# Healthcare-Robotics/mr-gan

Measured on NVIDIA B200. Metric: gan_train_step_pairs_per_sec, higher is better.
Workload: dtype f16

## Files before the change

mr_gan_b200/csrc/kernels_tc.cuh:

```cuda
#pragma once
#include <cuda.h>
#include "common.cuh"

enum { HEAD_NONE = 0, HEAD_DISC = 1, HEAD_FM = 2, HEAD_BN = 3 };

struct alignas(64) TcOp {
  CUtensorMap mapA, mapB;
  GemmDesc g;
  int ME, NE, KE;
  int bn;
  int net;
  int ws_stride;
  float* ws;
  int esz;
  int head;
  int stats_stride;
  const void* hd;
  float* stats;
};

#define TC_KBLK 32
#define TC_SPIN_LIMIT (1ll << 31)

#ifdef MRGAN_PHASE_TIMING
__device__ __forceinline__ unsigned long long gtimer() { unsigned long long t; asm volatile("mov.u64 %0, %globaltimer;" : "=l"(t)); return t; }
#define PT_MARK(i) do { pt[i] = gtimer(); } while (0)
#else
#define PT_MARK(i) do { } while (0)
#endif

namespace tc {

__device__ __forceinline__ uint32_t smem_u32(const void* p) { return (uint32_t)__cvta_generic_to_shared(p); }

__device__ __forceinline__ void mbar_init(uint64_t* bar, uint32_t count) {
  asm volatile("mbarrier.init.shared::cta.b64 [%1], %0;" ::"r"(count), "r"(smem_u32(bar)) : "memory");
}
__device__ __forceinline__ void mbar_expect_tx(uint64_t* bar, uint32_t bytes) {
  asm volatile("mbarrier.arrive.expect_tx.shared::cta.b64 _, [%1], %0;" ::"r"(bytes), "r"(smem_u32(bar)) : "memory");
}
__device__ __forceinline__ bool mbar_try_wait(uint64_t* bar, uint32_t parity) {
  uint32_t ok;
  asm volatile(
      "{\n\t.reg .pred P1;\n\t"
      "mbarrier.try_wait.parity.shared::cta.b64 P1, [%1], %2;\n\t"
      "selp.b32 %0, 1, 0, P1;\n\t}"
      : "=r"(ok) : "r"(smem_u32(bar)), "r"(parity) : "memory");
  return ok != 0;
}
__device__ __forceinline__ void mbar_wait(uint64_t* bar, uint32_t parity) {
  if (mbar_try_wait(bar, parity)) return;
  const long long t0 = clock64();
  while (!mbar_try_wait(bar, parity)) {
    if (clock64() - t0 > TC_SPIN_LIMIT) __trap();
  }
}
__device__ __forceinline__ void tma_load_2d(const CUtensorMap* map, uint64_t* bar, void* dst, int c0, int c1) {
  asm volatile(
      "cp.async.bulk.tensor.2d.shared::cluster.global.mbarrier::complete_tx::bytes [%0], [%1, {%3, %4}], [%2];"
      ::"r"(smem_u32(dst)), "l"((uint64_t)map), "r"(smem_u32(bar)), "r"(c0), "r"(c1) : "memory");
}
__device__ __forceinline__ void prefetch_map(const CUtensorMap* map) {
  asm volatile("prefetch.tensormap [%0];" ::"l"((uint64_t)map) : "memory");
}
__device__ __forceinline__ void fence_before() { asm volatile("tcgen05.fence::before_thread_sync;" ::: "memory"); }
__device__ __forceinline__ void fence_after() { asm volatile("tcgen05.fence::after_thread_sync;" ::: "memory"); }

__device__ __forceinline__ uint64_t smem_desc(uint32_t saddr, uint32_t lbo, uint32_t sbo, uint32_t layout) {
  return (uint64_t)((saddr >> 4) & 0x3FFF) | ((uint64_t)((lbo >> 4) & 0x3FFF) << 16) |
         ((uint64_t)((sbo >> 4) & 0x3FFF) << 32) | (1ull << 46) | ((uint64_t)layout << 61);
}
__device__ __forceinline__ void mma_tf32(uint32_t tmem_d, uint64_t da, uint64_t db, uint32_t idesc, uint32_t accum) {
  asm volatile(
      "{\n\t.reg .pred p;\n\t"
      "setp.ne.b32 p, %4, 0;\n\t"
      "tcgen05.mma.cta_group::1.kind::tf32 [%0], %1, %2, %3, p;\n\t}"
      ::"r"(tmem_d), "l"(da), "l"(db), "r"(idesc), "r"(accum) : "memory");
}
__device__ __forceinline__ void mma_f16(uint32_t tmem_d, uint64_t da, uint64_t db, uint32_t idesc, uint32_t accum) {
  asm volatile(
      "{\n\t.reg .pred p;\n\t"
      "setp.ne.b32 p, %4, 0;\n\t"
      "tcgen05.mma.cta_group::1.kind::f16 [%0], %1, %2, %3, p;\n\t}"
      ::"r"(tmem_d), "l"(da), "l"(db), "r"(idesc), "r"(accum) : "memory");
}
__device__ __forceinline__ void mma_commit(uint64_t* bar) {
  asm volatile("tcgen05.commit.cta_group::1.mbarrier::arrive::one.shared::cluster.b64 [%0];" ::"r"(smem_u32(bar)) : "memory");
}
__device__ __forceinline__ void tmem_ld16(uint32_t taddr, float v[16]) {
  uint32_t r[16];
  asm volatile(
      "tcgen05.ld.sync.aligned.32x32b.x16.b32 {%0, %1, %2, %3, %4, %5, %6, %7, %8, %9, %10, %11, %12, %13, %14, %15}, [%16];"
      : "=r"(r[0]), "=r"(r[1]), "=r"(r[2]), "=r"(r[3]), "=r"(r[4]), "=r"(r[5]), "=r"(r[6]), "=r"(r[7]), "=r"(r[8]),
        "=r"(r[9]), "=r"(r[10]), "=r"(r[11]), "=r"(r[12]), "=r"(r[13]), "=r"(r[14]), "=r"(r[15])
      : "r"(taddr) : "memory");
  asm volatile("tcgen05.wait::ld.sync.aligned;" ::: "memory");
#pragma unroll
  for (int i = 0; i < 16; ++i) v[i] = __uint_as_float(r[i]);
}

__device__ __forceinline__ void tmem_ld16_issue(uint32_t taddr, uint32_t (&r)[16]) {
  asm volatile(
      "tcgen05.ld.sync.aligned.32x32b.x16.b32 {%0, %1, %2, %3, %4, %5, %6, %7, %8, %9, %10, %11, %12, %13, %14, %15}, [%16];"
      : "=r"(r[0]), "=r"(r[1]), "=r"(r[2]), "=r"(r[3]), "=r"(r[4]), "=r"(r[5]), "=r"(r[6]), "=r"(r[7]), "=r"(r[8]),
        "=r"(r[9]), "=r"(r[10]), "=r"(r[11]), "=r"(r[12]), "=r"(r[13]), "=r"(r[14]), "=r"(r[15])
      : "r"(taddr) : "memory");
}
__device__ __forceinline__ void tmem_wait_ld() { asm volatile("tcgen05.wait::ld.sync.aligned;" ::: "memory"); }
__device__ __forceinline__ void tmem_fence16(uint32_t (&r)[16]) {
  asm volatile("" : "+r"(r[0]), "+r"(r[1]), "+r"(r[2]), "+r"(r[3]), "+r"(r[4]), "+r"(r[5]), "+r"(r[6]), "+r"(r[7]), "+r"(r[8]),
                    "+r"(r[9]), "+r"(r[10]), "+r"(r[11]), "+r"(r[12]), "+r"(r[13]), "+r"(r[14]), "+r"(r[15]) :: "memory");
}

__device__ __forceinline__ void tmem_ld8(uint32_t taddr, float v[8]) {
  uint32_t r[8];
  asm volatile(
      "tcgen05.ld.sync.aligned.32x32b.x8.b32 {%0, %1, %2, %3, %4, %5, %6, %7}, [%8];"
      : "=r"(r[0]), "=r"(r[1]), "=r"(r[2]), "=r"(r[3]), "=r"(r[4]), "=r"(r[5]), "=r"(r[6]), "=r"(r[7])
      : "r"(taddr) : "memory");
  asm volatile("tcgen05.wait::ld.sync.aligned;" ::: "memory");
#pragma unroll
  for (int i = 0; i < 8; ++i) v[i] = __uint_as_float(r[i]);
}

__device__ __forceinline__ void tmem_ld4(uint32_t taddr, float v[4]) {
  uint32_t r[4];
  asm volatile("tcgen05.ld.sync.aligned.32x32b.x4.b32 {%0, %1, %2, %3}, [%4];"
               : "=r"(r[0]), "=r"(r[1]), "=r"(r[2]), "=r"(r[3]) : "r"(taddr) : "memory");
  asm volatile("tcgen05.wait::ld.sync.aligned;" ::: "memory");
#pragma unroll
  for (int i = 0; i < 4; ++i) v[i] = __uint_as_float(r[i]);
}

__device__ __forceinline__ void tmem_st4(uint32_t taddr, const float v[4]) {
  asm volatile("tcgen05.st.sync.aligned.32x32b.x4.b32 [%0], {%1, %2, %3, %4};"
               ::"r"(taddr), "r"(__float_as_uint(v[0])), "r"(__float_as_uint(v[1])), "r"(__float_as_uint(v[2])), "r"(__float_as_uint(v[3]))
               : "memory");
}
__device__ __forceinline__ void tmem_st16(uint32_t taddr, const float v[16]) {
  asm volatile(
      "tcgen05.st.sync.aligned.32x32b.x16.b32 [%0], {%1, %2, %3, %4, %5, %6, %7, %8, %9, %10, %11, %12, %13, %14, %15, %16};"
      ::"r"(taddr), "r"(__float_as_uint(v[0])), "r"(__float_as_uint(v[1])), "r"(__float_as_uint(v[2])), "r"(__float_as_uint(v[3])),
        "r"(__float_as_uint(v[4])), "r"(__float_as_uint(v[5])), "r"(__float_as_uint(v[6])), "r"(__float_as_uint(v[7])),
        "r"(__float_as_uint(v[8])), "r"(__float_as_uint(v[9])), "r"(__float_as_uint(v[10])), "r"(__float_as_uint(v[11])),
        "r"(__float_as_uint(v[12])), "r"(__float_as_uint(v[13])), "r"(__float_as_uint(v[14])), "r"(__float_as_uint(v[15]))
      : "memory");
}
__device__ __forceinline__ void tmem_wait_st() { asm volatile("tcgen05.wait::st.sync.aligned;" ::: "memory"); }

}


__device__ __forceinline__ void stg_f32(float* p, float v) { asm volatile("st.global.f32 [%0], %1;" ::"l"(p), "f"(v) : "memory"); }
__device__ __forceinline__ void stg_h16(__half* p, __half v) { asm volatile("st.global.b16 [%0], %1;" ::"l"(p), "h"(__half_as_ushort(v)) : "memory"); }

template <bool F16, int ACT, bool HAS_C, bool HAS_C2, bool FULL>
__device__ __forceinline__ void fwd_rows(const uint32_t (&va)[16], const float (&nz)[16], int nrows, float* pC, __half* hC, int ldc,
                                         bool c_op, float* pC2, __half* hC2, int ldc2, bool c2_op, float sigma, float alpha, bool mul) {
  float x[16];
#pragma unroll
  for (int j = 0; j < 16; ++j) {
    float v = __uint_as_float(va[j]);
    if (!F16) v *= TF32_TRUNC_DEBIAS;
    if (ACT == ACT_RELU) v = fmaxf(v, 0.f);
    else if (ACT == ACT_SOFTPLUS) v = softplus_fast(v);
    else if (ACT == ACT_LEAKY) v = v > 0.f ? v : alpha * v;
    x[j] = v;
  }
  if (HAS_C) {
    if (!F16 && c_op) {
#pragma unroll
      for (int j = 0; j < 16; ++j) if (FULL || j < nrows) stg_f32(pC + (uint32_t)(j * ldc), rna_tf32(x[j]));
    } else {
#pragma unroll
      for (int j = 0; j < 16; ++j) if (FULL || j < nrows) stg_f32(pC + (uint32_t)(j * ldc), x[j]);
    }
    if (F16 && c_op) {
#pragma unroll
      for (int j = 0; j < 16; ++j) if (FULL || j < nrows) stg_h16(hC + (uint32_t)(j * ldc), __float2half_rn(x[j]));
    }
  }
  if (HAS_C2) {
    float y[16];
#pragma unroll
    for (int j = 0; j < 16; ++j) y[j] = mul ? x[j] * nz[j] : fmaf(sigma, nz[j], x[j]);
    if (F16 && c2_op) {
#pragma unroll
      for (int j = 0; j < 16; ++j) if (FULL || j < nrows) stg_h16(hC2 + (uint32_t)(j * ldc2), __float2half_rn(y[j]));
    } else if (!F16 && c2_op) {
#pragma unroll
      for (int j = 0; j < 16; ++j) if (FULL || j < nrows) stg_f32(pC2 + (uint32_t)(j * ldc2), rna_tf32(y[j]));
    } else {
#pragma unroll
      for (int j = 0; j < 16; ++j) if (FULL || j < nrows) stg_f32(pC2 + (uint32_t)(j * ldc2), y[j]);
    }
  }
}

template <bool F16, int ACT, bool FULL>
__device__ __forceinline__ void dx_rows(const uint32_t (&va)[16], const float (&av)[16], int nrows, float* pC, __half* hC, int ldc, bool op_only,
                                        float alpha, float dinv, bool drop) {
  float x[16];
#pragma unroll
  for (int j = 0; j < 16; ++j) {
    float v = __uint_as_float(va[j]);
    if (!F16) v *= TF32_TRUNC_DEBIAS;
    if (ACT == ACT_RELU || ACT == ACT_LEAKY) {
      float m = (av[j] > 0.f ? 1.0f : (ACT == ACT_LEAKY ? alpha : 0.f)) * dinv;
      if (drop && av[j] == 0.f) m = 0.f;
      v *= m;
    } else if (ACT == ACT_SOFTPLUS) v *= 1.0f - __expf(-av[j]);
    x[j] = v;
  }
  if (F16 && op_only) {
#pragma unroll
    for (int j = 0; j < 16; ++j) if (FULL || j < nrows) stg_h16(hC + (uint32_t)(j * ldc), grad_to_half(x[j]));
  } else if (!F16 && op_only) {
#pragma unroll
    for (int j = 0; j < 16; ++j) if (FULL || j < nrows) stg_f32(pC + (uint32_t)(j * ldc), rna_tf32(x[j]));
  } else {
#pragma unroll
    for (int j = 0; j < 16; ++j) if (FULL || j < nrows) stg_f32(pC + (uint32_t)(j * ldc), x[j]);
  }
}


template <bool F16, int ACT>
__device__ __forceinline__ void head_chunk(uint32_t taddr, float (&x)[16], float alpha = 0.f) {
  tc::tmem_ld16(taddr, x);
#pragma unroll
  for (int j = 0; j < 16; ++j) {
    if (!F16) x[j] *= TF32_TRUNC_DEBIAS;
    if (ACT == ACT_RELU) x[j] = fmaxf(x[j], 0.f);
    else if (ACT == ACT_SOFTPLUS) x[j] = softplus_fast(x[j]);
    else if (ACT == ACT_LEAKY) x[j] = x[j] > 0.f ? x[j] : alpha * x[j];
  }
}

template <bool F16, int EPW>
__device__ __forceinline__ void head_disc(uint32_t trow, int cbeg, int ncols, int nall, int lane_base, int lane, int ewarp,
                                          const LossDesc& L, const AdamHyper& hp, const OperandMode& om, float* sl, float* part) {
  const int K = hp.n_classes, B = hp.dp_bloc;
  const float Bg = (float)hp.dp_bg;
  if (lane_base == 0) {
    for (int c0 = cbeg; c0 < ncols; c0 += 16) {
      float v[16];
      head_chunk<F16, ACT_NONE>(trow + (uint32_t)c0, v);
#pragma unroll
      for (int j = 0; j < 16; ++j)
        if (lane < K && c0 + j < ncols) sl[(c0 + j) * K + lane] = v[j];
    }
  }
  asm volatile("bar.sync 1, %0;" ::"r"(32 * EPW) : "memory");
  float s_lab = 0.f, s_unl = 0.f, s_err = 0.f;
  for (int r = ewarp * 32 + lane; r < nall; r += 32 * EPW) {
    const float* l = sl + r * K;
    float mx = l[0]; int am = 0;
    for (int k = 1; k < K; ++k) if (l[k] > mx) { mx = l[k]; am = k; }
    float se = 0.f;
    for (int k = 0; k < K; ++k) se += expf(l[k] - mx);
    const float lse = mx + logf(se), inv = 1.0f / se;
    float* dl = L.dlogits + (size_t)r * L.ld;
    if (r < B) {
      const int y = L.labels[r];
      s_lab += lse - l[y];
      s_err += (am != y) ? 1.f : 0.f;
      for (int k = 0; k < K; ++k) put_grad_operand(dl + k, (expf(l[k] - mx) * inv - (k == y ? 1.f : 0.f)) / Bg, om);
    } else {
      const float sp = softplusf(lse), sg = 1.0f / (1.0f + expf(-lse));
      float coef;
      if (r < 2 * B) { s_unl += 0.5f * (sp - lse); coef = 0.5f * (sg - 1.0f); }
      else           { s_unl += 0.5f * sp;         coef = 0.5f * sg; }
      coef *= hp.w_unl / Bg;
      for (int k = 0; k < K; ++k) put_grad_operand(dl + k, coef * expf(l[k] - mx) * inv, om);
    }
  }
  s_lab = warp_sum(s_lab); s_unl = warp_sum(s_unl); s_err = warp_sum(s_err);
  if (lane == 0) { part[3 * ewarp] = s_lab; part[3 * ewarp + 1] = s_unl; part[3 * ewarp + 2] = s_err; }
}

template <bool F16, bool VAR>
__device__ __forceinline__ void head_fm(uint32_t trow, int ncols, int f, bool f_ok, int lane, const LossDesc& L, const AdamHyper& hp,
                                        const OperandMode& om, float* red) {
  constexpr int HACT = VAR ? ACT_LEAKY : ACT_RELU;
  const int B = hp.dp_bloc;
  float mg = 0.f, mr = 0.f;
  for (int c0 = 0; c0 < ncols; c0 += 16) {
    float x[16];
    head_chunk<F16, HACT>(trow + (uint32_t)c0, x, hp.alpha);
#pragma unroll
    for (int j = 0; j < 16; ++j) {
      const int r = c0 + j;
      if (r < B) mg += x[j]; else if (r < ncols) mr += x[j];
    }
  }
  const float diff = (mg - mr) / B;
  const float part = warp_sum(f_ok ? diff * diff : 0.f);
  if (lane == 0) *red = part;
  float g = 2.0f * diff / ((float)L.Wmid * B);
  if (!F16) g = rna_tf32(g);
  for (int c0 = 0; c0 < B; c0 += 16) {
    float x[16];
    head_chunk<F16, HACT>(trow + (uint32_t)c0, x, hp.alpha);
    if (!f_ok) continue;
#pragma unroll
    for (int j = 0; j < 16; ++j) {
      const int r = c0 + j;
      if (r < B) put_grad_operand(L.dmid + (size_t)r * L.lddmid + f, x[j] > 0.f ? g : hp.alpha * g, om);
    }
  }
}

template <bool F16>
__device__ __forceinline__ void head_bn(uint32_t trow, int cbeg, int ncols, int nall, int f, bool f_ok, const BnDesc& Bd,
                                        const AdamHyper& hp, const OperandMode& om) {
  float s = 0.f, q = 0.f, x0 = 0.f;
  for (int c0 = 0; c0 < nall; c0 += 16) {
    float x[16];
    head_chunk<F16, ACT_SOFTPLUS>(trow + (uint32_t)c0, x);
    if (c0 == 0) x0 = x[0];
#pragma unroll
    for (int j = 0; j < 16; ++j) if (c0 + j < nall) { const float d = x[j] - x0; s += d; q = fmaf(d, d, q); }
  }
  const float md = s / nall, mu = x0 + md;
  const float istd = rsqrtf(fmaxf(q / nall - md * md, 0.f) + hp.bn_eps);
  float ga = 0.f, be = 0.f;
  if (f_ok) { if (cbeg == 0) Bd.istd[f] = istd; ga = Bd.gamma[f]; be = Bd.beta[f]; }
  for (int c0 = cbeg; c0 < ncols; c0 += 16) {
    float x[16];
    head_chunk<F16, ACT_SOFTPLUS>(trow + (uint32_t)c0, x);
    if (!f_ok) continue;
#pragma unroll
    for (int j = 0; j < 16; ++j) {
      const int r = c0 + j;
      if (r >= ncols) break;
      const float xh = (x[j] - mu) * istd;
      Bd.xhat[(size_t)r * Bd.ld + f] = xh;
      put_operand(Bd.u + (size_t)r * Bd.ldu + f, fmaf(ga, xh, be), om);
    }
  }
}

template <bool A_MN, bool B_MN, int STAGES, int TMEM_COLS, int MINB, int EPW, int MT, bool F16, bool VAR>
__global__ void __launch_bounds__(64 + 32 * EPW, MINB)
k_gemm_tc(const TcOp* __restrict__ ops, FoldState* __restrict__ folds, int rows_override, AdamHyper hp, OperandMode om) {
  using namespace tc;
#ifdef MRGAN_PHASE_TIMING
  const unsigned long long pt_t0 = gtimer();
#endif
  constexpr int KBLK = F16 ? 64 : 32;
  constexpr uint32_t MN_BOX = F16 ? 8192u : 4096u;
  const int ksplit = (B_MN && rows_override > 1) ? rows_override : 1;
  const int kslice = (int)blockIdx.z % ksplit;
  const TcOp& op = ops[blockIdx.z / ksplit];
  const int ME = op.ME, KE = op.KE, bn = op.bn;
  int NE = op.NE;
  if (rows_override > 0 && !B_MN) NE = rows_override;
  const int m0 = blockIdx.x * 128 * MT, n0 = blockIdx.y * bn;
  if (m0 >= ME || n0 >= NE) return;

  extern __shared__ uint8_t smem_raw[];
  uint8_t* smem = reinterpret_cast<uint8_t*>((reinterpret_cast<uintptr_t>(smem_raw) + 1023) & ~(uintptr_t)1023);
  const uint32_t a_bytes = MT * 128 * 128, b_bytes = (uint32_t)bn * 128, stage_bytes = a_bytes + b_bytes;
  uint64_t* bars = reinterpret_cast<uint64_t*>(smem + STAGES * stage_bytes);
  uint64_t* full = bars;
  uint64_t* empty = bars + STAGES;
  uint64_t* tmem_full = bars + 2 * STAGES;
  uint32_t* tmem_holder = reinterpret_cast<uint32_t*>(bars + 2 * STAGES + 1);
  float* const red = reinterpret_cast<float*>(bars + 24);
#ifdef MRGAN_PHASE_TIMING
  unsigned long long* pt = reinterpret_cast<unsigned long long*>(bars + 16);
  if (threadIdx.x == 0) pt[0] = pt_t0;
#endif

  const int warp = threadIdx.x >> 5, lane = threadIdx.x & 31;
  const int nkb_all = (KE + KBLK - 1) / KBLK;
  const int kb_per = (nkb_all + ksplit - 1) / ksplit;
  const int kb0 = kslice * kb_per;
  const int nkb = min(nkb_all, kb0 + kb_per) - kb0;

  if (warp == 0 && lane == 0) {
    prefetch_map(&op.mapA);
    prefetch_map(&op.mapB);
    for (int s = 0; s < STAGES; ++s) { mbar_init(&full[s], 1); mbar_init(&empty[s], 1); }
    mbar_init(tmem_full, 1);
    asm volatile("fence.mbarrier_init.release.cluster;" ::: "memory");
  }
  if (warp == 1) {
    asm volatile("tcgen05.alloc.cta_group::1.sync.aligned.shared::cta.b32 [%0], %1;" ::"r"(smem_u32(tmem_holder)), "r"((uint32_t)TMEM_COLS) : "memory");
    asm volatile("tcgen05.relinquish_alloc_permit.cta_group::1.sync.aligned;" ::: "memory");
  }
  fence_before();
  __syncthreads();
  fence_after();
  const uint32_t tmem_base = *tmem_holder;
  if (threadIdx.x == 0) PT_MARK(1);

  if (warp == 0) {
    if (lane == 0) {
      for (int kb = 0; kb < nkb; ++kb) {
        const int s = kb % STAGES;
        const uint32_t ph = (uint32_t)(kb / STAGES) & 1u;
        mbar_wait(&empty[s], ph ^ 1u);
        mbar_expect_tx(&full[s], stage_bytes);
        uint8_t* sa = smem + (size_t)s * stage_bytes;
        uint8_t* sb = sa + a_bytes;
        const int k0 = (kb0 + kb) * KBLK;
        if (A_MN) {
#pragma unroll
          for (int b = 0; b < (128 / KBLK) * MT; ++b) tma_load_2d(&op.mapA, &full[s], sa + b * MN_BOX, m0 + KBLK * b, k0);
        } else {
#pragma unroll
          for (int mt = 0; mt < MT; ++mt) tma_load_2d(&op.mapA, &full[s], sa + mt * 16384, k0, m0 + 128 * mt);
        }
        if (B_MN) {
          for (int b = 0; b < bn / KBLK; ++b) tma_load_2d(&op.mapB, &full[s], sb + b * MN_BOX, n0 + KBLK * b, k0);
        } else {
          tma_load_2d(&op.mapB, &full[s], sb, k0, n0);
        }
      }
    }
  } else if (warp == 1) {
    if (lane == 0) {
      constexpr uint32_t fmt = F16 ? 0u : 2u;
      const uint32_t idesc = (1u << 4) | (fmt << 7) | (fmt << 10) | ((A_MN ? 1u : 0u) << 15) | ((B_MN ? 1u : 0u) << 16) |
                             ((uint32_t)(bn >> 3) << 17) | ((128u >> 4) << 24);
      constexpr uint32_t mn_lbo = MN_BOX, mn_sbo = F16 ? 1024u : 512u, mn_lay = F16 ? 2u : 1u, mn_step = F16 ? 2048u : 1024u;
      constexpr uint32_t lboA = A_MN ? mn_lbo : 16u, lboB = B_MN ? mn_lbo : 16u;
      constexpr uint32_t sboA = A_MN ? mn_sbo : 1024u, sboB = B_MN ? mn_sbo : 1024u;
      constexpr uint32_t layA = A_MN ? mn_lay : 2u, layB = B_MN ? mn_lay : 2u;
      constexpr uint32_t stepA = A_MN ? mn_step : 32u, stepB = B_MN ? mn_step : 32u;
      for (int kb = 0; kb < nkb; ++kb) {
        const int s = kb % STAGES;
        const uint32_t ph = (uint32_t)(kb / STAGES) & 1u;
        mbar_wait(&full[s], ph);
        if (kb == 0) PT_MARK(2);
        fence_after();
        const uint32_t sa = smem_u32(smem + (size_t)s * stage_bytes), sb = sa + a_bytes;
#pragma unroll
        for (int k = 0; k < 4; ++k) {
          const uint64_t db = smem_desc(sb + k * stepB, lboB, sboB, layB);
#pragma unroll
          for (int mt = 0; mt < MT; ++mt) {
            const uint64_t da = smem_desc(sa + mt * 16384u + k * stepA, lboA, sboA, layA);
            if (F16) mma_f16(tmem_base + 256u * mt, da, db, idesc, (kb > 0 || k > 0) ? 1u : 0u);
            else mma_tf32(tmem_base + 256u * mt, da, db, idesc, (kb > 0 || k > 0) ? 1u : 0u);
          }
        }
        mma_commit(&empty[s]);
      }
      mma_commit(tmem_full);
      PT_MARK(3);
    }
  } else {
    const int lane_base = 32 * (warp & 3);
    const int wg = (warp - 2) >> 2;
    const int sub = (MT == 2) ? wg : 0;
    const int chalf = (EPW == 8 && MT == 1) ? (((min(bn, NE - n0) + 1) / 2 + 15) & ~15) : bn;
    const int cbeg = (EPW == 8 && MT == 1) ? wg * chalf : 0;
    const int f = m0 + 128 * sub + lane_base + lane;
    const bool f_ok = f < ME;
    const GemmDesc g = op.g;
    constexpr float debias = F16 ? 1.0f : TF32_TRUNC_DEBIAS;
    const int ncols = min(min(bn, NE - n0), cbeg + chalf);
    const uint32_t trow = tmem_base + 256u * sub + ((uint32_t)lane_base << 16);
    int fbeg, flen;
    if (MT == 2) { fbeg = 256 * sub + bn; flen = (256 - bn) & ~15; }
    else { flen = ((TMEM_COLS - bn) / (EPW == 8 ? 2 : 1)) & ~15; fbeg = bn + wg * flen; }
    const uint32_t tfree = tmem_base + ((uint32_t)lane_base << 16) + (uint32_t)fbeg;
    const int nchunks = (ncols - cbeg + 15) >> 4;
    const int npark = max(min(flen >> 4, nchunks), 0);

    if constexpr (B_MN) {
      mbar_wait(tmem_full, 0);
      fence_after();
      float* const dst = ksplit > 1 ? op.ws + (size_t)kslice * op.ws_stride : g.C;
      for (int c0 = cbeg; c0 < ncols; c0 += 16) {
        float v[16];
        tmem_ld16(trow + (uint32_t)c0, v);
        if (!f_ok) continue;
#pragma unroll
        for (int j = 0; j < 16; ++j) {
          const int k = n0 + c0 + j;
          if (k >= NE) break;
          dst[(size_t)k * g.ldc + f] = v[j];
        }
      }
    } else if constexpr (!A_MN) {
      const bool has_act = g.act != ACT_NONE;
      const bool drop = VAR && hp.drop > 0.f && (g.act == ACT_RELU || g.act == ACT_LEAKY) && g.tid >= 1;
      const __half* const haux = (F16 && drop) ? om.hbase + (g.aux - om.fbase) : nullptr;
      auto fetch = [&](int c0, float (&av)[16]) {
#pragma unroll
        for (int j = 0; j < 16; ++j) {
          const size_t o = (size_t)(n0 + c0 + j) * g.ldaux + f;
          av[j] = (f_ok && has_act && c0 + j < ncols) ? (haux ? __half2float(haux[o]) : __ldg(g.aux + o)) : 1.0f;
        }
      };
      float avA[16], avB[16];
      const int npk = has_act ? npark : 0;
      if (npk > 0) {
        fetch(cbeg, avA);
        for (int k = 0; k < npk; k += 2) {
          if (k + 1 < npk) fetch(cbeg + 16 * (k + 1), avB);
          tmem_st16(tfree + 16u * (uint32_t)k, avA);
          if (k + 1 < npk) {
            if (k + 2 < npk) fetch(cbeg + 16 * (k + 2), avA);
            tmem_st16(tfree + 16u * (uint32_t)(k + 1), avB);
          }
        }
        tmem_wait_st();
      }
      if (has_act && npk < nchunks) fetch(cbeg + 16 * npk, avA);
      mbar_wait(tmem_full, 0);
      fence_after();
      __half* const hC = F16 ? om.hbase + (g.C - om.fbase) : nullptr;
      const bool op_only = (g.rnd & 1) != 0;
      for (int ch = 0; ch < nchunks; ++ch) {
        const int c0 = cbeg + 16 * ch;
        uint32_t va[16], vh[16];
        tmem_ld16_issue(trow + (uint32_t)c0, va);
        if (ch < npk) tmem_ld16_issue(tfree + 16u * (uint32_t)ch, vh);
        tmem_wait_ld();
        tmem_fence16(va);
        float av[16];
        if (ch < npk) {
          tmem_fence16(vh);
#pragma unroll
          for (int j = 0; j < 16; ++j) av[j] = __uint_as_float(vh[j]);
        } else if (has_act) {
          const bool odd = ((ch - npk) & 1) != 0;
#pragma unroll
          for (int j = 0; j < 16; ++j) av[j] = odd ? avB[j] : avA[j];
          if (ch + 1 < nchunks) { if (odd) fetch(c0 + 16, avA); else fetch(c0 + 16, avB); }
        } else {
#pragma unroll
          for (int j = 0; j < 16; ++j) av[j] = 1.0f;
        }
        if (!f_ok) continue;
        const size_t o0 = (size_t)(n0 + c0) * g.ldc + f;
        const int nrows = ncols - c0;
        float* const pC = g.C + o0;
        __half* const phC = F16 ? hC + o0 : nullptr;
        const float dinv = drop ? hp.drop_inv : 1.0f;
#define DX_ACT(FULL)                                                                                                        \
        do {                                                                                                                    \
          if (g.act == ACT_RELU) dx_rows<F16, ACT_RELU, FULL>(va, av, nrows, pC, phC, g.ldc, op_only, 0.f, dinv, drop);         \
          else if (VAR && g.act == ACT_LEAKY) dx_rows<F16, ACT_LEAKY, FULL>(va, av, nrows, pC, phC, g.ldc, op_only, hp.alpha, dinv, drop); \
          else if (g.act == ACT_SOFTPLUS) dx_rows<F16, ACT_SOFTPLUS, FULL>(va, av, nrows, pC, phC, g.ldc, op_only, 0.f, 1.0f, false);      \
          else dx_rows<F16, ACT_NONE, FULL>(va, av, nrows, pC, phC, g.ldc, op_only, 0.f, 1.0f, false);                          \
        } while (0)
        if (nrows >= 16) DX_ACT(true); else DX_ACT(false);
#undef DX_ACT
      }
    } else {
      const bool mul = VAR && hp.drop > 0.f && g.C2 != nullptr && g.tid >= 1;
      const float ddrop = mul ? hp.drop : 0.f;
      const bool noisy = g.C2 != nullptr && (g.sigma != 0.f || mul);
      uint32_t key0 = 0, key1 = 0, step = 0;
      if (noisy) { const FoldState& fs = folds[g.fold]; key0 = fs.key0; key1 = fs.key1; step = (uint32_t)fs.rng_step; }
      const bool grp = ((g.row0 + n0 + cbeg) & 3) == 0 && (hp.dp_bg == hp.dp_bloc || (hp.dp_bloc & 3) == 0);
      const bool dp = hp.dp_bg != hp.dp_bloc;
      const int dprank = hp.dp_rank < 0 ? g.fold : hp.dp_rank;
      auto draw16 = [&](int c0, float (&nz)[16]) {
        const int r0 = g.row0 + n0 + c0;
        if (grp && !dp) {
#pragma unroll
          for (int q = 0; q < 4; ++q) {
            if (VAR) noise_or_drop4(key0, key1, (uint32_t)(r0 + 4 * q) >> 2, (uint32_t)f, step, (uint32_t)g.tid, ddrop, hp.drop_inv, &nz[4 * q]);
            else normal4(key0, key1, (uint32_t)(r0 + 4 * q) >> 2, (uint32_t)f, step, (uint32_t)g.tid, &nz[4 * q]);
          }
        } else if (grp) {
#pragma unroll
          for (int q = 0; q < 4; ++q) {
            const float4 n4 = noise4_call(key0, key1, r0 + 4 * q, (uint32_t)f, step, (uint32_t)g.tid, hp.dp_bloc, hp.dp_bg, dprank, ddrop, hp.drop_inv);
            nz[4 * q] = n4.x; nz[4 * q + 1] = n4.y; nz[4 * q + 2] = n4.z; nz[4 * q + 3] = n4.w;
          }
        } else {
#pragma unroll
          for (int j = 0; j < 16; ++j)
            nz[j] = noise1_call(key0, key1, r0 + j, (uint32_t)f, step, (uint32_t)g.tid, hp.dp_bloc, hp.dp_bg, dprank, ddrop, hp.drop_inv);
        }
      };
      const int npk = (noisy && grp) ? npark : 0;
      for (int ch = 0; ch < npk; ++ch) {
        float nz[16];
        draw16(cbeg + 16 * ch, nz);
        tmem_st16(tfree + 16u * (uint32_t)ch, nz);
      }
      if (npk > 0) tmem_wait_st();
      if (warp == 2 && lane == 0) PT_MARK(4);
      mbar_wait(tmem_full, 0);
      if (warp == 2 && lane == 0) PT_MARK(5);
      fence_after();
      __half* const hC = (F16 && g.C) ? om.hbase + (g.C - om.fbase) : nullptr;
      __half* const hC2 = (F16 && g.C2) ? om.hbase + (g.C2 - om.fbase) : nullptr;
      const bool c_op = (g.rnd & 1) != 0, c2_op = (g.rnd & 2) != 0;
#ifdef MRGAN_PHASE_TIMING
      unsigned long long tch[24];
#endif
      for (int it = 0; it < nchunks; ++it) {
        const int ch = (wg & 1) ? nchunks - 1 - it : it;
        const int c0 = cbeg + 16 * ch;
        uint32_t va[16], vn[16];
        float nz[16];
#ifdef MRGAN_PHASE_TIMING
        if (ch < 12) tch[2 * ch] = gtimer();
#endif
        tmem_ld16_issue(trow + (uint32_t)c0, va);
        if (ch < npk) tmem_ld16_issue(tfree + 16u * (uint32_t)ch, vn);
        else if (noisy) draw16(c0, nz);
        tmem_wait_ld();
#ifdef MRGAN_PHASE_TIMING
        if (ch < 12) tch[2 * ch + 1] = gtimer();
#endif
        tmem_fence16(va);
        if (ch < npk) {
          tmem_fence16(vn);
#pragma unroll
          for (int j = 0; j < 16; ++j) nz[j] = __uint_as_float(vn[j]);
        }
        if (!f_ok) continue;
        const size_t o0 = (size_t)(n0 + c0) * g.ldc + f, o20 = (size_t)(n0 + c0) * g.ldc2 + f;
        const int nrows = ncols - c0;
        float* const pC = g.C ? g.C + o0 : nullptr;
        float* const pC2 = g.C2 ? g.C2 + o20 : nullptr;
        __half* const phC = hC ? hC + o0 : nullptr;
        __half* const phC2 = hC2 ? hC2 + o20 : nullptr;
        if (!noisy) {
#pragma unroll
          for (int j = 0; j < 16; ++j) nz[j] = 0.f;
        }
#define FWD_ROWS(ACT, HC, HC2, FULL) \
        fwd_rows<F16, ACT, HC, HC2, FULL>(va, nz, nrows, pC, phC, g.ldc, c_op, pC2, phC2, g.ldc2, c2_op, g.sigma, hp.alpha, VAR && mul)
#define FWD_ACT(HC, HC2, FULL)                                                     \
        do {                                                                       \
          if (g.act == ACT_RELU) FWD_ROWS(ACT_RELU, HC, HC2, FULL);                \
          else if (g.act == ACT_SOFTPLUS) FWD_ROWS(ACT_SOFTPLUS, HC, HC2, FULL);   \
          else if (VAR && g.act == ACT_LEAKY) FWD_ROWS(ACT_LEAKY, HC, HC2, FULL);  \
          else FWD_ROWS(ACT_NONE, HC, HC2, FULL);                                  \
        } while (0)
#define FWD_OUT(FULL)                                                              \
        do {                                                                       \
          if (g.C && g.C2) FWD_ACT(true, true, FULL);                              \
          else if (g.C) FWD_ACT(true, false, FULL);                                \
          else if (g.C2) FWD_ACT(false, true, FULL);                               \
        } while (0)
        if (nrows >= 16) FWD_OUT(true); else FWD_OUT(false);
#undef FWD_OUT
#undef FWD_ACT
#undef FWD_ROWS
      }
#ifdef MRGAN_PHASE_TIMING
      if (warp == 2 && lane == 0 && blockIdx.x == 0 && blockIdx.z == 0 && nchunks >= 10) {
        const unsigned long long te2 = gtimer();
        const unsigned long long b = pt[0];
        printf("PTCH npk=%d: %llu+%llu %llu+%llu %llu+%llu %llu+%llu %llu+%llu %llu+%llu %llu+%llu %llu+%llu %llu+%llu %llu+%llu end=%llu\n", npk,
               tch[0] - b, tch[1] - tch[0], tch[2] - b, tch[3] - tch[2], tch[4] - b, tch[5] - tch[4], tch[6] - b, tch[7] - tch[6], tch[8] - b, tch[9] - tch[8],
               tch[10] - b, tch[11] - tch[10], tch[12] - b, tch[13] - tch[12], tch[14] - b, tch[15] - tch[14], tch[16] - b, tch[17] - tch[16],
               tch[18] - b, tch[19] - tch[18], te2 - b);
      }
#endif
      if (op.head == HEAD_DISC) {
        float* const sl = reinterpret_cast<float*>(smem);
        head_disc<F16, EPW>(trow, cbeg, ncols, min(bn, NE - n0), lane_base, lane, warp - 2, *static_cast<const LossDesc*>(op.hd), hp, om,
                            sl, sl + 8192);
      } else if (op.head == HEAD_FM) {
        head_fm<F16, VAR>(trow, ncols, f, f_ok, lane, *static_cast<const LossDesc*>(op.hd), hp, om, red + (warp - 2));
      } else if (op.head == HEAD_BN) {
        head_bn<F16>(trow, cbeg, ncols, min(bn, NE - n0), f, f_ok, *static_cast<const BnDesc*>(op.hd), hp, om);
      }
    }
  }

  if (warp == 2 && lane == 0) PT_MARK(6);
  fence_before();
  __syncthreads();
  if (warp == 1) {
    fence_after();
    asm volatile("tcgen05.dealloc.cta_group::1.sync.aligned.b32 %0, %1;" ::"r"(tmem_base), "r"((uint32_t)TMEM_COLS) : "memory");
  }
  if (!B_MN && A_MN && threadIdx.x == 0 && (op.head == HEAD_DISC || op.head == HEAD_FM)) {
    float* const st = op.stats + (size_t)hp.t * op.stats_stride;
    if (op.head == HEAD_DISC) {
      const float Bg = (float)hp.dp_bg;
      const float* part = reinterpret_cast<const float*>(smem) + 8192;
      float a0 = 0.f, a1 = 0.f, a2 = 0.f;
      for (int w = 0; w < EPW; ++w) { a0 += part[3 * w]; a1 += part[3 * w + 1]; a2 += part[3 * w + 2]; }
      st[0] = a0 / Bg; st[1] = a1 / Bg; st[2] = a2 / Bg;
      FoldState& fs = folds[op.g.fold];
      if (hp.shared_t) fs.iterations += 1; else fs.it_net[0] += 1;
      fs.rng_step += 1;
    } else {
      float sum = 0.f;
      for (int w = 0; w < EPW; ++w) sum += red[w];
      st[3] = sum / static_cast<const LossDesc*>(op.hd)->Wmid;
    }
  }
#ifdef MRGAN_PHASE_TIMING
  if (threadIdx.x == 0 && blockIdx.x == 0 && blockIdx.y == 0 && (blockIdx.z % 24) == 0) {
    const unsigned long long te = gtimer();
    printf("PT z=%d grid=(%d,%d,%d) nkb=%d t0=%llu setup=%llu first=%llu mma_issued=%llu noise=%llu acc=%llu epi=%llu end=%llu\n", (int)blockIdx.z,
           (int)gridDim.x, (int)gridDim.y, (int)gridDim.z, nkb, pt[0], pt[1] - pt[0], pt[2] - pt[0], pt[3] - pt[0], pt[4] - pt[0], pt[5] - pt[0], pt[6] - pt[0], te - pt[0]);
  }
#endif
}

__global__ void __launch_bounds__(256) k_splitk_reduce(const TcOp* __restrict__ ops, int ks) {
  const TcOp& op = ops[blockIdx.y];
  const size_t n4 = (size_t)op.NE * op.g.ldc / 4, stride4 = (size_t)op.ws_stride / 4;
  const float4* __restrict__ ws = reinterpret_cast<const float4*>(op.ws);
  float4* __restrict__ out = reinterpret_cast<float4*>(op.g.C);
  for (size_t i = (size_t)blockIdx.x * blockDim.x + threadIdx.x; i < n4; i += (size_t)gridDim.x * blockDim.x) {
    float4 a = ws[i];
    for (int s = 1; s < ks; ++s) {
      const float4 b = ws[(size_t)s * stride4 + i];
      a.x += b.x; a.y += b.y; a.z += b.z; a.w += b.w;
    }
    out[i] = a;
  }
}

struct alignas(64) TcAdamOp {
  CUtensorMap mapA, mapB;
  CUtensorMap mapP, mapM, mapV;
  CUtensorMap mapH;
  int ME, NE, KE;
  int fold;
  int net;
  float ginv;
};

#define TCA_KC 8

namespace tc {
__device__ __forceinline__ void tma_store_2d(const CUtensorMap* map, const void* src, int c0, int c1) {
  asm volatile("cp.async.bulk.tensor.2d.global.shared::cta.bulk_group [%0, {%2, %3}], [%1];"
               ::"l"((uint64_t)map), "r"(smem_u32(src)), "r"(c0), "r"(c1) : "memory");
}
__device__ __forceinline__ void bulk_commit() { asm volatile("cp.async.bulk.commit_group;" ::: "memory"); }
__device__ __forceinline__ void bulk_wait_read0() { asm volatile("cp.async.bulk.wait_group.read 0;" ::: "memory"); }
__device__ __forceinline__ void mbar_arrive(uint64_t* bar) {
  asm volatile("mbarrier.arrive.shared::cta.b64 _, [%0];" ::"r"(smem_u32(bar)) : "memory");
}
__device__ __forceinline__ void fence_proxy_async() { asm volatile("fence.proxy.async.shared::cta;" ::: "memory"); }
}

template <bool F16, int KROWS> struct TcAdamCfg {
  static_assert(KROWS == (F16 ? 32 : 16), "operand stage geometry: 16 KB stages");
  static constexpr int STAGES = 2, KC = TCA_KC, NB = 3;
  static constexpr int MINB = 3;
  static constexpr uint32_t MN_BOX = 128u * KROWS;
  static constexpr uint32_t STAGE_BYTES = (F16 ? 4 : 8) * MN_BOX;
  static constexpr uint32_t ARR_BYTES = KC * 128 * 4;
  static constexpr uint32_t HALF_BYTES = F16 ? KC * 128 * 2 : 0;
  static constexpr uint32_t CHUNK_BYTES = 3 * ARR_BYTES + HALF_BYTES;
  static constexpr int NX = (STAGES * STAGE_BYTES) / CHUNK_BYTES;
  static constexpr int NBUF = NB + NX;
  static constexpr size_t SMEM = (size_t)STAGES * STAGE_BYTES + (size_t)NB * CHUNK_BYTES + 256;
};

template <bool F16, int KROWS>
__global__ void __launch_bounds__(192, (TcAdamCfg<F16, KROWS>::MINB))
k_dw_adam_tc(const TcAdamOp* __restrict__ ops, FoldState* __restrict__ folds, AdamHyper hp, int nfl, int op_stride) {
  using namespace tc;
  using Cfg = TcAdamCfg<F16, KROWS>;
  constexpr int STAGES = Cfg::STAGES, KC = Cfg::KC, NB = Cfg::NB, NBUF = Cfg::NBUF;
  constexpr uint32_t STAGE_BYTES = Cfg::STAGE_BYTES, ARR_BYTES = Cfg::ARR_BYTES, CHUNK_BYTES = Cfg::CHUNK_BYTES;
  constexpr int KBLK = KROWS;
  constexpr uint32_t MN_BOX = Cfg::MN_BOX;
  constexpr int MN_BOXES = F16 ? 2 : 4;
  constexpr int MN_W = F16 ? 64 : 32;
  const TcAdamOp& op = ops[((int)blockIdx.z / nfl) * op_stride + ((int)blockIdx.z % nfl)];
  const int ME = op.ME, NE = op.NE, KE = op.KE;
  const int m0 = blockIdx.x * 128, n0 = blockIdx.y * 128;
  if (m0 >= ME || n0 >= NE) return;

  extern __shared__ __align__(1024) uint8_t smem_dyn[];
  uint8_t* smem = smem_dyn;
  if ((smem_u32(smem) & 1023u) != 0) __trap();
  uint8_t* cbuf = smem + STAGES * STAGE_BYTES;
  uint64_t* bars = reinterpret_cast<uint64_t*>(cbuf + NB * CHUNK_BYTES);
  uint64_t* full = bars;
  uint64_t* empty = bars + STAGES;
  uint64_t* tmem_full = bars + 2 * STAGES;
  uint64_t* cfull = bars + 2 * STAGES + 1;
  uint64_t* cdone = cfull + NBUF;
  uint32_t* tmem_holder = reinterpret_cast<uint32_t*>(cdone + NBUF);
  auto buf_ptr = [&](int b) -> uint8_t* { return b < NB ? cbuf + (size_t)b * CHUNK_BYTES : smem + (size_t)(b - NB) * CHUNK_BYTES; };

  const int warp = threadIdx.x >> 5, lane = threadIdx.x & 31;
  const int nkb = (KE + KBLK - 1) / KBLK;
  const int ncols = min(128, NE - n0);
  const int nch = (ncols + KC - 1) / KC;

  if (warp == 0 && lane == 0) {
    prefetch_map(&op.mapA); prefetch_map(&op.mapB); prefetch_map(&op.mapP); prefetch_map(&op.mapM); prefetch_map(&op.mapV);
    if (F16) prefetch_map(&op.mapH);
    for (int s = 0; s < STAGES; ++s) { mbar_init(&full[s], 1); mbar_init(&empty[s], 1); }
    mbar_init(tmem_full, 1);
    for (int b = 0; b < NBUF; ++b) { mbar_init(&cfull[b], 1); mbar_init(&cdone[b], 128); }
    asm volatile("fence.mbarrier_init.release.cluster;" ::: "memory");
  }
  if (warp == 1) {
    asm volatile("tcgen05.alloc.cta_group::1.sync.aligned.shared::cta.b32 [%0], %1;" ::"r"(smem_u32(tmem_holder)), "r"(128u) : "memory");
    asm volatile("tcgen05.relinquish_alloc_permit.cta_group::1.sync.aligned;" ::: "memory");
  }
  fence_before();
  __syncthreads();
  fence_after();
  const uint32_t tmem_base = *tmem_holder;

  if (warp == 0) {
    if (lane == 0) {
      auto load_chunk = [&](int c) {
        const int b = c % NBUF;
        uint8_t* dst = buf_ptr(b);
        mbar_expect_tx(&cfull[b], 3 * ARR_BYTES);
        tma_load_2d(&op.mapP, &cfull[b], dst, m0, n0 + c * KC);
        tma_load_2d(&op.mapM, &cfull[b], dst + ARR_BYTES, m0, n0 + c * KC);
        tma_load_2d(&op.mapV, &cfull[b], dst + 2 * ARR_BYTES, m0, n0 + c * KC);
      };
      for (int c = 0; c < NB && c < nch; ++c) load_chunk(c);
      for (int kb = 0; kb < nkb; ++kb) {
        const int s = kb % STAGES;
        const uint32_t ph = (uint32_t)(kb / STAGES) & 1u;
        mbar_wait(&empty[s], ph ^ 1u);
        mbar_expect_tx(&full[s], STAGE_BYTES);
        uint8_t* sa = smem + (size_t)s * STAGE_BYTES;
        uint8_t* sb = sa + STAGE_BYTES / 2;
        const int k0 = kb * KBLK;
#pragma unroll
        for (int b = 0; b < MN_BOXES; ++b) tma_load_2d(&op.mapA, &full[s], sa + b * MN_BOX, m0 + MN_W * b, k0);
#pragma unroll
        for (int b = 0; b < MN_BOXES; ++b) tma_load_2d(&op.mapB, &full[s], sb + b * MN_BOX, n0 + MN_W * b, k0);
      }
      mbar_wait(tmem_full, 0);
      for (int c = NB; c < NBUF && c < nch; ++c) load_chunk(c);
      for (int c = 0; c < nch; ++c) {
        const int b = c % NBUF;
        mbar_wait(&cdone[b], (uint32_t)(c / NBUF) & 1u);
        const uint8_t* src = buf_ptr(b);
        tma_store_2d(&op.mapP, src, m0, n0 + c * KC);
        tma_store_2d(&op.mapM, src + ARR_BYTES, m0, n0 + c * KC);
        tma_store_2d(&op.mapV, src + 2 * ARR_BYTES, m0, n0 + c * KC);
        if (F16) tma_store_2d(&op.mapH, src + 3 * ARR_BYTES, m0, n0 + c * KC);
        bulk_commit();
        if (c >= 1 && c - 1 + NBUF < nch) {
          asm volatile("cp.async.bulk.wait_group.read 1;" ::: "memory");
          load_chunk(c - 1 + NBUF);
        }
      }
      bulk_wait_read0();
    }
  } else if (warp == 1) {
    if (lane == 0) {
      constexpr uint32_t fmt = F16 ? 0u : 2u;
      constexpr uint32_t idesc = (1u << 4) | (fmt << 7) | (fmt << 10) | (1u << 15) | (1u << 16) | ((128u >> 3) << 17) | ((128u >> 4) << 24);
      constexpr uint32_t lbo = MN_BOX, sbo = F16 ? 1024u : 512u, lay = F16 ? 2u : 1u, kstep = F16 ? 2048u : 1024u;
      for (int kb = 0; kb < nkb; ++kb) {
        const int s = kb % STAGES;
        const uint32_t ph = (uint32_t)(kb / STAGES) & 1u;
        mbar_wait(&full[s], ph);
        fence_after();
        const uint32_t sa = smem_u32(smem + (size_t)s * STAGE_BYTES), sb = sa + STAGE_BYTES / 2;
#pragma unroll
        for (int k = 0; k < KROWS / (F16 ? 16 : 8); ++k) {
          const uint64_t da = smem_desc(sa + k * kstep, lbo, sbo, lay), db = smem_desc(sb + k * kstep, lbo, sbo, lay);
          if (F16) mma_f16(tmem_base, da, db, idesc, (kb > 0 || k > 0) ? 1u : 0u);
          else mma_tf32(tmem_base, da, db, idesc, (kb > 0 || k > 0) ? 1u : 0u);
        }
        mma_commit(&empty[s]);
      }
      mma_commit(tmem_full);
    }
  } else {
    const int lane_base = 32 * (warp & 3);
    const int nl = lane_base + lane;
    const uint32_t trow = tmem_base + ((uint32_t)lane_base << 16);
    const float lr_t = folds[op.fold].lr_t[op.net];
    const float b1 = hp.b1, b2 = hp.b2, c1 = 1.0f - hp.b1, c2 = 1.0f - hp.b2, eps = hp.eps;
    const float ginv = op.ginv;
    mbar_wait(tmem_full, 0);
    fence_after();
    for (int c = 0; c < nch; ++c) {
      const int b = c % NBUF;
      float* sP = reinterpret_cast<float*>(buf_ptr(b));
      float* sM = sP + KC * 128;
      float* sV = sM + KC * 128;
      __half* sH = reinterpret_cast<__half*>(sV + KC * 128);
      float g[KC];
      tmem_ld8(trow + (uint32_t)(c * KC), g);
      mbar_wait(&cfull[b], (uint32_t)(c / NBUF) & 1u);
#pragma unroll
      for (int j = 0; j < KC; ++j) {
        const int i = j * 128 + nl;
        const float gr = F16 ? g[j] * ginv : g[j];
        const float m = fmaf(b1, sM[i], c1 * gr), v = fmaf(b2, sV[i], c2 * gr * gr);
        sM[i] = m; sV[i] = v;
        const float w = sP[i] - lr_t * __fdividef(m, sqrtf(v) + eps);
        sP[i] = w;
        if (F16) sH[i] = __float2half_rn(w);
      }
      fence_proxy_async();
      mbar_arrive(&cdone[b]);
    }
  }

  fence_before();
  __syncthreads();
  if (warp == 1) {
    fence_after();
    asm volatile("tcgen05.dealloc.cta_group::1.sync.aligned.b32 %0, %1;" ::"r"(tmem_base), "r"(128u) : "memory");
  }
}
```

mr_gan_b200/csrc/mrgan_api.cu:

```cuda
#include <cuda_runtime.h>
#include <cuda_fp16.h>
#include <dlfcn.h>
#include <math.h>
#include <stdio.h>
#include <stdlib.h>
#include <string.h>
#include <algorithm>
#include <map>
#include <string>
#include <vector>

#include "../../include/mrgan.h"
#include "kernels_simt.cuh"
#include "kernels_tc.cuh"
#include "kernels_svm.cuh"
#include "kernels_dp.cuh"

namespace {

thread_local std::string g_last_error;

enum Op {
  OP_G1, OP_G2, OP_G3D, OP_G3G,
  OP_D1, OP_D2, OP_D3, OP_D4, OP_D5, OP_D6,
  OP_DW1, OP_DW2, OP_DW3, OP_DW4, OP_DW5, OP_DW6,
  OP_DX2, OP_DX3, OP_DX4, OP_DX5, OP_DX6,
  OP_DX1G,
  OP_D1G, OP_D2G, OP_D3G, OP_D4G, OP_D5G,
  OP_DX2G, OP_DX3G, OP_DX4G, OP_DX5G,
  OP_GW1, OP_GW2, OP_GW3, OP_GX2, OP_GX3,
  OP_E1, OP_E1S, OP_E2, OP_E3, OP_E4, OP_E5, OP_E6,
  NUM_OPS,
  OP_EX2 = NUM_OPS, OP_EX3, OP_EX4, OP_EX5, OP_EX6,
  OP_EX1,
  NUM_OPS_ALL
};
constexpr int NUM_EX = NUM_OPS_ALL - NUM_OPS;

struct OpInfo { bool at = false, bt = false, used = false; int maxM = 0, maxN = 0; };

struct Arena {
  char* base = nullptr; size_t off = 0;
  template <typename T> T* take(size_t count) {
    off = (off + 255) & ~(size_t)255;
    T* p = base ? reinterpret_cast<T*>(base + off) : nullptr;
    off += count * sizeof(T);
    return p;
  }
};

struct TensorLayout { int rows, cols, pitch; long long off; };

struct NetLayout {
  std::vector<TensorLayout> t;
  long long n = 0;
  long long n_ref = 0;
  long long off = 0;
};

struct FoldBuffers {
  float *a[6], *hb[6], *dz[6], *lg, *dlg, *dfake, *zb, *h1g, *xhat, *istd, *u, *h2g, *dz2g, *du, *dz1g;
  float *stage_x, *stage_z, *ex_stage, *xte, *eh[6], *elg, *xtr, *eval_out, *eval_out_s;
  int *stage_y, *labels_cur, *ey_stage, *ytr, *yte, *idx;
  int *pred, *pred_s;
  int *lab_rows, *unl_rows;
  int n_lab = 0, n_unl = 0;
  int lda[6], ldz[6];
  bool loaded = false;
};

}

struct mrgan_handle;
namespace {
int tc_setup(mrgan_handle* h);
int tc_ex_setup(mrgan_handle* h, TcOp* dst);
void tc_teardown(mrgan_handle* h);
bool tc_launch_gemm(mrgan_handle* h, int op, int f0, int nfl, int rows_override, cudaStream_t st);
void tc_launch_dw_adam(mrgan_handle* h, int op, int nlayers, int f0, int nfl, cudaStream_t st);
bool tc_dw_merge(const mrgan_handle* h);
int tc_debug_gemm(mrgan_handle* h, int mode, const GemmDesc& g, int esz);
}

constexpr int kMaxChains = 16;
struct mrgan_handle {
  mrgan_config cfg;
  int nf = 0, R = 0, NE = 0, n_train = 0;
  std::vector<mrgan_fold_shape> shapes;
  std::vector<NetLayout> net[2];
  std::vector<FoldBuffers> fb;
  cudaStream_t stream = nullptr;
  cudaStream_t side = nullptr;
  cudaEvent_t ev_pool[16] = {nullptr}; int ev_next = 0;
  bool side_open = false;
  int nchains = 1;
  cudaStream_t cmain[kMaxChains] = {nullptr}, cside[kMaxChains] = {nullptr};
  char* arena = nullptr; size_t arena_bytes = 0;
  __half* harena = nullptr;
  OperandMode om = {0, 1.0f, nullptr, nullptr};
  float *P = nullptr, *Mo = nullptr, *Vo = nullptr, *Gr = nullptr; long long n_flat = 0;
  FoldState* d_folds = nullptr; std::vector<FoldState> h_folds;
  GemmDesc* d_descs = nullptr; std::vector<GemmDesc> h_descs;
  PermDesc* d_perm = nullptr;
  BnDesc* d_bn = nullptr; LossDesc* d_loss = nullptr; EvalDesc *d_eval = nullptr, *d_eval_s = nullptr;
  int* d_conf = nullptr;
  struct SalWork {
    char* mem = nullptr;
    GemmDesc* descs = nullptr;
    float* profile = nullptr;
    TcOp* tcops = nullptr;
  } sal;
  AdamRange* d_ranges[2] = {nullptr, nullptr};
  OpInfo ops[NUM_OPS_ALL];
  float *d_step_stats = nullptr, *d_epoch_stats = nullptr, *h_epoch_stats = nullptr;
  int* h_idx_pinned[2] = {nullptr, nullptr}; cudaEvent_t idx_free[2] = {nullptr, nullptr}; int idx_slot = 0;
  float* h_scratch = nullptr;
  std::map<int, cudaGraphExec_t> graphs;
  std::map<int, long long> graph_nodes;
  cudaEvent_t ev0 = nullptr, ev1 = nullptr;
  bool epoch_pending = false; double last_ms = 0.0;
  long long launches = 0;
  std::string err;
  int sticky = 0;
  AdamHyper hp;
  struct Dataset { float* x = nullptr; int* y = nullptr; int n = 0, D = 0, ld = 0; } datasets[8];
  double* d_prep_stats = nullptr; int* d_prep_rows = nullptr; int prep_rows_cap = 0, prep_stats_cap = 0;
  int dp_world = 1, dp_rank = 0;
  bool dp_virtual = false;
  bool dp_fused = false;
  unsigned* d_dpflags = nullptr;
  char* peer_arena[DP_MAX_RANKS] = {nullptr}; __half* peer_harena[DP_MAX_RANKS] = {nullptr};
  DpPeers dp_peers[2];
  void* nccl_comm = nullptr;
  float* d_dpmem = nullptr; DpBufs* d_dpbufs = nullptr;
  float *dp_bnf = nullptr, *dp_bnb = nullptr, *dp_fm = nullptr;
  float* dp_losspart = nullptr; unsigned* dp_lossctr = nullptr;
  TcOp* d_tcops = nullptr;
  int tc_bn[NUM_OPS_ALL] = {0}, tc_maxME[NUM_OPS_ALL] = {0}, tc_maxNE[NUM_OPS_ALL] = {0};
  int tc_ksplit[NUM_OPS] = {0};
  bool tc_mt1[NUM_OPS_ALL] = {false};
  float* d_tcws = nullptr;
  bool tc_fused_adam = true;
  int tc_heads = 0;
  TcAdamOp* d_tcadam = nullptr;
  AdamRange* d_ranges_tc[2] = {nullptr, nullptr};
  struct Svm {
    char* mem = nullptr; size_t bytes = 0;
    int n_lab = 0, npairs = 0, npmax = 0, max_rows = 0, max_nte = 0;
    double eps = 1e-3;
    bool fitted = false;
    std::vector<float*> Klab, Kte, dec;
    std::vector<int*> wrong;
    int *d_iters = nullptr, *d_capped = nullptr, *d_count = nullptr, *d_nte = nullptr;
    SvmSplitOp* d_split = nullptr; SvmGemmOp* d_gemm = nullptr; SvmPairJob* d_jobs = nullptr;
    float** d_Kt = nullptr; float** d_dec = nullptr; int** d_yte = nullptr; int** d_wrong = nullptr; int** d_pred = nullptr;
    std::vector<SvmGemmOp> h_gemm;
    float *Xs = nullptr, *Hs = nullptr, *Ls = nullptr, *Ks = nullptr, *decs = nullptr; double* ns = nullptr; int* preds = nullptr;
    SvmSplitOp* d_split_s = nullptr; SvmGemmOp* d_gemm_s = nullptr;
    float** d_Ks = nullptr; float** d_decs = nullptr; int** d_preds = nullptr; int* d_ns = nullptr;
    char* cv_mem = nullptr; size_t cv_bytes = 0;
  } svm;
};

namespace {

int take_sticky(mrgan_handle* h);

int fail(mrgan_handle* h, int code, const std::string& msg) {
  if (h) h->err = msg;
  g_last_error = msg;
  return code;
}

#define CKS()                                                                                      \
  do {                                                                                             \
    CK(cudaGetLastError());                                                                        \
    const int _s = take_sticky(h);                                                                 \
    if (_s) return _s;                                                                             \
  } while (0)

#define CK(expr)                                                                                   \
  do {                                                                                             \
    cudaError_t _e = (expr);                                                                       \
    if (_e != cudaSuccess)                                                                         \
      return fail(h, MRGAN_ERR_CUDA, std::string(#expr) + ": " + cudaGetErrorString(_e));          \
  } while (0)

const int kDW[5] = {1000, 500, 250, 250, 250};
const int kGH = 500;

long long align32(long long x) { return (x + 31) & ~31LL; }

NetLayout layout_disc(int D, int K) {
  NetLayout L;
  int dims[7] = {D, kDW[0], kDW[1], kDW[2], kDW[3], kDW[4], K};
  for (int l = 0; l < 6; ++l) {
    TensorLayout t{dims[l] + 1, dims[l + 1], pitch8(dims[l + 1]), L.n};
    L.t.push_back(t);
    L.n = align32(L.n + (long long)t.rows * t.pitch);
    L.n_ref += (long long)(dims[l] + 1) * dims[l + 1];
  }
  return L;
}

NetLayout layout_gen(int D, int nd) {
  NetLayout L;
  auto add = [&](int rows, int cols) {
    TensorLayout t{rows, cols, pitch8(cols), L.n};
    L.t.push_back(t);
    L.n = align32(L.n + (long long)rows * t.pitch);
    L.n_ref += (long long)rows * cols;
  };
  add(nd + 1, kGH);
  add(1, kGH);
  add(1, kGH);
  add(kGH + 1, kGH);
  add(kGH + 1, D);
  return L;
}

__global__ void k_round_tf32(float* p, size_t n) {
  for (size_t i = (size_t)blockIdx.x * blockDim.x + threadIdx.x; i < n; i += (size_t)gridDim.x * blockDim.x) p[i] = rna_tf32(p[i]);
}

__global__ void k_set_col(float* p, int ld, int rows, int col, float v, OperandMode om) {
  const int r = blockIdx.x * blockDim.x + threadIdx.x;
  if (r < rows) {
    p[(size_t)r * ld + col] = v;
    if (om.mode == 2) om.hbase[p + (size_t)r * ld + col - om.fbase] = __float2half_rn(v);
  }
}

__global__ void k_scale_buf(float* p, size_t n, float mul) {
  for (size_t i = (size_t)blockIdx.x * blockDim.x + threadIdx.x; i < n; i += (size_t)gridDim.x * blockDim.x) p[i] *= mul;
}

__global__ void k_from_half(const float* src, float* dst, size_t n, float mul, OperandMode om) {
  for (size_t i = (size_t)blockIdx.x * blockDim.x + threadIdx.x; i < n; i += (size_t)gridDim.x * blockDim.x)
    dst[i] = __half2float(om.hbase[src + i - om.fbase]) * mul;
}

void layout_buffers(mrgan_handle* h, Arena& ar) {
  const mrgan_config& c = h->cfg;
  const int B = c.batch, R = h->R, NE = h->NE, K = c.n_classes, nd = c.noise_dim, nf = h->nf;
  const bool gan = c.model == MRGAN_MODEL_GAN;
  if (c.model == MRGAN_MODEL_SVM) {
    for (int f = 0; f < nf; ++f) {
      FoldBuffers& b = h->fb[f];
      const int D = h->shapes[f].D;
      b.lda[0] = pitch8(D + 1);
      b.xte = ar.take<float>((size_t)h->shapes[f].n_test * b.lda[0]);
      b.xtr = ar.take<float>((size_t)h->shapes[f].n_train * pitch8(D));
      b.ytr = ar.take<int>(h->shapes[f].n_train);
      b.yte = ar.take<int>(h->shapes[f].n_test);
      b.pred = ar.take<int>(h->shapes[f].n_test);
    }
    h->d_eval = ar.take<EvalDesc>(nf);
    h->d_conf = ar.take<int>((size_t)nf * K * K);
    return;
  }
  h->P = ar.take<float>(h->n_flat);
  h->Mo = ar.take<float>(h->n_flat);
  h->Vo = ar.take<float>(h->n_flat);
  h->Gr = ar.take<float>(h->n_flat);
  h->d_folds = ar.take<FoldState>(nf);
  h->d_descs = ar.take<GemmDesc>((size_t)NUM_OPS * nf);
  h->d_perm = ar.take<PermDesc>(nf);
  h->d_bn = ar.take<BnDesc>(nf);
  h->d_loss = ar.take<LossDesc>(nf);
  h->d_eval = ar.take<EvalDesc>(nf);
  h->d_eval_s = ar.take<EvalDesc>(nf);
  h->d_ranges[0] = ar.take<AdamRange>(nf);
  h->d_ranges[1] = ar.take<AdamRange>(nf);
  h->d_step_stats = ar.take<float>((size_t)(h->n_train / B + 1) * nf * 4);
  h->d_dpflags = ar.take<unsigned>((size_t)DP_MAX_RANKS * DP_FLAG_WORDS);
  h->d_epoch_stats = ar.take<float>((size_t)nf * 8);
  for (int f = 0; f < nf; ++f) {
    FoldBuffers& b = h->fb[f];
    const int D = h->shapes[f].D, ntr = h->shapes[f].n_train, nte = h->shapes[f].n_test;
    const int ldx = pitch8(D);
    int win[6] = {D, kDW[0], kDW[1], kDW[2], kDW[3], kDW[4]};
    for (int l = 0; l < 6; ++l) { b.lda[l] = pitch8(win[l] + 1); b.ldz[l] = pitch8(win[l]); }
    b.a[0] = ar.take<float>((size_t)R * b.lda[0]);
    b.hb[0] = nullptr; b.dz[0] = nullptr;
    for (int l = 1; l <= 5; ++l) {
      b.hb[l] = ar.take<float>((size_t)R * b.lda[l]);
      b.a[l] = (l < 5) ? ar.take<float>((size_t)R * b.lda[l]) : b.hb[l];
      b.dz[l] = ar.take<float>((size_t)R * b.ldz[l]);
    }
    b.lg = ar.take<float>((size_t)R * pitch8(K));
    b.dlg = ar.take<float>((size_t)R * pitch8(K));
    b.labels_cur = ar.take<int>(R);
    b.stage_x = ar.take<float>((size_t)R * ldx);
    b.stage_y = ar.take<int>(R);
    if (gan) {
      b.dfake = ar.take<float>((size_t)B * ldx);
      b.zb = ar.take<float>((size_t)B * pitch8(nd + 1));
      const int ldg = pitch8(kGH);
      b.h1g = ar.take<float>((size_t)B * ldg);
      b.xhat = ar.take<float>((size_t)B * ldg);
      b.istd = ar.take<float>(kGH);
      b.u = ar.take<float>((size_t)B * pitch8(kGH + 1));
      b.h2g = ar.take<float>((size_t)B * pitch8(kGH + 1));
      b.dz2g = ar.take<float>((size_t)B * ldg);
      b.du = ar.take<float>((size_t)B * ldg);
      b.dz1g = ar.take<float>((size_t)B * ldg);
      b.stage_z = ar.take<float>((size_t)B * nd);
    }
    b.ex_stage = ar.take<float>((size_t)NE * b.lda[0]);
    b.xte = ar.take<float>((size_t)nte * b.lda[0]);
    for (int l = 1; l <= 5; ++l) b.eh[l] = ar.take<float>((size_t)NE * b.lda[l]);
    b.elg = ar.take<float>((size_t)NE * pitch8(K));
    b.ey_stage = ar.take<int>(NE);
    b.eval_out = ar.take<float>(4);
    b.eval_out_s = ar.take<float>(4);
    b.xtr = ar.take<float>((size_t)ntr * ldx);
    b.ytr = ar.take<int>(ntr);
    b.yte = ar.take<int>(nte);
    b.idx = ar.take<int>((size_t)3 * ntr);
    b.lab_rows = ar.take<int>(ntr);
    b.unl_rows = ar.take<int>(ntr);
    b.pred = ar.take<int>(nte);
    b.pred_s = ar.take<int>(NE);
  }
  h->d_conf = ar.take<int>((size_t)nf * K * K);
}

GemmDesc make_desc(const float* A, int lda, const float* Bm, int ldb, float* C, int ldc, int M, int N, int K, int epi,
                   int act, int fold) {
  GemmDesc d;
  memset(&d, 0, sizeof(d));
  d.A = A; d.lda = lda; d.B = Bm; d.ldb = ldb; d.C = C; d.ldc = ldc; d.M = M; d.N = N; d.K = K;
  d.epi = epi; d.act = act; d.fold = fold;
  return d;
}

int build_descs(mrgan_handle* h) {
  const mrgan_config& c = h->cfg;
  const int B = c.batch, R = h->R, K = c.n_classes, nd = c.noise_dim, nf = h->nf;
  const bool gan = c.model == MRGAN_MODEL_GAN;
  h->h_descs.assign((size_t)NUM_OPS_ALL * nf, GemmDesc{});
  h->h_folds.assign(nf, FoldState{});
  std::vector<BnDesc> bn(nf); std::vector<LossDesc> ls(nf); std::vector<EvalDesc> ev(nf), evs(nf);
  std::vector<AdamRange> rg0(nf), rg1(nf);
  const bool tensor = c.precision != MRGAN_PREC_FP32;
  auto setop = [&](int op, int f, GemmDesc d, bool at, bool bt, int rnd = 0) {
    d.rnd = tensor ? rnd : 0;
    h->h_descs[(size_t)op * nf + f] = d;
    OpInfo& oi = h->ops[op];
    oi.at = at; oi.bt = bt; oi.used = true;
    if (d.M > oi.maxM) oi.maxM = d.M;
    if (d.N > oi.maxN) oi.maxN = d.N;
  };
  for (int f = 0; f < nf; ++f) {
    FoldBuffers& b = h->fb[f];
    const int D = h->shapes[f].D;
    const NetLayout& LD = h->net[0][f];
    float* PD = h->P + LD.off; float* GD = h->Gr + LD.off;
    int win[6] = {D, kDW[0], kDW[1], kDW[2], kDW[3], kDW[4]};
    int wout[6] = {kDW[0], kDW[1], kDW[2], kDW[3], kDW[4], K};
    const float sig[5] = {c.sigma_in, c.sigma_hidden, c.sigma_hidden, c.sigma_hidden, c.sigma_hidden};
    const int hact = c.hidden_act == MRGAN_ACT_LEAKY_RELU ? ACT_LEAKY : ACT_RELU;
    const bool dropout = c.dropout > 0.0f;
    for (int l = 1; l <= 6; ++l) {
      const TensorLayout& W = LD.t[l - 1];
      float* C = (l <= 5) ? b.hb[l] : b.lg;
      const int ldc = (l <= 5) ? b.lda[l] : pitch8(K);
      GemmDesc d = make_desc(b.a[l - 1], b.lda[l - 1], PD + W.off, W.pitch, C, ldc, R, wout[l - 1], win[l - 1] + 1,
                             EPI_FWD, l <= 5 ? hact : ACT_NONE, f);
      if (l <= 4) { d.C2 = b.a[l]; d.ldc2 = b.lda[l]; d.sigma = sig[l]; d.tid = l; d.row0 = 0; }
      setop(OP_D1 + l - 1, f, d, false, false, (l == 5 ? 1 : 0) | 2);
      if (gan && l <= 5) { GemmDesc dg = d; dg.M = 2 * B; setop(OP_D1G + l - 1, f, dg, false, false, (l == 5 ? 1 : 0) | 2); }
      const float* EA = (l == 1) ? b.xte : b.eh[l - 1];
      float* EC = (l <= 5) ? b.eh[l] : b.elg;
      GemmDesc e = make_desc(EA, b.lda[l - 1], PD + W.off, W.pitch, EC, ldc, h->shapes[f].n_test, wout[l - 1],
                             win[l - 1] + 1, EPI_FWD, l <= 5 ? hact : ACT_NONE, f);
      setop(l == 1 ? OP_E1 : OP_E2 + l - 2, f, e, false, false, l <= 5 ? 1 : 0);
      if (l == 1) { e.A = b.ex_stage; setop(OP_E1S, f, e, false, false, 1); }
      const float* dZ = (l <= 5) ? b.dz[l] : b.dlg;
      const int lddz = (l <= 5) ? b.ldz[l] : pitch8(K);
      GemmDesc w = make_desc(b.a[l - 1], b.lda[l - 1], dZ, lddz, GD + W.off, W.pitch, win[l - 1] + 1, wout[l - 1], R,
                             EPI_STORE, ACT_NONE, f);
      setop(OP_DW1 + l - 1, f, w, true, false);
// ... 5 lines not shown
        if (gan && l <= 5) { GemmDesc xg = x; xg.M = B; setop(OP_DX2G + l - 2, f, xg, false, true, 1); }
        GemmDesc ex = make_desc(EC, ldc, PD + W.off, W.pitch, b.eh[l - 1], b.lda[l - 1], h->shapes[f].n_test, win[l - 1], wout[l - 1],
                                EPI_DX, hact, f);
        ex.aux = b.eh[l - 1]; ex.ldaux = b.lda[l - 1]; ex.tid = 0;
        setop(OP_EX2 + l - 2, f, ex, false, true, 1);
      }
    }
    const TensorLayout& EW1 = LD.t[0];
    setop(OP_EX1, f, make_desc(b.eh[1], b.lda[1], PD + EW1.off, EW1.pitch, b.ex_stage, b.lda[0], h->shapes[f].n_test, D, kDW[0], EPI_DX,
                               ACT_NONE, f), false, true);
    rg0[f] = AdamRange{LD.off, LD.n};
    ls[f] = LossDesc{b.lg, b.dlg, pitch8(K), b.labels_cur, b.hb[5], b.dz[5], b.lda[5], b.ldz[5], kDW[4]};
    ev[f] = EvalDesc{b.elg, pitch8(K), b.yte, h->shapes[f].n_test, (h->shapes[f].n_test / B) * B, b.eval_out, b.pred};
    evs[f] = EvalDesc{b.elg, pitch8(K), b.ey_stage, h->shapes[f].n_test, 0, b.eval_out_s, b.pred_s};
    if (gan) {
      const NetLayout& LG = h->net[1][f];
      float* PG = h->P + LG.off; float* GG = h->Gr + LG.off;
      const TensorLayout &W1 = LG.t[0], &Tg = LG.t[1], &Tb = LG.t[2], &W2 = LG.t[3], &W3 = LG.t[4];
      const int ldzb = pitch8(nd + 1), ldu = pitch8(kGH + 1), ldx = pitch8(D), ldg = pitch8(kGH);
      setop(OP_G1, f, make_desc(b.zb, ldzb, PG + W1.off, W1.pitch, b.h1g, ldg, B, kGH, nd + 1, EPI_FWD, ACT_SOFTPLUS, f), false, false);
      setop(OP_G2, f, make_desc(b.u, ldu, PG + W2.off, W2.pitch, b.h2g, ldu, B, kGH, kGH + 1, EPI_FWD, ACT_SOFTPLUS, f), false, false, 1);
      GemmDesc g3 = make_desc(b.h2g, ldu, PG + W3.off, W3.pitch, nullptr, 0, B, D, kGH + 1, EPI_FWD, ACT_NONE, f);
      g3.C2 = b.a[0] + (size_t)2 * B * b.lda[0]; g3.ldc2 = b.lda[0]; g3.sigma = c.sigma_in; g3.tid = 0; g3.row0 = 2 * B;
      setop(OP_G3D, f, g3, false, false, 2);
      g3.C2 = b.a[0]; g3.row0 = 0;
      setop(OP_G3G, f, g3, false, false, 2);
      const TensorLayout& DW1 = LD.t[0];
      setop(OP_DX1G, f, make_desc(b.dz[1], b.ldz[1], PD + DW1.off, DW1.pitch, b.dfake, ldx, B, D, kDW[0], EPI_DX, ACT_NONE, f), false, true, 1);
      setop(OP_GW3, f, make_desc(b.h2g, ldu, b.dfake, ldx, GG + W3.off, W3.pitch, kGH + 1, D, B, EPI_STORE, ACT_NONE, f), true, false);
      GemmDesc gx3 = make_desc(b.dfake, ldx, PG + W3.off, W3.pitch, b.dz2g, ldg, B, kGH, D, EPI_DX, ACT_SOFTPLUS, f);
      gx3.aux = b.h2g; gx3.ldaux = ldu;
      setop(OP_GX3, f, gx3, false, true, 1);
      setop(OP_GW2, f, make_desc(b.u, ldu, b.dz2g, ldg, GG + W2.off, W2.pitch, kGH + 1, kGH, B, EPI_STORE, ACT_NONE, f), true, false);
      setop(OP_GX2, f, make_desc(b.dz2g, ldg, PG + W2.off, W2.pitch, b.du, ldg, B, kGH, kGH, EPI_DX, ACT_NONE, f), false, true);
      setop(OP_GW1, f, make_desc(b.zb, ldzb, b.dz1g, ldg, GG + W1.off, W1.pitch, nd + 1, kGH, B, EPI_STORE, ACT_NONE, f), true, false);
      bn[f] = BnDesc{b.h1g, b.xhat, b.u, b.istd, PG + Tg.off, PG + Tb.off, b.du, b.dz1g, GG + Tg.off, GG + Tb.off,
                     ldg, ldu, B, kGH};
      rg1[f] = AdamRange{LG.off, LG.n};
    }
    FoldState& fs = h->h_folds[f];
    fs.key0 = (uint32_t)(h->shapes[f].seed & 0xFFFFFFFFull);
    fs.key1 = (uint32_t)(h->shapes[f].seed >> 32);
    fs.D = D; fs.n_train = h->shapes[f].n_train; fs.n_test = h->shapes[f].n_test; fs.ldx = pitch8(D);
    fs.x_train = b.xtr; fs.y_train = b.ytr; fs.y_test = b.yte;
    for (int s = 0; s < 3; ++s) fs.idx[s] = b.idx + (size_t)s * h->shapes[f].n_train;
    fs.stage_x = b.stage_x; fs.stage_y = b.stage_y; fs.stage_z = gan ? b.stage_z : nullptr;
    fs.a0 = b.a[0]; fs.lda0 = b.lda[0]; fs.z = gan ? b.zb : nullptr; fs.ldz = pitch8(nd + 1);
    fs.labels_cur = b.labels_cur;
  }
  CK(cudaMemcpy(h->d_descs, h->h_descs.data(), (size_t)NUM_OPS * nf * sizeof(GemmDesc), cudaMemcpyHostToDevice));
  CK(cudaMemcpy(h->d_folds, h->h_folds.data(), nf * sizeof(FoldState), cudaMemcpyHostToDevice));
  CK(cudaMemcpy(h->d_loss, ls.data(), nf * sizeof(LossDesc), cudaMemcpyHostToDevice));
  CK(cudaMemcpy(h->d_eval, ev.data(), nf * sizeof(EvalDesc), cudaMemcpyHostToDevice));
  CK(cudaMemcpy(h->d_eval_s, evs.data(), nf * sizeof(EvalDesc), cudaMemcpyHostToDevice));
  CK(cudaMemcpy(h->d_ranges[0], rg0.data(), nf * sizeof(AdamRange), cudaMemcpyHostToDevice));
  if (gan) {
    CK(cudaMemcpy(h->d_bn, bn.data(), nf * sizeof(BnDesc), cudaMemcpyHostToDevice));
    CK(cudaMemcpy(h->d_ranges[1], rg1.data(), nf * sizeof(AdamRange), cudaMemcpyHostToDevice));
  }
  return MRGAN_OK;
}

void set_ones(mrgan_handle* h, float* p, int ld, int rows, int col) {
  k_set_col<<<(rows + 127) / 128, 128, 0, h->stream>>>(p, ld, rows, col, 1.0f, h->om);
}

void init_ones(mrgan_handle* h) {
  const mrgan_config& c = h->cfg;
  const bool gan = c.model == MRGAN_MODEL_GAN;
  for (int f = 0; f < h->nf; ++f) {
    FoldBuffers& b = h->fb[f];
    const int D = h->shapes[f].D;
    int win[6] = {D, kDW[0], kDW[1], kDW[2], kDW[3], kDW[4]};
    set_ones(h, b.a[0], b.lda[0], h->R, D);
    set_ones(h, b.ex_stage, b.lda[0], h->NE, D);
    set_ones(h, b.xte, b.lda[0], h->shapes[f].n_test, D);
    for (int l = 1; l <= 5; ++l) {
      set_ones(h, b.hb[l], b.lda[l], h->R, win[l]);
      if (l < 5) set_ones(h, b.a[l], b.lda[l], h->R, win[l]);
      set_ones(h, b.eh[l], b.lda[l], h->NE, win[l]);
    }
    if (gan) {
      set_ones(h, b.zb, pitch8(c.noise_dim + 1), c.batch, c.noise_dim);
      set_ones(h, b.u, pitch8(kGH + 1), c.batch, kGH);
      set_ones(h, b.h2g, pitch8(kGH + 1), c.batch, kGH);
    }
  }
}


template <typename... KArgs, typename... Args>
void launch_k(mrgan_handle* h, void (*kern)(KArgs...), dim3 grid, dim3 block, size_t smem, cudaStream_t st, Args... args) {
  cudaLaunchConfig_t cfg;
  memset(&cfg, 0, sizeof(cfg));
  cfg.gridDim = grid; cfg.blockDim = block; cfg.dynamicSmemBytes = smem; cfg.stream = st;
  const cudaError_t e = cudaLaunchKernelEx(&cfg, kern, static_cast<KArgs>(args)...);
  if (e != cudaSuccess && !h->sticky) { h->sticky = MRGAN_ERR_CUDA; h->err = std::string("kernel launch: ") + cudaGetErrorString(e); }
  h->launches++;
}

int take_sticky(mrgan_handle* h) {
  if (!h->sticky) return MRGAN_OK;
  const int code = h->sticky;
  h->sticky = 0;
  g_last_error = h->err;
  return code;
}

struct NcclId { char b[128]; };
struct NcclApi {
  void* lib = nullptr;
  int (*GetUniqueId)(NcclId*) = nullptr;
  int (*CommInitRank)(void**, int, NcclId, int) = nullptr;
  int (*AllReduce)(const void*, void*, size_t, int, int, void*, cudaStream_t) = nullptr;
  int (*CommDestroy)(void*) = nullptr;
  const char* (*GetErrorString)(int) = nullptr;
};
NcclApi g_nccl;

bool nccl_load() {
  if (g_nccl.lib) return true;
  void* lib = dlopen("libnccl.so.2", RTLD_NOW | RTLD_GLOBAL);
  if (!lib) lib = dlopen("libnccl.so", RTLD_NOW | RTLD_GLOBAL);
  if (!lib) return false;
  g_nccl.GetUniqueId = (int (*)(NcclId*))dlsym(lib, "ncclGetUniqueId");
  g_nccl.CommInitRank = (int (*)(void**, int, NcclId, int))dlsym(lib, "ncclCommInitRank");
  g_nccl.AllReduce = (int (*)(const void*, void*, size_t, int, int, void*, cudaStream_t))dlsym(lib, "ncclAllReduce");
  g_nccl.CommDestroy = (int (*)(void*))dlsym(lib, "ncclCommDestroy");
  g_nccl.GetErrorString = (const char* (*)(int))dlsym(lib, "ncclGetErrorString");
  if (!g_nccl.GetUniqueId || !g_nccl.CommInitRank || !g_nccl.AllReduce || !g_nccl.CommDestroy) return false;
  g_nccl.lib = lib;
  return true;
}

__global__ void k_virtual_allreduce(float* __restrict__ buf, size_t seg, int W) {
  for (size_t i = (size_t)blockIdx.x * blockDim.x + threadIdx.x; i < seg; i += (size_t)gridDim.x * blockDim.x) {
    float s = 0.f;
    for (int w = 0; w < W; ++w) s += buf[(size_t)w * seg + i];
    for (int w = 0; w < W; ++w) buf[(size_t)w * seg + i] = s;
  }
}

void dp_allreduce(mrgan_handle* h, float* buf, size_t n) {
  if (h->dp_world <= 1 || n == 0) return;
  if (h->dp_virtual) {
    const size_t seg = n / (size_t)h->dp_world;
    const int blocks = (int)std::min<size_t>((seg + 255) / 256, 1184);
    k_virtual_allreduce<<<blocks, 256, 0, h->stream>>>(buf, seg, h->dp_world);
    h->launches++;
    return;
  }
  const int rc = g_nccl.AllReduce(buf, buf, n, 7, 0, h->nccl_comm, h->stream);
  if (rc != 0 && !h->sticky) {
    h->sticky = MRGAN_ERR_CUDA;
    h->err = std::string("ncclAllReduce: ") + (g_nccl.GetErrorString ? g_nccl.GetErrorString(rc) : "error");
  }
}

void dp_allreduce_grads(mrgan_handle* h, int net) {
  if (h->dp_world <= 1) return;
  long long n = 0;
  for (int f = 0; f < h->nf; ++f) n += h->net[net][f].n;
  dp_allreduce(h, h->Gr + h->net[net][0].off, (size_t)n);
}

void launch_adam(mrgan_handle* h, int f0, int nfl, int net);

void dp_build_peers(mrgan_handle* h) {
  const float* abase = reinterpret_cast<const float*>(h->arena);
  for (int net = 0; net < 2; ++net) {
    DpPeers& pp = h->dp_peers[net];
    memset(&pp, 0, sizeof(pp));
    if (h->net[net].empty()) continue;
    for (int p = 0; p < h->dp_world; ++p) {
      if (h->dp_virtual) {
        const long long d = h->net[net][p].off - h->net[net][0].off;
        pp.P[p] = h->P + d; pp.Gr[p] = h->Gr + d; pp.Mo[p] = h->Mo + d; pp.Vo[p] = h->Vo + d;
        pp.Ph[p] = h->harena ? h->harena + (h->P - abase) + d : nullptr;
        pp.flags[p] = h->d_dpflags + (size_t)p * DP_FLAG_WORDS;
      } else {
        float* pb = reinterpret_cast<float*>(h->peer_arena[p]);
        pp.P[p] = pb + (h->P - abase); pp.Gr[p] = pb + (h->Gr - abase); pp.Mo[p] = pb + (h->Mo - abase); pp.Vo[p] = pb + (h->Vo - abase);
        pp.Ph[p] = h->peer_harena[p] ? h->peer_harena[p] + (h->P - abase) : nullptr;
        pp.flags[p] = reinterpret_cast<unsigned*>(h->peer_arena[p] + (reinterpret_cast<char*>(h->d_dpflags) - h->arena));
      }
    }
  }
}

void dp_exchange(mrgan_handle* h, int net) {
  long long len = 0;
  if (h->dp_virtual) len = h->net[net][0].n;
  else for (int f = 0; f < h->nf; ++f) len += h->net[net][f].n;
  const long long off = h->net[net][0].off;
  const int W = h->dp_world;
  const int bx = h->dp_virtual ? std::max(1, 296 / W) : 296;
  cudaLaunchConfig_t cfg;
  memset(&cfg, 0, sizeof(cfg));
  cfg.gridDim = dim3(bx, h->dp_virtual ? W : 1, 1); cfg.blockDim = dim3(256); cfg.stream = h->stream;
  cudaLaunchAttribute attr[1];
  attr[0].id = cudaLaunchAttributeCooperative;
  attr[0].val.cooperative = 1;
  cfg.attrs = attr; cfg.numAttrs = 1;
  const float ginv = h->om.mode == 2 ? 1.0f / h->om.gscale : 1.0f;
  const cudaError_t e = cudaLaunchKernelEx(&cfg, k_dp_exchange, h->dp_peers[net], W, h->dp_virtual ? -1 : h->dp_rank, off, len, h->d_folds,
                                           h->nf, net, h->hp, ginv);
  if (e != cudaSuccess && !h->sticky) { h->sticky = MRGAN_ERR_CUDA; h->err = std::string("k_dp_exchange launch: ") + cudaGetErrorString(e); }
  h->launches++;
}

void dp_update(mrgan_handle* h, int f0, int nfl, int net) {
  if (h->dp_fused) { dp_exchange(h, net); return; }
  dp_allreduce_grads(h, net);
  launch_adam(h, f0, nfl, net);
}

int alloc_split_bufs(mrgan_handle* h) {
  if (h->d_dpbufs) return MRGAN_OK;
  const int nf = h->nf;
  const size_t stats = 2 * kGH + 2 * kGH + 2 * kDW[4];
  const size_t per = stats + (size_t)SPLIT_MAX_Y * 2 * SPLIT_PART_W + 4 * LOSS_MAX_BLOCKS + 32;
  CK(cudaMalloc(&h->d_dpmem, per * nf * sizeof(float)));
  CK(cudaMemset(h->d_dpmem, 0, per * nf * sizeof(float)));
  h->dp_bnf = h->d_dpmem; h->dp_bnb = h->dp_bnf + (size_t)nf * 2 * kGH; h->dp_fm = h->dp_bnb + (size_t)nf * 2 * kGH;
  float* const part = h->dp_fm + (size_t)nf * 2 * kDW[4];
  h->dp_losspart = part + (size_t)nf * SPLIT_MAX_Y * 2 * SPLIT_PART_W;
  unsigned* const ctr = reinterpret_cast<unsigned*>(h->dp_losspart + (size_t)nf * 4 * LOSS_MAX_BLOCKS);
  h->dp_lossctr = ctr + (size_t)nf * 16;
  std::vector<DpBufs> bufs(nf);
  for (int f = 0; f < nf; ++f)
    bufs[f] = DpBufs{h->dp_bnf + (size_t)f * 2 * kGH, h->dp_bnb + (size_t)f * 2 * kGH, h->dp_fm + (size_t)f * 2 * kDW[4],
                     part + (size_t)f * SPLIT_MAX_Y * 2 * SPLIT_PART_W, ctr + (size_t)f * 16};
  CK(cudaMalloc(&h->d_dpbufs, nf * sizeof(DpBufs)));
  CK(cudaMemcpy(h->d_dpbufs, bufs.data(), nf * sizeof(DpBufs), cudaMemcpyHostToDevice));
  return MRGAN_OK;
}

int split_chunks(int rows) {
  const int y = (rows + 255) / 256;
  return y < 1 ? 1 : (y > SPLIT_MAX_Y ? SPLIT_MAX_Y : y);
}

void launch_gemm(mrgan_handle* h, int op, int f0, int nfl, int rows_override, cudaStream_t st = nullptr) {
  if (!st) st = h->stream;
  const OpInfo& oi = h->ops[op];
  int M = oi.maxM;
  if (rows_override > 0 && !oi.at) M = rows_override;
  const GemmDesc* d = (op < NUM_OPS ? h->d_descs + (size_t)op * h->nf : h->sal.descs + (size_t)(op - NUM_OPS) * h->nf) + f0;
  if (h->cfg.precision != MRGAN_PREC_FP32 && tc_launch_gemm(h, op, f0, nfl, rows_override, st)) return;
  dim3 grid((oi.maxN + 63) / 64, (M + 63) / 64, nfl);
  if (!oi.at && !oi.bt) launch_k(h, k_gemm_simt<false, false>, grid, dim3(256), 0, st, d, (const FoldState*)h->d_folds, rows_override, h->hp);
  else if (!oi.at && oi.bt) launch_k(h, k_gemm_simt<false, true>, grid, dim3(256), 0, st, d, (const FoldState*)h->d_folds, rows_override, h->hp);
  else launch_k(h, k_gemm_simt<true, false>, grid, dim3(256), 0, st, d, (const FoldState*)h->d_folds, rows_override, h->hp);
}

void fork_side(mrgan_handle* h) {
  cudaEvent_t e = h->ev_pool[h->ev_next++ & 15];
  cudaEventRecord(e, h->stream);
  cudaStreamWaitEvent(h->side, e, 0);
  h->side_open = true;
}
void join_side(mrgan_handle* h) {
  if (!h->side_open) return;
  h->side_open = false;
  cudaEvent_t e = h->ev_pool[h->ev_next++ & 15];
  cudaEventRecord(e, h->side);
  cudaStreamWaitEvent(h->stream, e, 0);
}

int max_D(const mrgan_handle* h, int f0, int nfl) {
  int m = 0;
  for (int f = f0; f < f0 + nfl; ++f) m = h->shapes[f].D > m ? h->shapes[f].D : m;
  return m;
}

void launch_prep(mrgan_handle* h, int f0, int nfl, int mode, int from_stage, int t, int nrows) {
  const mrgan_config& c = h->cfg;
  int cols = max_D(h, f0, nfl);
  if (c.noise_dim > cols) cols = c.noise_dim;
  const int pg = nrows > 512 ? 4 : 2;
  dim3 grid((cols + 127) / 128, (nrows + 4 * pg - 1) / (4 * pg), nfl);
#define LAUNCH_PREP(PG) launch_k(h, k_prep<PG>, grid, dim3(128), 0, h->stream, h->d_folds, f0, mode, from_stage, t, c.batch, nrows, c.noise_dim, \
                                 c.sigma_in, h->hp, h->om)
  if (pg == 4) LAUNCH_PREP(4); else LAUNCH_PREP(2);
#undef LAUNCH_PREP
}

void launch_adam(mrgan_handle* h, int f0, int nfl, int net) {
  long long nmax = 0;
  for (int f = f0; f < f0 + nfl; ++f) nmax = h->net[net][f].n > nmax ? h->net[net][f].n : nmax;
  int blocks = (int)((nmax / 4 + 255) / 256);
  if (blocks > 2048) blocks = 2048;
  if (blocks < 1) blocks = 1;
  const AdamRange* ranges = h->d_ranges[net];
  if (h->cfg.precision != MRGAN_PREC_FP32 && h->tc_fused_adam) { ranges = h->d_ranges_tc[net]; blocks = 1; }
  const float ginv = h->om.mode == 2 ? 1.0f / h->om.gscale : 1.0f;
  __half* Ph = h->om.mode == 2 ? h->harena + (h->P - reinterpret_cast<float*>(h->arena)) : nullptr;
  launch_k(h, k_adam, dim3(blocks, nfl), dim3(256), 0, h->stream, h->P, h->Mo, h->Vo, (const float*)h->Gr, ranges, h->d_folds, f0, net, h->hp,
           ginv, Ph);
}

int heads_on(const mrgan_handle* h) { return h->cfg.precision != MRGAN_PREC_FP32 ? h->tc_heads : 0; }

void enqueue_gen_fwd(mrgan_handle* h, int f0, int nfl, int op_g3) {
  launch_gemm(h, OP_G1, f0, nfl, 0);
  if (heads_on(h) & 4) {
    launch_gemm(h, OP_G2, f0, nfl, 0);
    launch_gemm(h, op_g3, f0, nfl, 0);
    return;
  }
  const dim3 bnf((kGH + BN_COLS - 1) / BN_COLS, h->d_dpbufs ? split_chunks(h->cfg.batch) : 1, nfl);
  const dim3 bnt(h->cfg.batch > 256 ? 1024 : 256);
  const OperandMode tf32 = h->om;
  if (h->d_dpbufs) {
    k_bn_stats<<<bnf, bnt, 0, h->stream>>>(h->d_bn + f0, h->d_dpbufs + f0);
    dp_allreduce(h, h->dp_bnf + (size_t)f0 * 2 * kGH, (size_t)nfl * 2 * kGH);
    k_bn_apply<<<bnf, bnt, 0, h->stream>>>(h->d_bn + f0, h->d_dpbufs + f0, h->cfg.bn_eps, tf32, h->hp.dp_bg);
    h->launches += 2;
  } else {
    launch_k(h, k_bn_fwd, bnf, bnt, 0, h->stream, (const BnDesc*)(h->d_bn + f0), h->cfg.bn_eps, tf32);
  }
  launch_gemm(h, OP_G2, f0, nfl, 0);
  launch_gemm(h, op_g3, f0, nfl, 0);
}

void enqueue_disc_step(mrgan_handle* h, int f0, int nfl, int t, int from_stage) {
  const mrgan_config& c = h->cfg;
  const int B = c.batch;
  const bool heads = (heads_on(h) & 1) != 0;
  h->hp.t = t;
  launch_prep(h, f0, nfl, 0, from_stage, t, 2 * B);
  enqueue_gen_fwd(h, f0, nfl, OP_G3D);
  for (int l = 0; l < 6; ++l) launch_gemm(h, OP_D1 + l, f0, nfl, 0);
  if (!heads) {
    int lb = h->dp_losspart ? (3 * B + 511) / 512 : 1;
    lb = lb < 1 ? 1 : (lb > LOSS_MAX_BLOCKS ? LOSS_MAX_BLOCKS : lb);
    launch_k(h, k_loss_disc, dim3(lb, 1, nfl), dim3(256), 0, h->stream, (const LossDesc*)(h->d_loss + f0), h->d_step_stats, f0, h->nf, t, B,
             c.n_classes, c.unlabeled_weight, h->om, h->hp.dp_bg, h->dp_losspart, h->dp_lossctr);
  }
  const bool merge = tc_dw_merge(h);
  for (int l = 6; l >= 1; --l) {
    if (l >= 2) launch_gemm(h, OP_DX2 + l - 2, f0, nfl, 0);
    if (merge && l > 3) continue;
    fork_side(h);
    if (merge && l == 3) { tc_launch_dw_adam(h, OP_DW3, 4, f0, nfl, h->side); continue; }
    launch_gemm(h, OP_DW1 + l - 1, f0, nfl, 0, h->side);
  }
  join_side(h);
  if (h->dp_world > 1) dp_update(h, f0, nfl, 0);
  else if (!heads) launch_adam(h, f0, nfl, 0);
  if (from_stage) dp_allreduce(h, h->d_step_stats + ((size_t)t * h->nf + f0) * 4, (size_t)nfl * 4);
}

void enqueue_gen_step(mrgan_handle* h, int f0, int nfl, int t, int from_stage) {
  const mrgan_config& c = h->cfg;
  const int B = c.batch;
  const int hm = heads_on(h);
  h->hp.t = t;
  launch_prep(h, f0, nfl, 1, from_stage, t, 2 * B);
  enqueue_gen_fwd(h, f0, nfl, OP_G3G);
  for (int l = 0; l < 5; ++l) launch_gemm(h, OP_D1G + l, f0, nfl, 0);
  if (h->d_dpbufs) {
    const dim3 fmg((kDW[4] + BN_COLS - 1) / BN_COLS, split_chunks(B), nfl), fmt(B > 256 ? 1024 : 256);
    k_fm_stats<<<fmg, fmt, 0, h->stream>>>(h->d_loss + f0, h->d_dpbufs + f0, B);
    dp_allreduce(h, h->dp_fm + (size_t)f0 * 2 * kDW[4], (size_t)nfl * 2 * kDW[4]);
    k_fm_apply<<<fmg, fmt, 0, h->stream>>>(h->d_loss + f0, h->d_dpbufs + f0, h->d_step_stats, f0, h->nf, t, B,
                                           h->om, h->hp.dp_bg, h->dp_world, h->hp.alpha);
    h->launches += 2;
  } else if (!(hm & 2)) {
    launch_k(h, k_fm, dim3(1, 1, nfl), dim3(1024), 0, h->stream, (const LossDesc*)(h->d_loss + f0), h->d_step_stats, f0, h->nf, t, B,
             h->om, h->hp.alpha);
  }
  for (int l = 5; l >= 2; --l) launch_gemm(h, OP_DX2G + l - 2, f0, nfl, 0);
  launch_gemm(h, OP_DX1G, f0, nfl, 0);
  launch_gemm(h, OP_GX3, f0, nfl, 0);
  fork_side(h);
  launch_gemm(h, OP_GW3, f0, nfl, 0, h->side);
  launch_gemm(h, OP_GX2, f0, nfl, 0);
  const bool merge = tc_dw_merge(h);
  if (!merge) {
    fork_side(h);
    launch_gemm(h, OP_GW2, f0, nfl, 0, h->side);
  }
  const dim3 bng((kGH + BN_COLS - 1) / BN_COLS, h->d_dpbufs ? split_chunks(B) : 1, nfl), bnt(B > 256 ? 1024 : 256);
  if (h->d_dpbufs) {
    k_bn_bwd_stats<<<bng, bnt, 0, h->stream>>>(h->d_bn + f0, h->d_dpbufs + f0, h->om);
    dp_allreduce(h, h->dp_bnb + (size_t)f0 * 2 * kGH, (size_t)nfl * 2 * kGH);
    k_bn_bwd_apply<<<bng, bnt, 0, h->stream>>>(h->d_bn + f0, h->d_dpbufs + f0, h->om, h->hp.dp_bg);
    h->launches += 2;
  } else {
    launch_k(h, k_bn_bwd, bng, bnt, 0, h->stream, (const BnDesc*)(h->d_bn + f0), h->om);
  }
  fork_side(h);
  if (merge) tc_launch_dw_adam(h, OP_GW1, 2, f0, nfl, h->side);
  else launch_gemm(h, OP_GW1, f0, nfl, 0, h->side);
  join_side(h);
  if (h->dp_world > 1) dp_update(h, f0, nfl, 1);
  else launch_adam(h, f0, nfl, 1);
  dp_allreduce(h, h->d_step_stats + ((size_t)t * h->nf + f0) * 4, (size_t)nfl * 4);
}

void enqueue_nn_step(mrgan_handle* h, int f0, int nfl, int t, int from_stage, int n) {
  const mrgan_config& c = h->cfg;
  h->hp.t = t;
  launch_prep(h, f0, nfl, 2, from_stage, t, n);
  for (int l = 0; l < 6; ++l) launch_gemm(h, OP_D1 + l, f0, nfl, 0);
  launch_k(h, k_loss_mse, dim3(1, 1, nfl), dim3(256), 0, h->stream, (const LossDesc*)(h->d_loss + f0), h->d_step_stats, f0, h->nf, t, n, h->R,
           c.n_classes, h->om);
  for (int l = 6; l >= 1; --l) {
    if (l >= 2) launch_gemm(h, OP_DX2 + l - 2, f0, nfl, 0);
    fork_side(h);
    launch_gemm(h, OP_DW1 + l - 1, f0, nfl, 0, h->side);
  }
  join_side(h);
  launch_adam(h, f0, nfl, 0);
}

void enqueue_eval(mrgan_handle* h, int f0, int nfl, bool staged, int n_override, bool with_pred = false) {
  join_side(h);
  launch_gemm(h, staged ? OP_E1S : OP_E1, f0, nfl, n_override);
  for (int l = 1; l < 6; ++l) launch_gemm(h, OP_E2 + l - 1, f0, nfl, n_override);
  launch_k(h, k_argmax_err, dim3(1, 1, nfl), dim3(256), 0, h->stream, (const EvalDesc*)((staged ? h->d_eval_s : h->d_eval) + f0), n_override,
           h->cfg.n_classes, (int)with_pred);
}

void enqueue_confusion(mrgan_handle* h) {
  const int K = h->cfg.n_classes;
  int nmax = 1;
  for (int f = 0; f < h->nf; ++f) nmax = std::max(nmax, h->shapes[f].n_test);
  cudaMemsetAsync(h->d_conf, 0, (size_t)h->nf * K * K * sizeof(int), h->stream);
  launch_k(h, k_confusion, dim3((nmax + CONF_ROWS - 1) / CONF_ROWS, h->nf), dim3(256), 0, h->stream, (const EvalDesc*)h->d_eval, K, h->d_conf);
}

enum { TGT_PRED = 0, TGT_TEST = 1, TGT_STAGED = 2 };
void enqueue_input_grad(mrgan_handle* h, int f0, int nfl, bool staged, int n_override, int tgt) {
  enqueue_eval(h, f0, nfl, staged, n_override);
  int n = n_override;
  for (int f = f0; f < f0 + nfl && n_override <= 0; ++f) n = std::max(n, h->shapes[f].n_test);
  launch_k(h, k_logprob_seed, dim3((n + 255) / 256, 1, nfl), dim3(256), 0, h->stream,
           (const EvalDesc*)((tgt == TGT_STAGED ? h->d_eval_s : h->d_eval) + f0), n_override, h->cfg.n_classes, (int)(tgt == TGT_PRED), h->om);
  for (int l = 6; l >= 1; --l) launch_gemm(h, l >= 2 ? OP_EX2 + l - 2 : OP_EX1, f0, nfl, n_override);
  if (h->om.mode == 2)
    launch_k(h, k_unscale_grad, dim3(std::min((n * max_D(h, f0, nfl) + 255) / 256, 1184), 1, nfl), dim3(256), 0, h->stream,
             (const GemmDesc*)(h->sal.descs + (size_t)(OP_EX1 - NUM_OPS) * h->nf + f0), n_override, 1.0f / h->om.gscale);
}

void enqueue_saliency(mrgan_handle* h) {
  const int Dmax = max_D(h, 0, h->nf);
  enqueue_input_grad(h, 0, h->nf, false, 0, TGT_TEST);
  launch_k(h, k_saliency, dim3((Dmax + 127) / 128, h->nf), dim3(128), 0, h->stream,
           (const GemmDesc*)(h->sal.descs + (size_t)(OP_EX1 - NUM_OPS) * h->nf), (const EvalDesc*)h->d_eval, h->cfg.n_classes, Dmax, h->sal.profile);
}

int saliency_setup(mrgan_handle* h) {
  mrgan_handle::SalWork& S = h->sal;
  if (S.mem) return MRGAN_OK;
  const int nf = h->nf;
  const bool tc = h->cfg.precision != MRGAN_PREC_FP32;
  auto layout = [&](Arena& ar) {
    S.descs = ar.take<GemmDesc>((size_t)NUM_EX * nf);
    S.profile = ar.take<float>((size_t)nf * h->cfg.n_classes * max_D(h, 0, nf));
    S.tcops = tc ? ar.take<TcOp>((size_t)NUM_EX * nf) : nullptr;
  };
  Arena sizing;
  layout(sizing);
  char* mem = nullptr;
  CK(cudaMalloc(&mem, sizing.off + 256));
  Arena real; real.base = mem;
  layout(real);
  int rc = MRGAN_OK;
  if (cudaMemcpy(S.descs, h->h_descs.data() + (size_t)NUM_OPS * nf, (size_t)NUM_EX * nf * sizeof(GemmDesc), cudaMemcpyHostToDevice) != cudaSuccess)
    rc = fail(h, MRGAN_ERR_CUDA, "saliency workspace: descriptor upload failed");
  if (rc == MRGAN_OK && tc) rc = tc_ex_setup(h, S.tcops);
  if (rc != MRGAN_OK) { cudaFree(mem); return rc; }
  S.mem = mem;
  return MRGAN_OK;
}

int need_local(mrgan_handle* h, const char* fn) {
  if (h->dp_world > 1 || h->dp_virtual || h->nccl_comm) return fail(h, MRGAN_ERR_STATE, std::string(fn) + ": not available on a data-parallel handle");
  return MRGAN_OK;
}

int check_fold(mrgan_handle* h, int fold) {
  if (!h) return fail(nullptr, MRGAN_ERR_ARG, "null handle");
  if (fold < 0 || fold >= h->nf) return fail(h, MRGAN_ERR_ARG, "fold index out of range");
  return MRGAN_OK;
}

int need_nets(mrgan_handle* h, const char* fn) {
  if (!h) return fail(nullptr, MRGAN_ERR_ARG, "null handle");
  if (h->cfg.model == MRGAN_MODEL_SVM) return fail(h, MRGAN_ERR_STATE, std::string(fn) + ": not available on an SVM handle");
  return MRGAN_OK;
}

int finish_pending(mrgan_handle* h) {
  if (h->epoch_pending) {
    CK(cudaStreamSynchronize(h->stream));
    float ms = 0.f;
    CK(cudaEventElapsedTime(&ms, h->ev0, h->ev1));
    h->last_ms = ms;
    h->epoch_pending = false;
  }
  return MRGAN_OK;
}

void pack_params(const mrgan_handle* h, int fold, int net, const float* src, std::vector<float>& dst, bool to_internal,
                 float* out_ref) {
  const NetLayout& L = h->net[net][fold];
  long long o = 0;
  auto mat = [&](const TensorLayout& t, int rows_w) {
    for (int r = 0; r < rows_w + 1; ++r)
      for (int cidx = 0; cidx < t.cols; ++cidx) {
        const long long ii = t.off + (long long)r * t.pitch + cidx;
        if (to_internal) dst[ii] = src[o]; else out_ref[o] = dst[ii];
        ++o;
      }
  };
  auto vec = [&](const TensorLayout& t) {
    for (int cidx = 0; cidx < t.cols; ++cidx) {
      if (to_internal) dst[t.off + cidx] = src[o]; else out_ref[o] = dst[t.off + cidx];
      ++o;
    }
  };
  if (net == 0) {
    for (int l = 0; l < 6; ++l) mat(L.t[l], L.t[l].rows - 1);
  } else {
    mat(L.t[0], L.t[0].rows - 1); vec(L.t[1]); vec(L.t[2]); mat(L.t[3], L.t[3].rows - 1); mat(L.t[4], L.t[4].rows - 1);
  }
}

int build_graph(mrgan_handle* h, int key, int nb) {
  if (h->graphs.count(key)) return MRGAN_OK;
  const mrgan_config& c = h->cfg;
  const long long before = h->launches;
  cudaGraph_t g = nullptr;
  CK(cudaStreamBeginCapture(h->stream, cudaStreamCaptureModeThreadLocal));
  {
    cudaStream_t origin = h->stream, origin_side = h->side;
    const int nch = h->dp_world > 1 ? 1 : h->nchains;
    cudaEvent_t e = h->ev_pool[h->ev_next++ & 15];
    cudaEventRecord(e, origin);
    for (int ch = 1; ch < nch; ++ch) cudaStreamWaitEvent(h->cmain[ch], e, 0);
    for (int ch = 0; ch < nch; ++ch) {
      const int f0 = (int)((long long)h->nf * ch / nch), f1 = (int)((long long)h->nf * (ch + 1) / nch);
      if (f1 <= f0) continue;
      h->stream = h->cmain[ch]; h->side = h->cside[ch];
      h->side_open = false;
      if (c.model == MRGAN_MODEL_GAN) {
        for (int t = 0; t < nb; ++t) {
          enqueue_disc_step(h, f0, f1 - f0, t, 0);
          enqueue_gen_step(h, f0, f1 - f0, t, 0);
        }
        if (c.eval_each_epoch) enqueue_eval(h, f0, f1 - f0, false, 0);
        join_side(h);
      } else {
        for (int t = 0; t < nb; ++t) enqueue_nn_step(h, f0, f1 - f0, t, 0, c.batch);
        join_side(h);
      }
    }
    h->stream = origin; h->side = origin_side;
    for (int ch = 1; ch < nch; ++ch) {
      cudaEvent_t j = h->ev_pool[h->ev_next++ & 15];
      cudaEventRecord(j, h->cmain[ch]);
      cudaStreamWaitEvent(origin, j, 0);
    }
  }
  k_epoch_reduce<<<h->nf, 32, 0, h->stream>>>(h->d_step_stats, h->d_eval, h->d_epoch_stats, h->nf, nb,
                                              c.model == MRGAN_MODEL_GAN && c.eval_each_epoch);
  h->launches++;
  CK(cudaMemcpyAsync(h->h_epoch_stats, h->d_epoch_stats, (size_t)h->nf * 8 * sizeof(float), cudaMemcpyDeviceToHost, h->stream));
  CK(cudaStreamEndCapture(h->stream, &g));
  { const int sk = take_sticky(h); if (sk) { cudaGraphDestroy(g); return sk; } }
  cudaGraphExec_t ge = nullptr;
  CK(cudaGraphInstantiate(&ge, g, 0));
  CK(cudaGraphDestroy(g));
  h->graphs[key] = ge;
  h->graph_nodes[key] = h->launches - before;
  h->launches = before;
  return MRGAN_OK;
}

int upload_indices(mrgan_handle* h, const int32_t* const* streams, int n_streams, int n_idx) {
  const int slot = h->idx_slot;
  h->idx_slot ^= 1;
  CK(cudaEventSynchronize(h->idx_free[slot]));
  int* pin = h->h_idx_pinned[slot];
  for (int f = 0; f < h->nf; ++f)
    for (int s = 0; s < n_streams; ++s)
      memcpy(pin + ((size_t)f * 3 + s) * h->n_train, streams[s] + (size_t)f * n_idx, (size_t)n_idx * sizeof(int));
  for (int f = 0; f < h->nf; ++f)
    CK(cudaMemcpyAsync(h->fb[f].idx, pin + (size_t)f * 3 * h->n_train, (size_t)3 * h->n_train * sizeof(int),
                       cudaMemcpyHostToDevice, h->stream));
  CK(cudaEventRecord(h->idx_free[slot], h->stream));
  return MRGAN_OK;
}

}


namespace {

typedef CUresult (*EncodeTiledFn)(CUtensorMap*, CUtensorMapDataType, cuuint32_t, void*, const cuuint64_t*,
                                  const cuuint64_t*, const cuuint32_t*, const cuuint32_t*, CUtensorMapInterleave,
                                  CUtensorMapSwizzle, CUtensorMapL2promotion, CUtensorMapFloatOOBfill);

constexpr CUtensorMapL2promotion kL2Promo = CU_TENSOR_MAP_L2_PROMOTION_L2_256B;

bool make_map(EncodeTiledFn fn, CUtensorMap* m, const void* base, int cols, int rows, int pitch, int box_rows,
              bool mn_major, int box_cols = 0, int esz = 4) {
  const int row_elems = 128 / esz;
  if (box_cols == 0) box_cols = row_elems;
  cuuint64_t dims[2] = {(cuuint64_t)cols, (cuuint64_t)rows};
  cuuint64_t strides[1] = {(cuuint64_t)pitch * (cuuint64_t)esz};
  cuuint32_t box[2] = {(cuuint32_t)box_cols, (cuuint32_t)box_rows};
  cuuint32_t es[2] = {1u, 1u};
  return fn(m, esz == 2 ? CU_TENSOR_MAP_DATA_TYPE_FLOAT16 : CU_TENSOR_MAP_DATA_TYPE_FLOAT32, 2, const_cast<void*>(base), dims,
            strides, box, es, CU_TENSOR_MAP_INTERLEAVE_NONE,
            box_cols != row_elems ? CU_TENSOR_MAP_SWIZZLE_NONE
                                  : ((mn_major && esz == 4) ? CU_TENSOR_MAP_SWIZZLE_128B_ATOM_32B : CU_TENSOR_MAP_SWIZZLE_128B),
            kL2Promo,
            CU_TENSOR_MAP_FLOAT_OOB_FILL_NONE) == CUDA_SUCCESS;
}

int round_up(int x, int m) { return (x + m - 1) / m * m; }

#define TC_FWD_STAGES 4
#define TC_DW_STAGES 2
#define TC_FWD_THREADS (64 + 32 * 8)
#define TC_DW_THREADS (64 + 32 * 4)
#define K_TC_FWD(F, V) k_gemm_tc<true, false, TC_FWD_STAGES, 256, 1, 8, 1, F, V>
#define K_TC_FWD_N(F, V) k_gemm_tc<true, false, TC_FWD_STAGES, 512, 1, 8, 1, F, V>
#define K_TC_DX(F, V) k_gemm_tc<false, false, TC_FWD_STAGES, 256, 1, 8, 1, F, V>
#define K_TC_FWD2(F, V) k_gemm_tc<true, false, TC_FWD_STAGES, 512, 1, 8, 2, F, V>
#define K_TC_DX_N(F, V) k_gemm_tc<false, false, TC_FWD_STAGES, 512, 1, 8, 1, F, V>
#define K_TC_DX2(F, V) k_gemm_tc<false, false, TC_FWD_STAGES, 512, 1, 8, 2, F, V>
#define K_TC_DW(F, V) k_gemm_tc<true, true, TC_DW_STAGES, 128, 2, 4, 1, F, V>
#define TC_BIG_STAGES 3
#define K_TC_FWD_BIG(F, V) k_gemm_tc<true, false, TC_BIG_STAGES, 512, 1, 8, 2, F, V>
#define K_TC_DX_BIG(F, V) k_gemm_tc<false, false, TC_BIG_STAGES, 512, 1, 8, 2, F, V>
#define K_TC_DW_BIG(F, V) k_gemm_tc<true, true, TC_BIG_STAGES, 512, 1, 8, 2, F, V>
#define TC_LAUNCH(h, f16, K, grid, block, smem, st, ...)                          \
  do {                                                                            \
    const bool var_ = (h)->cfg.hidden_act != MRGAN_ACT_RELU || (h)->cfg.dropout > 0.0f;                \
    if (f16 && var_) launch_k(h, K(true, true), grid, block, smem, st, __VA_ARGS__);                   \
    else if (f16) launch_k(h, K(true, false), grid, block, smem, st, __VA_ARGS__);                     \
    else if (var_) launch_k(h, K(false, true), grid, block, smem, st, __VA_ARGS__);                    \
    else launch_k(h, K(false, false), grid, block, smem, st, __VA_ARGS__);                             \
  } while (0)
size_t tc_smem_bytes(int bn, int stages, int mt = 1) { return 1024 + (size_t)stages * ((size_t)mt * 128 * 128 + (size_t)bn * 128) + 256; }
bool tc_use_mt2(int maxME, int bn) { return maxME >= 500 && tc_smem_bytes(bn, TC_FWD_STAGES, 2) <= 227 * 1024; }

int tc_setup(mrgan_handle* h);

EncodeTiledFn tc_encoder() {
  EncodeTiledFn fn = nullptr;
  cudaDriverEntryPointQueryResult qres;
  if (cudaGetDriverEntryPoint("cuTensorMapEncodeTiled", (void**)&fn, cudaEnableDefault, &qres) != cudaSuccess ||
      qres != cudaDriverEntryPointSuccess) return nullptr;
  return fn;
}

template <bool F, bool V> void tc_set_smem_attr_fmt() {
  cudaFuncSetAttribute(K_TC_FWD(F, V), cudaFuncAttributeMaxDynamicSharedMemorySize, (int)tc_smem_bytes(256, TC_FWD_STAGES));
  cudaFuncSetAttribute(K_TC_FWD_N(F, V), cudaFuncAttributeMaxDynamicSharedMemorySize, (int)tc_smem_bytes(256, TC_FWD_STAGES));
  cudaFuncSetAttribute(K_TC_DX(F, V), cudaFuncAttributeMaxDynamicSharedMemorySize, (int)tc_smem_bytes(256, TC_FWD_STAGES));
  cudaFuncSetAttribute(K_TC_DX_N(F, V), cudaFuncAttributeMaxDynamicSharedMemorySize, (int)tc_smem_bytes(256, TC_FWD_STAGES));
  cudaFuncSetAttribute(K_TC_FWD_BIG(F, V), cudaFuncAttributeMaxDynamicSharedMemorySize, 227 * 1024);
  cudaFuncSetAttribute(K_TC_DX_BIG(F, V), cudaFuncAttributeMaxDynamicSharedMemorySize, 227 * 1024);
  cudaFuncSetAttribute(K_TC_DW_BIG(F, V), cudaFuncAttributeMaxDynamicSharedMemorySize, 227 * 1024);
  cudaFuncSetAttribute(K_TC_FWD2(F, V), cudaFuncAttributeMaxDynamicSharedMemorySize, 227 * 1024);
  cudaFuncSetAttribute(K_TC_DX2(F, V), cudaFuncAttributeMaxDynamicSharedMemorySize, 227 * 1024);
  cudaFuncSetAttribute(K_TC_DW(F, V), cudaFuncAttributeMaxDynamicSharedMemorySize, (int)tc_smem_bytes(128, TC_DW_STAGES));
  if (!V) cudaFuncSetAttribute(k_dw_adam_tc<F, (F ? 32 : 16)>, cudaFuncAttributeMaxDynamicSharedMemorySize, (int)TcAdamCfg<F, (F ? 32 : 16)>::SMEM);
}
void tc_set_smem_attr() {
  tc_set_smem_attr_fmt<false, false>(); tc_set_smem_attr_fmt<true, false>();
  tc_set_smem_attr_fmt<false, true>(); tc_set_smem_attr_fmt<true, true>();
}

void tc_pick_tile(int rows, int feats, int nf, int* bn, bool* mt1) {
  *bn = 256; *mt1 = false;
  auto tiles = [&](int b, bool one) { return ((feats + (one ? 127 : 255)) / (one ? 128 : 256)) * ((rows + b - 1) / b) * nf; };
  if (tiles(256, false) >= 120) return;
  *mt1 = true;
  for (int b : {256, 128, 64}) { *bn = b; if (tiles(b, true) >= 120) return; }
}

bool tc_fill_op(EncodeTiledFn fn, TcOp& t, const GemmDesc& g, int mode, int esz = 4, int bn_big = 256) {
  t.g = g;
  t.esz = esz;
  t.ME = g.N; t.NE = g.M; t.KE = g.K;
  const int kb = 128 / esz;
  if (mode == 0) {
    t.bn = g.M <= 256 ? round_up(g.M, 16) : bn_big;
    return make_map(fn, &t.mapA, g.B, g.N, g.K, g.ldb, kb, true, 0, esz) && make_map(fn, &t.mapB, g.A, g.K, g.M, g.lda, t.bn, false, 0, esz);
  }
  if (mode == 1) {
    t.bn = g.M <= 256 ? round_up(g.M, 16) : bn_big;
    return make_map(fn, &t.mapA, g.B, g.K, g.N, g.ldb, 128, false, 0, esz) && make_map(fn, &t.mapB, g.A, g.K, g.M, g.lda, t.bn, false, 0, esz);
  }
  t.bn = g.K > 512 ? 256 : 128;
  return make_map(fn, &t.mapA, g.B, g.N, g.K, g.ldb, kb, true, 0, esz) && make_map(fn, &t.mapB, g.A, g.M, g.K, g.lda, kb, true, 0, esz);
}

int tc_debug_gemm(mrgan_handle* h, int mode, const GemmDesc& g, int esz) {
  EncodeTiledFn fn = tc_encoder();
  if (!fn) return fail(h, MRGAN_ERR_CUDA, "cuTensorMapEncodeTiled not available from the driver");
  TcOp t; memset(&t, 0, sizeof(t));
  if (!tc_fill_op(fn, t, g, mode, esz)) return fail(h, MRGAN_ERR_CUDA, "cuTensorMapEncodeTiled failed");
  TcOp* d = nullptr;
  CK(cudaMalloc(&d, sizeof(TcOp)));
  CK(cudaMemcpyAsync(d, &t, sizeof(t), cudaMemcpyHostToDevice, h->stream));
  tc_set_smem_attr();
  dim3 grid((t.ME + 127) / 128, (t.NE + t.bn - 1) / t.bn, 1);
  const OperandMode om0{0, 1.0f, nullptr, nullptr};
  const bool f16 = esz == 2;
  if (mode == 0) TC_LAUNCH(h, f16, K_TC_FWD, grid, dim3(TC_FWD_THREADS), tc_smem_bytes(t.bn, TC_FWD_STAGES), h->stream, (const TcOp*)d, h->d_folds, 0, h->hp, om0);
  else if (mode == 1) TC_LAUNCH(h, f16, K_TC_DX, grid, dim3(TC_FWD_THREADS), tc_smem_bytes(t.bn, TC_FWD_STAGES), h->stream, (const TcOp*)d, h->d_folds, 0, h->hp, om0);
  else TC_LAUNCH(h, f16, K_TC_DW, grid, dim3(TC_DW_THREADS), tc_smem_bytes(t.bn, TC_DW_STAGES), h->stream, (const TcOp*)d, h->d_folds, 0, h->hp, om0);
  CK(cudaStreamSynchronize(h->stream));
  cudaFree(d);
  return MRGAN_OK;
}

int tc_make_op(mrgan_handle* h, EncodeTiledFn fn, int op, TcOp* ts) {
  const OpInfo& oi = h->ops[op];
  if (!oi.used) return MRGAN_OK;
  const int nf = h->nf;
  for (int f = 0; f < nf; ++f) {
    const GemmDesc& g = h->h_descs[(size_t)op * nf + f];
    TcOp& t = ts[f];
    const int mode = (!oi.at && !oi.bt) ? 0 : ((!oi.at && oi.bt) ? 1 : 2);
    int bn_big = 256;
    if (mode != 2 && oi.maxM > 256) { bool m1; tc_pick_tile(oi.maxM, oi.maxN, nf, &bn_big, &m1); h->tc_mt1[op] = m1; }
    if (h->om.mode == 2) {
      GemmDesc gh = g;
      gh.A = reinterpret_cast<const float*>(h->harena + (g.A - h->om.fbase));
      gh.B = reinterpret_cast<const float*>(h->harena + (g.B - h->om.fbase));
      if (!tc_fill_op(fn, t, gh, mode, 2, bn_big)) return fail(nullptr, MRGAN_ERR_CUDA, "cuTensorMapEncodeTiled (fp16 operands) failed");
      t.g = g;
    } else if (!tc_fill_op(fn, t, g, mode, 4, bn_big)) return fail(nullptr, MRGAN_ERR_CUDA, "cuTensorMapEncodeTiled failed");
    t.net = (op == OP_GW1 || op == OP_GW2 || op == OP_GW3) ? 1 : 0;
    if (h->tc_heads) {
      t.stats = h->d_step_stats + (size_t)f * 4;
      t.stats_stride = nf * 4;
      if (op == OP_D6 && (h->tc_heads & 1)) { t.head = HEAD_DISC; t.hd = h->d_loss + f; }
      else if (op == OP_D5G && (h->tc_heads & 2)) { t.head = HEAD_FM; t.hd = h->d_loss + f; }
      else if (op == OP_G1 && (h->tc_heads & 4)) { t.head = HEAD_BN; t.hd = h->d_bn + f; }
    }
    if (t.bn > h->tc_bn[op]) h->tc_bn[op] = t.bn;
    if (t.ME > h->tc_maxME[op]) h->tc_maxME[op] = t.ME;
    if (t.NE > h->tc_maxNE[op]) h->tc_maxNE[op] = t.NE;
  }
  return MRGAN_OK;
}

int tc_setup(mrgan_handle* h) {
  EncodeTiledFn fn = tc_encoder();
  if (!fn) return fail(nullptr, MRGAN_ERR_CUDA, "cuTensorMapEncodeTiled not available from the driver");
  if (h->R > 512) h->tc_fused_adam = false;
  const int nf = h->nf;
  h->tc_heads = (h->cfg.model == MRGAN_MODEL_GAN && h->tc_fused_adam && !h->d_dpbufs && h->R <= 256 && h->cfg.n_classes <= 32) ? 7 : 0;
  std::vector<TcOp> ops((size_t)NUM_OPS * nf);
  memset(ops.data(), 0, ops.size() * sizeof(TcOp));
  for (int op = 0; op < NUM_OPS; ++op) {
    const int rc = tc_make_op(h, fn, op, &ops[(size_t)op * nf]);
    if (rc != MRGAN_OK) return rc;
  }
  if (!h->tc_fused_adam) {
    size_t ws_floats = 0;
    for (int op = 0; op < NUM_OPS; ++op) {
      const OpInfo& oi = h->ops[op];
      if (!oi.used || !oi.at || h->tc_bn[op] != 256) continue;
      const int kblk = h->om.mode == 2 ? 64 : TC_KBLK;
      const int nkb = (ops[(size_t)op * nf].KE + kblk - 1) / kblk;
      const int tiles = ((h->tc_maxME[op] + 255) / 256) * ((h->tc_maxNE[op] + 255) / 256) * nf;
      int ks = std::min(std::min(2 * 148 / tiles, nkb / 8), 32);
      if (ks < 2) continue;
      const int per = (nkb + ks - 1) / ks;
      ks = (nkb + per - 1) / per;
      h->tc_ksplit[op] = ks;
      for (int f = 0; f < nf; ++f) {
        TcOp& t = ops[(size_t)op * nf + f];
        t.ws_stride = t.NE * t.g.ldc;
        t.ws = reinterpret_cast<float*>(ws_floats);
        ws_floats += (size_t)ks * t.ws_stride;
      }
    }
    if (ws_floats) {
      if (cudaMalloc(&h->d_tcws, ws_floats * sizeof(float)) != cudaSuccess) return fail(nullptr, MRGAN_ERR_CUDA, "cudaMalloc split-K workspace");
      cudaMemset(h->d_tcws, 0, ws_floats * sizeof(float));
      for (int op = 0; op < NUM_OPS; ++op)
        if (h->tc_ksplit[op] > 1)
          for (int f = 0; f < nf; ++f) {
            TcOp& t = ops[(size_t)op * nf + f];
            t.ws = h->d_tcws + reinterpret_cast<size_t>(t.ws);
          }
    }
  }
  if (cudaMalloc(&h->d_tcops, ops.size() * sizeof(TcOp)) != cudaSuccess) return fail(nullptr, MRGAN_ERR_CUDA, "cudaMalloc tc ops");
  if (cudaMemcpy(h->d_tcops, ops.data(), ops.size() * sizeof(TcOp), cudaMemcpyHostToDevice) != cudaSuccess) return fail(nullptr, MRGAN_ERR_CUDA, "cudaMemcpy tc ops");
  if (h->tc_fused_adam) {
    std::vector<TcAdamOp> aops((size_t)NUM_OPS * nf);
    memset(aops.data(), 0, aops.size() * sizeof(TcAdamOp));
    for (int op = 0; op < NUM_OPS; ++op) {
      const OpInfo& oi = h->ops[op];
      if (!oi.used || !oi.at) continue;
      for (int f = 0; f < nf; ++f) {
        const TcOp& t = ops[(size_t)op * nf + f];
        TcAdamOp& a = aops[(size_t)op * nf + f];
        const GemmDesc& g = t.g;
        a.ME = t.ME; a.NE = t.NE; a.KE = t.KE; a.fold = g.fold; a.net = t.net;
        bool ok;
        if (h->om.mode == 2) {
          const __half* hA = h->harena + (g.A - h->om.fbase);
          const __half* hB = h->harena + (g.B - h->om.fbase);
          ok = make_map(fn, &a.mapA, hB, g.N, g.K, g.ldb, 32, true, 0, 2) && make_map(fn, &a.mapB, hA, g.M, g.K, g.lda, 32, true, 0, 2);
        } else {
          ok = make_map(fn, &a.mapA, g.B, g.N, g.K, g.ldb, 16, true) && make_map(fn, &a.mapB, g.A, g.M, g.K, g.lda, 16, true);
        }
        if (!ok) return fail(nullptr, MRGAN_ERR_CUDA, "cuTensorMapEncodeTiled (dW operands) failed");
        a.ginv = h->om.mode == 2 ? 1.0f / h->om.gscale : 1.0f;
        const size_t off = (size_t)(g.C - h->Gr);
        float *P = h->P + off, *Mo = h->Mo + off, *Vo = h->Vo + off;
        if (h->om.mode == 2 && !make_map(fn, &a.mapH, h->harena + (P - h->om.fbase), t.ME, t.NE, g.ldc, TCA_KC, false, 128, 2))
          return fail(nullptr, MRGAN_ERR_CUDA, "cuTensorMapEncodeTiled (fp16 weight copy) failed");
        if (!make_map(fn, &a.mapP, P, t.ME, t.NE, g.ldc, TCA_KC, false, 128) ||
            !make_map(fn, &a.mapM, Mo, t.ME, t.NE, g.ldc, TCA_KC, false, 128) ||
            !make_map(fn, &a.mapV, Vo, t.ME, t.NE, g.ldc, TCA_KC, false, 128))
          return fail(nullptr, MRGAN_ERR_CUDA, "cuTensorMapEncodeTiled (optimizer state) failed");
      }
    }
    if (cudaMalloc(&h->d_tcadam, aops.size() * sizeof(TcAdamOp)) != cudaSuccess) return fail(nullptr, MRGAN_ERR_CUDA, "cudaMalloc tc adam ops");
    if (cudaMemcpy(h->d_tcadam, aops.data(), aops.size() * sizeof(TcAdamOp), cudaMemcpyHostToDevice) != cudaSuccess) return fail(nullptr, MRGAN_ERR_CUDA, "cudaMemcpy tc adam ops");
  }
  std::vector<AdamRange> r0(nf), r1(nf);
  for (int f = 0; f < nf; ++f) {
    r0[f] = AdamRange{h->net[0][f].off, 0};
    if (h->cfg.model == MRGAN_MODEL_GAN) {
      const NetLayout& LG = h->net[1][f];
      r1[f] = AdamRange{LG.off + LG.t[1].off, LG.t[3].off - LG.t[1].off};
    }
  }
  for (int n = 0; n < 2; ++n) {
    if (cudaMalloc(&h->d_ranges_tc[n], nf * sizeof(AdamRange)) != cudaSuccess) return fail(nullptr, MRGAN_ERR_CUDA, "cudaMalloc");
    if (cudaMemcpy(h->d_ranges_tc[n], (n == 0 ? r0 : r1).data(), nf * sizeof(AdamRange), cudaMemcpyHostToDevice) != cudaSuccess) return fail(nullptr, MRGAN_ERR_CUDA, "cudaMemcpy adam ranges");
  }
  tc_set_smem_attr();
  return MRGAN_OK;
}

int tc_ex_setup(mrgan_handle* h, TcOp* dst) {
  EncodeTiledFn fn = tc_encoder();
  if (!fn) return fail(h, MRGAN_ERR_CUDA, "cuTensorMapEncodeTiled not available from the driver");
  std::vector<TcOp> ops((size_t)NUM_EX * h->nf);
  memset(ops.data(), 0, ops.size() * sizeof(TcOp));
  for (int op = NUM_OPS; op < NUM_OPS_ALL; ++op) {
    const int rc = tc_make_op(h, fn, op, &ops[(size_t)(op - NUM_OPS) * h->nf]);
    if (rc != MRGAN_OK) return rc;
  }
  CK(cudaMemcpy(dst, ops.data(), ops.size() * sizeof(TcOp), cudaMemcpyHostToDevice));
  return MRGAN_OK;
}

void tc_teardown(mrgan_handle* h) {
  if (h->d_tcops) cudaFree(h->d_tcops);
  if (h->d_tcadam) cudaFree(h->d_tcadam);
  if (h->d_tcws) cudaFree(h->d_tcws);
  h->d_tcws = nullptr;
  for (int i = 0; i < NUM_OPS; ++i) h->tc_ksplit[i] = 0;
  for (int n = 0; n < 2; ++n) { if (h->d_ranges_tc[n]) cudaFree(h->d_ranges_tc[n]); h->d_ranges_tc[n] = nullptr; }
  for (int i = 0; i < NUM_OPS; ++i) { h->tc_bn[i] = 0; h->tc_maxME[i] = 0; h->tc_maxNE[i] = 0; h->tc_mt1[i] = false; }
  h->d_tcadam = nullptr;
  h->d_tcops = nullptr;
}

void tc_launch_dw_adam(mrgan_handle* h, int op, int nlayers, int f0, int nfl, cudaStream_t st) {
  const bool f16 = h->om.mode == 2;
  int gx = 0, gy = 0;
  for (int l = 0; l < nlayers; ++l) {
    gx = std::max(gx, (h->tc_maxME[op + l] + 127) / 128);
    gy = std::max(gy, (h->tc_maxNE[op + l] + 127) / 128);
  }
  const dim3 grid(gx, gy, nlayers * nfl);
  const TcAdamOp* ad = h->d_tcadam + (size_t)op * h->nf + f0;
  if (f16) launch_k(h, k_dw_adam_tc<true, 32>, grid, dim3(192), TcAdamCfg<true, 32>::SMEM, st, ad, h->d_folds, h->hp, nfl, h->nf);
  else launch_k(h, k_dw_adam_tc<false, 16>, grid, dim3(192), TcAdamCfg<false, 16>::SMEM, st, ad, h->d_folds, h->hp, nfl, h->nf);
}

bool tc_dw_merge(const mrgan_handle* h) { return h->cfg.precision != MRGAN_PREC_FP32 && h->d_tcadam != nullptr; }

bool tc_launch_gemm(mrgan_handle* h, int op, int f0, int nfl, int rows_override, cudaStream_t st) {
  const OpInfo& oi = h->ops[op];
  const bool f16 = h->om.mode == 2;
  const int bn = h->tc_bn[op];
  int NE = h->tc_maxNE[op];
  if (rows_override > 0 && !oi.at) NE = rows_override;
  dim3 grid((h->tc_maxME[op] + 127) / 128, (NE + bn - 1) / bn, nfl);
  const TcOp* d = (op < NUM_OPS ? h->d_tcops + (size_t)op * h->nf : h->sal.tcops + (size_t)(op - NUM_OPS) * h->nf) + f0;
  if (bn == 256 && (oi.at || h->tc_maxME[op] >= 500) && !h->tc_mt1[op]) {
    grid.x = (h->tc_maxME[op] + 255) / 256;
    const size_t smem = tc_smem_bytes(256, TC_BIG_STAGES, 2);
    if (oi.at) {
      const int ks = h->tc_ksplit[op] > 1 ? h->tc_ksplit[op] : 1;
      grid.z = nfl * ks;
      TC_LAUNCH(h, f16, K_TC_DW_BIG, grid, dim3(TC_FWD_THREADS), smem, st, d, h->d_folds, ks, h->hp, h->om);
      if (ks > 1) {
        const int n4 = h->tc_maxNE[op] * pitch8(h->tc_maxME[op]) / 4;
        launch_k(h, k_splitk_reduce, dim3(std::min((n4 + 255) / 256, 1184), nfl, 1), dim3(256), 0, st, d, ks);
      }
    } else if (!oi.bt) TC_LAUNCH(h, f16, K_TC_FWD_BIG, grid, dim3(TC_FWD_THREADS), smem, st, d, h->d_folds, rows_override, h->hp, h->om);
    else TC_LAUNCH(h, f16, K_TC_DX_BIG, grid, dim3(TC_FWD_THREADS), smem, st, d, h->d_folds, rows_override, h->hp, h->om);
    return true;
  }
  const bool head_mt2 = (h->tc_heads & 2) && op == OP_D5G;
  if (!oi.at && !h->tc_mt1[op] && (tc_use_mt2(h->tc_maxME[op], bn) || head_mt2)) {
    grid.x = (h->tc_maxME[op] + 255) / 256;
    const size_t smem = tc_smem_bytes(bn, TC_FWD_STAGES, 2);
    if (!oi.bt) TC_LAUNCH(h, f16, K_TC_FWD2, grid, dim3(TC_FWD_THREADS), smem, st, d, h->d_folds, rows_override, h->hp, h->om);
    else TC_LAUNCH(h, f16, K_TC_DX2, grid, dim3(TC_FWD_THREADS), smem, st, d, h->d_folds, rows_override, h->hp, h->om);
    return true;
  }
  if (!oi.at && !oi.bt) {
    if (2 * tc_smem_bytes(bn, TC_FWD_STAGES) > 227 * 1024)
      TC_LAUNCH(h, f16, K_TC_FWD_N, grid, dim3(TC_FWD_THREADS), tc_smem_bytes(bn, TC_FWD_STAGES), st, d, h->d_folds, rows_override, h->hp, h->om);
    else
      TC_LAUNCH(h, f16, K_TC_FWD, grid, dim3(TC_FWD_THREADS), tc_smem_bytes(bn, TC_FWD_STAGES), st, d, h->d_folds, rows_override, h->hp, h->om);
  }
  else if (!oi.at && oi.bt) {
    if (2 * tc_smem_bytes(bn, TC_FWD_STAGES) > 227 * 1024)
      TC_LAUNCH(h, f16, K_TC_DX_N, grid, dim3(TC_FWD_THREADS), tc_smem_bytes(bn, TC_FWD_STAGES), st, d, h->d_folds, rows_override, h->hp, h->om);
    else
      TC_LAUNCH(h, f16, K_TC_DX, grid, dim3(TC_FWD_THREADS), tc_smem_bytes(bn, TC_FWD_STAGES), st, d, h->d_folds, rows_override, h->hp, h->om);
  }
  else if (h->d_tcadam) { tc_launch_dw_adam(h, op, 1, f0, nfl, st); return true; }
  else TC_LAUNCH(h, f16, K_TC_DW, grid, dim3(TC_DW_THREADS), tc_smem_bytes(bn, TC_DW_STAGES), st, d, h->d_folds, 0, h->hp, h->om);
  return true;
}

}

extern "C" {

const char* mrgan_version(void) { return "mrgan-b200 0.2 (sm_100a)"; }

int mrgan_abi_info(int out[4]) {
  if (!out) return fail(nullptr, MRGAN_ERR_ARG, "abi_info: null pointer");
  out[0] = MRGAN_ABI_VERSION; out[1] = (int)sizeof(mrgan_config); out[2] = (int)sizeof(mrgan_fold_shape); out[3] = (int)sizeof(mrgan_epoch_stats);
  return MRGAN_OK;
}

int mrgan_default_config(int model, mrgan_config* cfg) {
  if (!cfg) return fail(nullptr, MRGAN_ERR_ARG, "cfg is null");
  memset(cfg, 0, sizeof(*cfg));
  cfg->model = model;
  cfg->n_folds = 1;
  cfg->n_classes = 6;
  cfg->noise_dim = 100;
  cfg->precision = MRGAN_PREC_FP32;
  cfg->shared_t = 1;
  cfg->eval_each_epoch = 1;
  cfg->device = 0;
  cfg->beta2 = 0.999f; cfg->adam_eps = 1e-8f; cfg->bn_eps = 2e-5f;
  cfg->unlabeled_weight = 1.0f; cfg->sigma_in = 0.3f; cfg->sigma_hidden = 0.5f;
  cfg->hidden_act = MRGAN_ACT_RELU; cfg->leaky_alpha = 0.3f; cfg->dropout = 0.0f;
  if (model == MRGAN_MODEL_NN) { cfg->batch = 20; cfg->lr = 1e-3f; cfg->beta1 = 0.9f; }
  else { cfg->batch = 50; cfg->lr = 6e-4f; cfg->beta1 = 0.5f; }
  return MRGAN_OK;
}

const char* mrgan_last_error(const mrgan_handle* h) { return h ? h->err.c_str() : g_last_error.c_str(); }

int mrgan_create(const mrgan_config* cfg, const mrgan_fold_shape* folds, mrgan_handle** out) {
  mrgan_handle* h = nullptr;
  if (!cfg || !folds || !out) return fail(nullptr, MRGAN_ERR_ARG, "null argument");
  *out = nullptr;
  if (cfg->n_folds < 1 || cfg->batch < 1 || cfg->n_classes < 2 || cfg->n_classes > 64 || cfg->noise_dim < 1)
    return fail(nullptr, MRGAN_ERR_ARG, "bad config (n_folds/batch/n_classes/noise_dim)");
  if (cfg->model != MRGAN_MODEL_GAN && cfg->model != MRGAN_MODEL_NN && cfg->model != MRGAN_MODEL_SVM) return fail(nullptr, MRGAN_ERR_ARG, "bad model");
  if (cfg->model == MRGAN_MODEL_SVM && cfg->precision != MRGAN_PREC_FP32)
    return fail(nullptr, MRGAN_ERR_ARG, "bad config: the SVM has one arithmetic path (precision must be MRGAN_PREC_FP32)");
  if (cfg->batch > (1 << 16)) return fail(nullptr, MRGAN_ERR_ARG, "batch too large");
  if ((cfg->hidden_act != MRGAN_ACT_RELU && cfg->hidden_act != MRGAN_ACT_LEAKY_RELU) || !(cfg->dropout >= 0.0f && cfg->dropout < 1.0f))
    return fail(nullptr, MRGAN_ERR_ARG, "bad config (hidden_act / dropout)");
  for (int f = 0; f < cfg->n_folds; ++f) {
    if (folds[f].D < 1 || folds[f].n_train < cfg->batch || folds[f].n_test < 1)
      return fail(nullptr, MRGAN_ERR_ARG, "bad fold shape");
    if (folds[f].n_train != folds[0].n_train)
      return fail(nullptr, MRGAN_ERR_ARG, "all folds of a handle must have the same n_train");
  }
  int ndev = 0;
  if (cudaGetDeviceCount(&ndev) != cudaSuccess || ndev == 0 || cfg->device >= ndev)
    return fail(nullptr, MRGAN_ERR_NO_DEVICE, "no CUDA device: this library has no CPU fallback");
  cudaDeviceProp prop;
  if (cudaGetDeviceProperties(&prop, cfg->device) != cudaSuccess || prop.major != 10 || prop.minor != 0)
    return fail(nullptr, MRGAN_ERR_NO_DEVICE, "device is not sm_100 (B200): the library holds sm_100a code only and has no CPU fallback");
  if (cfg->precision < MRGAN_PREC_FP32 || cfg->precision > MRGAN_PREC_F16) return fail(nullptr, MRGAN_ERR_ARG, "bad config (precision)");
  h = new mrgan_handle();
  h->cfg = *cfg;
  h->nf = cfg->n_folds;
  h->R = cfg->model == MRGAN_MODEL_GAN ? 3 * cfg->batch : cfg->batch;
  h->n_train = folds[0].n_train;
  h->shapes.assign(folds, folds + h->nf);
  h->fb.resize(h->nf);
  h->hp = AdamHyper{cfg->lr, cfg->beta1, cfg->beta2, cfg->adam_eps, cfg->shared_t, cfg->batch, cfg->batch, 0,
                    cfg->unlabeled_weight, cfg->bn_eps, cfg->n_classes, 0,
                    cfg->hidden_act == MRGAN_ACT_LEAKY_RELU ? cfg->leaky_alpha : 0.0f, cfg->dropout, 1.0f / (1.0f - cfg->dropout)};
  int ne = h->R;
  for (int f = 0; f < h->nf; ++f) ne = folds[f].n_test > ne ? folds[f].n_test : ne;
  h->NE = ne;
  auto cleanup = [&](int code) { mrgan_destroy(h); return code; };
  if (cudaSetDevice(cfg->device) != cudaSuccess) return cleanup(fail(nullptr, MRGAN_ERR_CUDA, "cudaSetDevice failed"));
  long long off = 0;
  for (int n = 0; n < (cfg->model == MRGAN_MODEL_GAN ? 2 : (cfg->model == MRGAN_MODEL_NN ? 1 : 0)); ++n) {
    h->net[n].resize(h->nf);
    for (int f = 0; f < h->nf; ++f) {
      NetLayout L = n == 0 ? layout_disc(folds[f].D, cfg->n_classes) : layout_gen(folds[f].D, cfg->noise_dim);
      L.off = off;
      off += L.n;
      h->net[n][f] = L;
    }
  }
  h->n_flat = off;
  Arena sizing;
  layout_buffers(h, sizing);
  h->arena_bytes = sizing.off + 256;
  cudaError_t e = cudaMalloc(&h->arena, h->arena_bytes);
  if (e != cudaSuccess) return cleanup(fail(nullptr, MRGAN_ERR_CUDA, std::string("cudaMalloc arena: ") + cudaGetErrorString(e)));
  e = cudaMemset(h->arena, 0, h->arena_bytes);
  if (e == cudaSuccess) e = cudaDeviceSynchronize();
  if (e != cudaSuccess) return cleanup(fail(nullptr, MRGAN_ERR_CUDA, std::string("cudaMemset: ") + cudaGetErrorString(e)));
  Arena real; real.base = h->arena;
  layout_buffers(h, real);
  h->om = OperandMode{cfg->precision, 1.0f, reinterpret_cast<const float*>(h->arena), nullptr};
  if (cfg->precision == MRGAN_PREC_F16) {
    e = cudaMalloc(&h->harena, h->arena_bytes / 2);
    if (e == cudaSuccess) e = cudaMemset(h->harena, 0, h->arena_bytes / 2);
    if (e == cudaSuccess) e = cudaDeviceSynchronize();
    if (e != cudaSuccess) return cleanup(fail(nullptr, MRGAN_ERR_CUDA, std::string("cudaMalloc fp16 operand arena: ") + cudaGetErrorString(e)));
    h->om.hbase = h->harena;
    h->om.gscale = MRGAN_F16_LOSS_SCALE;
    if (const char* ls = getenv("MRGAN_LOSS_SCALE")) { const float v = (float)atof(ls); if (v >= 1.0f) h->om.gscale = v; }
  }
  bool ok = cudaStreamCreateWithFlags(&h->stream, cudaStreamNonBlocking) == cudaSuccess;
  ok = ok && cudaStreamCreateWithFlags(&h->side, cudaStreamNonBlocking) == cudaSuccess;
  for (int i = 0; i < 16 && ok; ++i) ok = cudaEventCreateWithFlags(&h->ev_pool[i], cudaEventDisableTiming) == cudaSuccess;
  {
    const char* env = getenv("MRGAN_CHAINS");
    int nch = env ? atoi(env) : (h->nf >= 32 ? 4 : (h->nf >= 8 ? 2 : 1));
    if (nch < 1) nch = 1;
    if (nch > kMaxChains) nch = kMaxChains;
    if (nch > h->nf) nch = h->nf;
    h->nchains = nch;
    h->cmain[0] = h->stream; h->cside[0] = h->side;
    for (int ch = 1; ch < nch && ok; ++ch) {
      ok = cudaStreamCreateWithFlags(&h->cmain[ch], cudaStreamNonBlocking) == cudaSuccess &&
           cudaStreamCreateWithFlags(&h->cside[ch], cudaStreamNonBlocking) == cudaSuccess;
    }
  }
  ok = ok && cudaEventCreate(&h->ev0) == cudaSuccess && cudaEventCreate(&h->ev1) == cudaSuccess;
  ok = ok && cudaMallocHost(&h->h_epoch_stats, (size_t)h->nf * 8 * sizeof(float)) == cudaSuccess;
  ok = ok && cudaMallocHost(&h->h_scratch, 64 * sizeof(float)) == cudaSuccess;
  for (int s = 0; s < 2 && ok; ++s) {
    ok = ok && cudaMallocHost(&h->h_idx_pinned[s], (size_t)h->nf * 3 * h->n_train * sizeof(int)) == cudaSuccess;
    ok = ok && cudaEventCreateWithFlags(&h->idx_free[s], cudaEventDisableTiming) == cudaSuccess;
  }
  if (!ok) return cleanup(fail(nullptr, MRGAN_ERR_CUDA, "stream/event/pinned allocation failed"));
  if (cfg->model != MRGAN_MODEL_SVM) {
    const int rc = build_descs(h); if (rc != MRGAN_OK) return cleanup(rc);
    init_ones(h);
  } else {
    std::vector<EvalDesc> ev(h->nf);
    for (int f = 0; f < h->nf; ++f) ev[f] = EvalDesc{nullptr, 0, h->fb[f].yte, folds[f].n_test, 0, nullptr, h->fb[f].pred};
    if (cudaMemcpy(h->d_eval, ev.data(), h->nf * sizeof(EvalDesc), cudaMemcpyHostToDevice) != cudaSuccess)
      return cleanup(fail(nullptr, MRGAN_ERR_CUDA, "create: descriptor upload failed"));
  }
  if (cfg->model == MRGAN_MODEL_GAN && cfg->batch > 256) {
    int rc = alloc_split_bufs(h);
    if (rc != MRGAN_OK) return cleanup(rc);
  }
  if (cfg->precision != MRGAN_PREC_FP32) {
    int rc = tc_setup(h);
    if (rc != MRGAN_OK) return cleanup(rc);
  }
  e = cudaStreamSynchronize(h->stream);
  if (e == cudaSuccess) e = cudaGetLastError();
  if (e != cudaSuccess) return cleanup(fail(nullptr, MRGAN_ERR_CUDA, std::string("create: ") + cudaGetErrorString(e)));
  *out = h;
  return MRGAN_OK;
}

int mrgan_destroy(mrgan_handle* h) {
  if (!h) return MRGAN_OK;
  cudaSetDevice(h->cfg.device);
  if (h->stream) cudaStreamSynchronize(h->stream);
  for (auto& kv : h->graphs) cudaGraphExecDestroy(kv.second);
  for (auto& ds : h->datasets) { if (ds.x) cudaFree(ds.x); if (ds.y) cudaFree(ds.y); }
  if (h->d_prep_stats) cudaFree(h->d_prep_stats);
  if (h->d_prep_rows) cudaFree(h->d_prep_rows);
  if (h->nccl_comm && g_nccl.CommDestroy) g_nccl.CommDestroy(h->nccl_comm);
  if (!h->dp_virtual)
    for (int p = 0; p < DP_MAX_RANKS; ++p) {
      if (h->peer_arena[p] && h->peer_arena[p] != h->arena) cudaIpcCloseMemHandle(h->peer_arena[p]);
      if (h->peer_harena[p] && h->peer_harena[p] != h->harena) cudaIpcCloseMemHandle(h->peer_harena[p]);
    }
  if (h->d_dpmem) cudaFree(h->d_dpmem);
  if (h->d_dpbufs) cudaFree(h->d_dpbufs);
  if (h->sal.mem) cudaFree(h->sal.mem);
  tc_teardown(h);
  if (h->svm.mem) cudaFree(h->svm.mem);
  if (h->svm.cv_mem) cudaFree(h->svm.cv_mem);
  if (h->arena) cudaFree(h->arena);
  if (h->harena) cudaFree(h->harena);
  if (h->h_epoch_stats) cudaFreeHost(h->h_epoch_stats);
  if (h->h_scratch) cudaFreeHost(h->h_scratch);
  for (int s = 0; s < 2; ++s) {
    if (h->h_idx_pinned[s]) cudaFreeHost(h->h_idx_pinned[s]);
    if (h->idx_free[s]) cudaEventDestroy(h->idx_free[s]);
  }
  if (h->ev0) cudaEventDestroy(h->ev0);
  if (h->ev1) cudaEventDestroy(h->ev1);
  for (int i = 0; i < 16; ++i) if (h->ev_pool[i]) cudaEventDestroy(h->ev_pool[i]);
  for (int ch = 1; ch < kMaxChains; ++ch) { if (h->cmain[ch]) cudaStreamDestroy(h->cmain[ch]); if (h->cside[ch]) cudaStreamDestroy(h->cside[ch]); }
  if (h->side) cudaStreamDestroy(h->side);
  if (h->stream) cudaStreamDestroy(h->stream);
  delete h;
  return MRGAN_OK;
}

int mrgan_sync(mrgan_handle* h) {
  if (!h) return fail(nullptr, MRGAN_ERR_ARG, "null handle");
  CK(cudaSetDevice(h->cfg.device));
  int rc = finish_pending(h);
  if (rc) return rc;
  CK(cudaStreamSynchronize(h->stream));
  return MRGAN_OK;
}

int64_t mrgan_num_params(const mrgan_handle* h, int fold, int net) {
  if (!h || fold < 0 || fold >= h->nf || net < 0 || net > 1 || h->net[net].empty()) return -1;
  return h->net[net][fold].n_ref;
}

int mrgan_set_params(mrgan_handle* h, int fold, int net, const float* src, int64_t n) {
  int rc = check_fold(h, fold); if (rc) return rc; rc = need_nets(h, "set_params"); if (rc) return rc;
  if (net < 0 || net > 1 || h->net[net].empty()) return fail(h, MRGAN_ERR_ARG, "no such net in this model");
  const NetLayout& L = h->net[net][fold];
  if (!src || n != L.n_ref) return fail(h, MRGAN_ERR_ARG, "set_params: length does not match mrgan_num_params");
  CK(cudaSetDevice(h->cfg.device));
  rc = finish_pending(h); if (rc) return rc;
  std::vector<float> buf((size_t)L.n, 0.f);
  pack_params(h, fold, net, src, buf, true, nullptr);
  CK(cudaMemcpyAsync(h->P + L.off, buf.data(), (size_t)L.n * sizeof(float), cudaMemcpyHostToDevice, h->stream));
  if (h->om.mode == 2) {
    k_to_half<<<256, 256, 0, h->stream>>>(h->P + L.off, (size_t)L.n, h->om);
    h->launches++;
  }
  CK(cudaStreamSynchronize(h->stream));
  return MRGAN_OK;
}

static int get_flat(mrgan_handle* h, int fold, int net, const float* dev, float* dst, int64_t n) {
  const NetLayout& L = h->net[net][fold];
  if (!dst || n != L.n_ref) return fail(h, MRGAN_ERR_ARG, "length does not match mrgan_num_params");
  std::vector<float> buf((size_t)L.n);
  CK(cudaMemcpyAsync(buf.data(), dev + L.off, (size_t)L.n * sizeof(float), cudaMemcpyDeviceToHost, h->stream));
  CK(cudaStreamSynchronize(h->stream));
  pack_params(h, fold, net, nullptr, buf, false, dst);
  return MRGAN_OK;
}

int mrgan_get_params(mrgan_handle* h, int fold, int net, float* dst, int64_t n) {
  int rc = check_fold(h, fold); if (rc) return rc; rc = need_nets(h, "get_params"); if (rc) return rc;
  if (net < 0 || net > 1 || h->net[net].empty()) return fail(h, MRGAN_ERR_ARG, "no such net in this model");
  CK(cudaSetDevice(h->cfg.device));
  rc = finish_pending(h); if (rc) return rc;
  return get_flat(h, fold, net, h->P, dst, n);
}

int mrgan_get_adam(mrgan_handle* h, int fold, int net, float* m, float* v, int64_t n) {
  int rc = check_fold(h, fold); if (rc) return rc; rc = need_nets(h, "get_adam"); if (rc) return rc;
  if (net < 0 || net > 1 || h->net[net].empty()) return fail(h, MRGAN_ERR_ARG, "no such net in this model");
  CK(cudaSetDevice(h->cfg.device));
  rc = finish_pending(h); if (rc) return rc;
  rc = get_flat(h, fold, net, h->Mo, m, n); if (rc) return rc;
  return get_flat(h, fold, net, h->Vo, v, n);
}

int mrgan_get_counters(mrgan_handle* h, int fold, int* iterations, int* rng_step) {
  int rc = check_fold(h, fold); if (rc) return rc; rc = need_nets(h, "get_counters"); if (rc) return rc;
  CK(cudaSetDevice(h->cfg.device));
  rc = finish_pending(h); if (rc) return rc;
  FoldState fs;
// ... 1238 lines not shown
```

Before: 44030.

## Fuse discriminator tail layers, loss head and early backward into one persistent kernel

Adds a k_tail_tc kernel that runs one CTA per fold through the last discriminator forward layers, the loss head (disc or feature-matching), and the first backward dx layers. Successive layers are chained inside the kernel with an mbarrier handoff. This removes many small per-layer GEMM launches and the separate loss kernels when at least 8 folds are processed. The dx and fwd epilogues are pulled out into shared helpers so both kernels can use them. The fused kernel gives each fold a single CTA, which may leave SMs idle and serialises layers that were previously parallel across tiles.

```diff
diff --git a/mr_gan_b200/csrc/kernels_tc.cuh b/mr_gan_b200/csrc/kernels_tc.cuh
--- a/mr_gan_b200/csrc/kernels_tc.cuh
+++ b/mr_gan_b200/csrc/kernels_tc.cuh
@@ -24,7 +24,7 @@
 
 #ifdef MRGAN_PHASE_TIMING
 __device__ __forceinline__ unsigned long long gtimer() { unsigned long long t; asm volatile("mov.u64 %0, %globaltimer;" : "=l"(t)); return t; }
-#define PT_MARK(i) do { pt[i] = gtimer(); } while (0)
+#define PT_MARK(i) do { if (pt) pt[i] = gtimer(); } while (0)
 #else
 #define PT_MARK(i) do { } while (0)
 #endif
@@ -341,6 +341,212 @@
   }
 }
 
+template <int EPW>
+__device__ __forceinline__ void head_publish(const TcOp& op, FoldState* folds, const AdamHyper& hp, const float* part, const float* red) {
+  float* const st = op.stats + (size_t)hp.t * op.stats_stride;
+  if (op.head == HEAD_DISC) {
+    const float Bg = (float)hp.dp_bg;
+    float a0 = 0.f, a1 = 0.f, a2 = 0.f;
+    for (int w = 0; w < EPW; ++w) { a0 += part[3 * w]; a1 += part[3 * w + 1]; a2 += part[3 * w + 2]; }
+    st[0] = a0 / Bg; st[1] = a1 / Bg; st[2] = a2 / Bg;
+    FoldState& fs = folds[op.g.fold];
+    if (hp.shared_t) fs.iterations += 1; else fs.it_net[0] += 1;
+    fs.rng_step += 1;
+  } else {
+    float sum = 0.f;
+    for (int w = 0; w < EPW; ++w) sum += red[w];
+    st[3] = sum / static_cast<const LossDesc*>(op.hd)->Wmid;
+  }
+}
+
+
+template <bool F16, bool VAR, bool AUX_NC>
+__device__ __forceinline__ void epi_dx(const GemmDesc& g, const AdamHyper& hp, const OperandMode& om, int n0, int cbeg, int ncols, int nchunks,
+                                       int npark, int f, bool f_ok, uint32_t trow, uint32_t tfree, uint64_t* tmem_full, uint32_t parity) {
+  using namespace tc;
+  const bool has_act = g.act != ACT_NONE;
+  const bool drop = VAR && hp.drop > 0.f && (g.act == ACT_RELU || g.act == ACT_LEAKY) && g.tid >= 1;
+  const __half* const haux = (F16 && drop) ? om.hbase + (g.aux - om.fbase) : nullptr;
+  auto fetch = [&](int c0, float (&av)[16]) {
+#pragma unroll
+    for (int j = 0; j < 16; ++j) {
+      const size_t o = (size_t)(n0 + c0 + j) * g.ldaux + f;
+      av[j] = (f_ok && has_act && c0 + j < ncols) ? (haux ? __half2float(haux[o]) : (AUX_NC ? __ldg(g.aux + o) : __ldcg(g.aux + o))) : 1.0f;
+    }
+  };
+  float avA[16], avB[16];
+  const int npk = has_act ? npark : 0;
+  if (npk > 0) {
+    fetch(cbeg, avA);
+    for (int k = 0; k < npk; k += 2) {
+      if (k + 1 < npk) fetch(cbeg + 16 * (k + 1), avB);
+      tmem_st16(tfree + 16u * (uint32_t)k, avA);
+      if (k + 1 < npk) {
+        if (k + 2 < npk) fetch(cbeg + 16 * (k + 2), avA);
+        tmem_st16(tfree + 16u * (uint32_t)(k + 1), avB);
+      }
+    }
+    tmem_wait_st();
+  }
+  if (has_act && npk < nchunks) fetch(cbeg + 16 * npk, avA);
+  mbar_wait(tmem_full, parity);
+  fence_after();
+  __half* const hC = F16 ? om.hbase + (g.C - om.fbase) : nullptr;
+  const bool op_only = (g.rnd & 1) != 0;
+  for (int ch = 0; ch < nchunks; ++ch) {
+    const int c0 = cbeg + 16 * ch;
+    uint32_t va[16], vh[16];
+    tmem_ld16_issue(trow + (uint32_t)c0, va);
+    if (ch < npk) tmem_ld16_issue(tfree + 16u * (uint32_t)ch, vh);
+    tmem_wait_ld();
+    tmem_fence16(va);
+    float av[16];
+    if (ch < npk) {
+      tmem_fence16(vh);
+#pragma unroll
+      for (int j = 0; j < 16; ++j) av[j] = __uint_as_float(vh[j]);
+    } else if (has_act) {
+      const bool odd = ((ch - npk) & 1) != 0;
+#pragma unroll
+      for (int j = 0; j < 16; ++j) av[j] = odd ? avB[j] : avA[j];
+      if (ch + 1 < nchunks) { if (odd) fetch(c0 + 16, avA); else fetch(c0 + 16, avB); }
+    } else {
+#pragma unroll
+      for (int j = 0; j < 16; ++j) av[j] = 1.0f;
+    }
+    if (!f_ok) continue;
+    const size_t o0 = (size_t)(n0 + c0) * g.ldc + f;
+    const int nrows = ncols - c0;
+    float* const pC = g.C + o0;
+    __half* const phC = F16 ? hC + o0 : nullptr;
+    const float dinv = drop ? hp.drop_inv : 1.0f;
+#define DX_ACT(FULL)                                                                                                        \
+    do {                                                                                                                    \
+      if (g.act == ACT_RELU) dx_rows<F16, ACT_RELU, FULL>(va, av, nrows, pC, phC, g.ldc, op_only, 0.f, dinv, drop);         \
+      else if (VAR && g.act == ACT_LEAKY) dx_rows<F16, ACT_LEAKY, FULL>(va, av, nrows, pC, phC, g.ldc, op_only, hp.alpha, dinv, drop); \
+      else if (g.act == ACT_SOFTPLUS) dx_rows<F16, ACT_SOFTPLUS, FULL>(va, av, nrows, pC, phC, g.ldc, op_only, 0.f, 1.0f, false);      \
+      else dx_rows<F16, ACT_NONE, FULL>(va, av, nrows, pC, phC, g.ldc, op_only, 0.f, 1.0f, false);                          \
+    } while (0)
+    if (nrows >= 16) DX_ACT(true); else DX_ACT(false);
+#undef DX_ACT
+  }
+}
+
+template <bool F16, bool VAR>
+__device__ __forceinline__ void epi_fwd(const GemmDesc& g, const FoldState* folds, const AdamHyper& hp, const OperandMode& om, int n0, int cbeg,
+                                        int ncols, int nchunks, int npark, int f, bool f_ok, int wg, uint32_t trow, uint32_t tfree,
+                                        uint64_t* tmem_full, uint32_t parity, unsigned long long* pt) {
+  using namespace tc;
+  const int warp = threadIdx.x >> 5, lane = threadIdx.x & 31;
+  const bool mul = VAR && hp.drop > 0.f && g.C2 != nullptr && g.tid >= 1;
+  const float ddrop = mul ? hp.drop : 0.f;
+  const bool noisy = g.C2 != nullptr && (g.sigma != 0.f || mul);
+  uint32_t key0 = 0, key1 = 0, step = 0;
+  if (noisy) { const FoldState& fs = folds[g.fold]; key0 = fs.key0; key1 = fs.key1; step = (uint32_t)fs.rng_step; }
+  const bool grp = ((g.row0 + n0 + cbeg) & 3) == 0 && (hp.dp_bg == hp.dp_bloc || (hp.dp_bloc & 3) == 0);
+  const bool dp = hp.dp_bg != hp.dp_bloc;
+  const int dprank = hp.dp_rank < 0 ? g.fold : hp.dp_rank;
+  auto draw16 = [&](int c0, float (&nz)[16]) {
+    const int r0 = g.row0 + n0 + c0;
+    if (grp && !dp) {
+#pragma unroll
+      for (int q = 0; q < 4; ++q) {
+        if (VAR) noise_or_drop4(key0, key1, (uint32_t)(r0 + 4 * q) >> 2, (uint32_t)f, step, (uint32_t)g.tid, ddrop, hp.drop_inv, &nz[4 * q]);
+        else normal4(key0, key1, (uint32_t)(r0 + 4 * q) >> 2, (uint32_t)f, step, (uint32_t)g.tid, &nz[4 * q]);
+      }
+    } else if (grp) {
+#pragma unroll
+      for (int q = 0; q < 4; ++q) {
+        const float4 n4 = noise4_call(key0, key1, r0 + 4 * q, (uint32_t)f, step, (uint32_t)g.tid, hp.dp_bloc, hp.dp_bg, dprank, ddrop, hp.drop_inv);
+        nz[4 * q] = n4.x; nz[4 * q + 1] = n4.y; nz[4 * q + 2] = n4.z; nz[4 * q + 3] = n4.w;
+      }
+    } else {
+#pragma unroll
+      for (int j = 0; j < 16; ++j)
+        nz[j] = noise1_call(key0, key1, r0 + j, (uint32_t)f, step, (uint32_t)g.tid, hp.dp_bloc, hp.dp_bg, dprank, ddrop, hp.drop_inv);
+    }
+  };
+  const int npk = (noisy && grp) ? npark : 0;
+  for (int ch = 0; ch < npk; ++ch) {
+    float nz[16];
+    draw16(cbeg + 16 * ch, nz);
+    tmem_st16(tfree + 16u * (uint32_t)ch, nz);
+  }
+  if (npk > 0) tmem_wait_st();
+  if (warp == 2 && lane == 0) PT_MARK(4);
+  mbar_wait(tmem_full, parity);
+  if (warp == 2 && lane == 0) PT_MARK(5);
+  fence_after();
+  __half* const hC = (F16 && g.C) ? om.hbase + (g.C - om.fbase) : nullptr;
+  __half* const hC2 = (F16 && g.C2) ? om.hbase + (g.C2 - om.fbase) : nullptr;
+  const bool c_op = (g.rnd & 1) != 0, c2_op = (g.rnd & 2) != 0;
+#ifdef MRGAN_PHASE_TIMING
+  unsigned long long tch[24];
+#endif
+  for (int it = 0; it < nchunks; ++it) {
+    const int ch = (wg & 1) ? nchunks - 1 - it : it;
+    const int c0 = cbeg + 16 * ch;
+    uint32_t va[16], vn[16];
+    float nz[16];
+#ifdef MRGAN_PHASE_TIMING
+    if (ch < 12) tch[2 * ch] = gtimer();
+#endif
+    tmem_ld16_issue(trow + (uint32_t)c0, va);
+    if (ch < npk) tmem_ld16_issue(tfree + 16u * (uint32_t)ch, vn);
+    else if (noisy) draw16(c0, nz);
+    tmem_wait_ld();
+#ifdef MRGAN_PHASE_TIMING
+    if (ch < 12) tch[2 * ch + 1] = gtimer();
+#endif
+    tmem_fence16(va);
+    if (ch < npk) {
+      tmem_fence16(vn);
+#pragma unroll
+      for (int j = 0; j < 16; ++j) nz[j] = __uint_as_float(vn[j]);
+    }
+    if (!f_ok) continue;
+    const size_t o0 = (size_t)(n0 + c0) * g.ldc + f, o20 = (size_t)(n0 + c0) * g.ldc2 + f;
+    const int nrows = ncols - c0;
+    float* const pC = g.C ? g.C + o0 : nullptr;
+    float* const pC2 = g.C2 ? g.C2 + o20 : nullptr;
+    __half* const phC = hC ? hC + o0 : nullptr;
+    __half* const phC2 = hC2 ? hC2 + o20 : nullptr;
+    if (!noisy) {
+#pragma unroll
+      for (int j = 0; j < 16; ++j) nz[j] = 0.f;
+    }
+#define FWD_ROWS(ACT, HC, HC2, FULL) \
+    fwd_rows<F16, ACT, HC, HC2, FULL>(va, nz, nrows, pC, phC, g.ldc, c_op, pC2, phC2, g.ldc2, c2_op, g.sigma, hp.alpha, VAR && mul)
+#define FWD_ACT(HC, HC2, FULL)                                                     \
+    do {                                                                       \
+      if (g.act == ACT_RELU) FWD_ROWS(ACT_RELU, HC, HC2, FULL);                \
+      else if (g.act == ACT_SOFTPLUS) FWD_ROWS(ACT_SOFTPLUS, HC, HC2, FULL);   \
+      else if (VAR && g.act == ACT_LEAKY) FWD_ROWS(ACT_LEAKY, HC, HC2, FULL);  \
+      else FWD_ROWS(ACT_NONE, HC, HC2, FULL);                                  \
+    } while (0)
+#define FWD_OUT(FULL)                                                              \
+    do {                                                                       \
+      if (g.C && g.C2) FWD_ACT(true, true, FULL);                              \
+      else if (g.C) FWD_ACT(true, false, FULL);                                \
+      else if (g.C2) FWD_ACT(false, true, FULL);                               \
+    } while (0)
+    if (nrows >= 16) FWD_OUT(true); else FWD_OUT(false);
+#undef FWD_OUT
+#undef FWD_ACT
+#undef FWD_ROWS
+  }
+#ifdef MRGAN_PHASE_TIMING
+  if (pt && warp == 2 && lane == 0 && blockIdx.x == 0 && blockIdx.z == 0 && nchunks >= 10) {
+    const unsigned long long te2 = gtimer();
+    const unsigned long long b = pt[0];
+    printf("PTCH npk=%d: %llu+%llu %llu+%llu %llu+%llu %llu+%llu %llu+%llu %llu+%llu %llu+%llu %llu+%llu %llu+%llu %llu+%llu end=%llu\n", npk,
+           tch[0] - b, tch[1] - tch[0], tch[2] - b, tch[3] - tch[2], tch[4] - b, tch[5] - tch[4], tch[6] - b, tch[7] - tch[6], tch[8] - b, tch[9] - tch[8],
+           tch[10] - b, tch[11] - tch[10], tch[12] - b, tch[13] - tch[12], tch[14] - b, tch[15] - tch[14], tch[16] - b, tch[17] - tch[16],
+           tch[18] - b, tch[19] - tch[18], te2 - b);
+  }
+#endif
+}
+
 template <bool A_MN, bool B_MN, int STAGES, int TMEM_COLS, int MINB, int EPW, int MT, bool F16, bool VAR>
 __global__ void __launch_bounds__(64 + 32 * EPW, MINB)
 k_gemm_tc(const TcOp* __restrict__ ops, FoldState* __restrict__ folds, int rows_override, AdamHyper hp, OperandMode om) {
@@ -368,8 +574,9 @@
   uint64_t* tmem_full = bars + 2 * STAGES;
   uint32_t* tmem_holder = reinterpret_cast<uint32_t*>(bars + 2 * STAGES + 1);
   float* const red = reinterpret_cast<float*>(bars + 24);
+  unsigned long long* pt = nullptr;
 #ifdef MRGAN_PHASE_TIMING
-  unsigned long long* pt = reinterpret_cast<unsigned long long*>(bars + 16);
+  pt = reinterpret_cast<unsigned long long*>(bars + 16);
   if (threadIdx.x == 0) pt[0] = pt_t0;
 #endif
 
@@ -487,180 +694,9 @@
         }
       }
     } else if constexpr (!A_MN) {
-      const bool has_act = g.act != ACT_NONE;
-      const bool drop = VAR && hp.drop > 0.f && (g.act == ACT_RELU || g.act == ACT_LEAKY) && g.tid >= 1;
-      const __half* const haux = (F16 && drop) ? om.hbase + (g.aux - om.fbase) : nullptr;
-      auto fetch = [&](int c0, float (&av)[16]) {
-#pragma unroll
-        for (int j = 0; j < 16; ++j) {
-          const size_t o = (size_t)(n0 + c0 + j) * g.ldaux + f;
-          av[j] = (f_ok && has_act && c0 + j < ncols) ? (haux ? __half2float(haux[o]) : __ldg(g.aux + o)) : 1.0f;
-        }
-      };
-      float avA[16], avB[16];
-      const int npk = has_act ? npark : 0;
-      if (npk > 0) {
-        fetch(cbeg, avA);
-        for (int k = 0; k < npk; k += 2) {
-          if (k + 1 < npk) fetch(cbeg + 16 * (k + 1), avB);
-          tmem_st16(tfree + 16u * (uint32_t)k, avA);
-          if (k + 1 < npk) {
-            if (k + 2 < npk) fetch(cbeg + 16 * (k + 2), avA);
-            tmem_st16(tfree + 16u * (uint32_t)(k + 1), avB);
-          }
-        }
-        tmem_wait_st();
-      }
-      if (has_act && npk < nchunks) fetch(cbeg + 16 * npk, avA);
-      mbar_wait(tmem_full, 0);
-      fence_after();
-      __half* const hC = F16 ? om.hbase + (g.C - om.fbase) : nullptr;
-      const bool op_only = (g.rnd & 1) != 0;
-      for (int ch = 0; ch < nchunks; ++ch) {
-        const int c0 = cbeg + 16 * ch;
-        uint32_t va[16], vh[16];
-        tmem_ld16_issue(trow + (uint32_t)c0, va);
-        if (ch < npk) tmem_ld16_issue(tfree + 16u * (uint32_t)ch, vh);
-        tmem_wait_ld();
-        tmem_fence16(va);
-        float av[16];
-        if (ch < npk) {
-          tmem_fence16(vh);
-#pragma unroll
-          for (int j = 0; j < 16; ++j) av[j] = __uint_as_float(vh[j]);
-        } else if (has_act) {
-          const bool odd = ((ch - npk) & 1) != 0;
-#pragma unroll
-          for (int j = 0; j < 16; ++j) av[j] = odd ? avB[j] : avA[j];
-          if (ch + 1 < nchunks) { if (odd) fetch(c0 + 16, avA); else fetch(c0 + 16, avB); }
-        } else {
-#pragma unroll
-          for (int j = 0; j < 16; ++j) av[j] = 1.0f;
-        }
-        if (!f_ok) continue;
-        const size_t o0 = (size_t)(n0 + c0) * g.ldc + f;
-        const int nrows = ncols - c0;
-        float* const pC = g.C + o0;
-        __half* const phC = F16 ? hC + o0 : nullptr;
-        const float dinv = drop ? hp.drop_inv : 1.0f;
-#define DX_ACT(FULL)                                                                                                        \
-        do {                                                                                                                    \
-          if (g.act == ACT_RELU) dx_rows<F16, ACT_RELU, FULL>(va, av, nrows, pC, phC, g.ldc, op_only, 0.f, dinv, drop);         \
-          else if (VAR && g.act == ACT_LEAKY) dx_rows<F16, ACT_LEAKY, FULL>(va, av, nrows, pC, phC, g.ldc, op_only, hp.alpha, dinv, drop); \
-          else if (g.act == ACT_SOFTPLUS) dx_rows<F16, ACT_SOFTPLUS, FULL>(va, av, nrows, pC, phC, g.ldc, op_only, 0.f, 1.0f, false);      \
-          else dx_rows<F16, ACT_NONE, FULL>(va, av, nrows, pC, phC, g.ldc, op_only, 0.f, 1.0f, false);                          \
-        } while (0)
-        if (nrows >= 16) DX_ACT(true); else DX_ACT(false);
-#undef DX_ACT
-      }
+      epi_dx<F16, VAR, true>(g, hp, om, n0, cbeg, ncols, nchunks, npark, f, f_ok, trow, tfree, tmem_full, 0);
     } else {
-      const bool mul = VAR && hp.drop > 0.f && g.C2 != nullptr && g.tid >= 1;
-      const float ddrop = mul ? hp.drop : 0.f;
-      const bool noisy = g.C2 != nullptr && (g.sigma != 0.f || mul);
-      uint32_t key0 = 0, key1 = 0, step = 0;
-      if (noisy) { const FoldState& fs = folds[g.fold]; key0 = fs.key0; key1 = fs.key1; step = (uint32_t)fs.rng_step; }
-      const bool grp = ((g.row0 + n0 + cbeg) & 3) == 0 && (hp.dp_bg == hp.dp_bloc || (hp.dp_bloc & 3) == 0);
-      const bool dp = hp.dp_bg != hp.dp_bloc;
-      const int dprank = hp.dp_rank < 0 ? g.fold : hp.dp_rank;
-      auto draw16 = [&](int c0, float (&nz)[16]) {
-        const int r0 = g.row0 + n0 + c0;
-        if (grp && !dp) {
-#pragma unroll
-          for (int q = 0; q < 4; ++q) {
-            if (VAR) noise_or_drop4(key0, key1, (uint32_t)(r0 + 4 * q) >> 2, (uint32_t)f, step, (uint32_t)g.tid, ddrop, hp.drop_inv, &nz[4 * q]);
-            else normal4(key0, key1, (uint32_t)(r0 + 4 * q) >> 2, (uint32_t)f, step, (uint32_t)g.tid, &nz[4 * q]);
-          }
-        } else if (grp) {
-#pragma unroll
-          for (int q = 0; q < 4; ++q) {
-            const float4 n4 = noise4_call(key0, key1, r0 + 4 * q, (uint32_t)f, step, (uint32_t)g.tid, hp.dp_bloc, hp.dp_bg, dprank, ddrop, hp.drop_inv);
-            nz[4 * q] = n4.x; nz[4 * q + 1] = n4.y; nz[4 * q + 2] = n4.z; nz[4 * q + 3] = n4.w;
-          }
-        } else {
-#pragma unroll
-          for (int j = 0; j < 16; ++j)
-            nz[j] = noise1_call(key0, key1, r0 + j, (uint32_t)f, step, (uint32_t)g.tid, hp.dp_bloc, hp.dp_bg, dprank, ddrop, hp.drop_inv);
-        }
-      };
-      const int npk = (noisy && grp) ? npark : 0;
-      for (int ch = 0; ch < npk; ++ch) {
-        float nz[16];
-        draw16(cbeg + 16 * ch, nz);
-        tmem_st16(tfree + 16u * (uint32_t)ch, nz);
-      }
-      if (npk > 0) tmem_wait_st();
-      if (warp == 2 && lane == 0) PT_MARK(4);
-      mbar_wait(tmem_full, 0);
-      if (warp == 2 && lane == 0) PT_MARK(5);
-      fence_after();
-      __half* const hC = (F16 && g.C) ? om.hbase + (g.C - om.fbase) : nullptr;
-      __half* const hC2 = (F16 && g.C2) ? om.hbase + (g.C2 - om.fbase) : nullptr;
-      const bool c_op = (g.rnd & 1) != 0, c2_op = (g.rnd & 2) != 0;
-#ifdef MRGAN_PHASE_TIMING
-      unsigned long long tch[24];
-#endif
-      for (int it = 0; it < nchunks; ++it) {
-        const int ch = (wg & 1) ? nchunks - 1 - it : it;
-        const int c0 = cbeg + 16 * ch;
-        uint32_t va[16], vn[16];
-        float nz[16];
-#ifdef MRGAN_PHASE_TIMING
-        if (ch < 12) tch[2 * ch] = gtimer();
-#endif
-        tmem_ld16_issue(trow + (uint32_t)c0, va);
-        if (ch < npk) tmem_ld16_issue(tfree + 16u * (uint32_t)ch, vn);
-        else if (noisy) draw16(c0, nz);
-        tmem_wait_ld();
-#ifdef MRGAN_PHASE_TIMING
-        if (ch < 12) tch[2 * ch + 1] = gtimer();
-#endif
-        tmem_fence16(va);
-        if (ch < npk) {
-          tmem_fence16(vn);
-#pragma unroll
-          for (int j = 0; j < 16; ++j) nz[j] = __uint_as_float(vn[j]);
-        }
-        if (!f_ok) continue;
-        const size_t o0 = (size_t)(n0 + c0) * g.ldc + f, o20 = (size_t)(n0 + c0) * g.ldc2 + f;
-        const int nrows = ncols - c0;
-        float* const pC = g.C ? g.C + o0 : nullptr;
-        float* const pC2 = g.C2 ? g.C2 + o20 : nullptr;
-        __half* const phC = hC ? hC + o0 : nullptr;
-        __half* const phC2 = hC2 ? hC2 + o20 : nullptr;
-        if (!noisy) {
-#pragma unroll
-          for (int j = 0; j < 16; ++j) nz[j] = 0.f;
-        }
-#define FWD_ROWS(ACT, HC, HC2, FULL) \
-        fwd_rows<F16, ACT, HC, HC2, FULL>(va, nz, nrows, pC, phC, g.ldc, c_op, pC2, phC2, g.ldc2, c2_op, g.sigma, hp.alpha, VAR && mul)
-#define FWD_ACT(HC, HC2, FULL)                                                     \
-        do {                                                                       \
-          if (g.act == ACT_RELU) FWD_ROWS(ACT_RELU, HC, HC2, FULL);                \
-          else if (g.act == ACT_SOFTPLUS) FWD_ROWS(ACT_SOFTPLUS, HC, HC2, FULL);   \
-          else if (VAR && g.act == ACT_LEAKY) FWD_ROWS(ACT_LEAKY, HC, HC2, FULL);  \
-          else FWD_ROWS(ACT_NONE, HC, HC2, FULL);                                  \
-        } while (0)
-#define FWD_OUT(FULL)                                                              \
-        do {                                                                       \
-          if (g.C && g.C2) FWD_ACT(true, true, FULL);                              \
-          else if (g.C) FWD_ACT(true, false, FULL);                                \
-          else if (g.C2) FWD_ACT(false, true, FULL);                               \
-        } while (0)
-        if (nrows >= 16) FWD_OUT(true); else FWD_OUT(false);
-#undef FWD_OUT
-#undef FWD_ACT
-#undef FWD_ROWS
-      }
-#ifdef MRGAN_PHASE_TIMING
-      if (warp == 2 && lane == 0 && blockIdx.x == 0 && blockIdx.z == 0 && nchunks >= 10) {
-        const unsigned long long te2 = gtimer();
-        const unsigned long long b = pt[0];
-        printf("PTCH npk=%d: %llu+%llu %llu+%llu %llu+%llu %llu+%llu %llu+%llu %llu+%llu %llu+%llu %llu+%llu %llu+%llu %llu+%llu end=%llu\n", npk,
-               tch[0] - b, tch[1] - tch[0], tch[2] - b, tch[3] - tch[2], tch[4] - b, tch[5] - tch[4], tch[6] - b, tch[7] - tch[6], tch[8] - b, tch[9] - tch[8],
-               tch[10] - b, tch[11] - tch[10], tch[12] - b, tch[13] - tch[12], tch[14] - b, tch[15] - tch[14], tch[16] - b, tch[17] - tch[16],
-               tch[18] - b, tch[19] - tch[18], te2 - b);
-      }
-#endif
+      epi_fwd<F16, VAR>(g, folds, hp, om, n0, cbeg, ncols, nchunks, npark, f, f_ok, wg, trow, tfree, tmem_full, 0, pt);
       if (op.head == HEAD_DISC) {
         float* const sl = reinterpret_cast<float*>(smem);
         head_disc<F16, EPW>(trow, cbeg, ncols, min(bn, NE - n0), lane_base, lane, warp - 2, *static_cast<const LossDesc*>(op.hd), hp, om,
@@ -680,23 +716,8 @@
     fence_after();
     asm volatile("tcgen05.dealloc.cta_group::1.sync.aligned.b32 %0, %1;" ::"r"(tmem_base), "r"((uint32_t)TMEM_COLS) : "memory");
   }
-  if (!B_MN && A_MN && threadIdx.x == 0 && (op.head == HEAD_DISC || op.head == HEAD_FM)) {
-    float* const st = op.stats + (size_t)hp.t * op.stats_stride;
-    if (op.head == HEAD_DISC) {
-      const float Bg = (float)hp.dp_bg;
-      const float* part = reinterpret_cast<const float*>(smem) + 8192;
-      float a0 = 0.f, a1 = 0.f, a2 = 0.f;
-      for (int w = 0; w < EPW; ++w) { a0 += part[3 * w]; a1 += part[3 * w + 1]; a2 += part[3 * w + 2]; }
-      st[0] = a0 / Bg; st[1] = a1 / Bg; st[2] = a2 / Bg;
-      FoldState& fs = folds[op.g.fold];
-      if (hp.shared_t) fs.iterations += 1; else fs.it_net[0] += 1;
-      fs.rng_step += 1;
-    } else {
-      float sum = 0.f;
-      for (int w = 0; w < EPW; ++w) sum += red[w];
-      st[3] = sum / static_cast<const LossDesc*>(op.hd)->Wmid;
-    }
-  }
+  if (!B_MN && A_MN && threadIdx.x == 0 && (op.head == HEAD_DISC || op.head == HEAD_FM))
+    head_publish<EPW>(op, folds, hp, reinterpret_cast<const float*>(smem) + 8192, red);
 #ifdef MRGAN_PHASE_TIMING
   if (threadIdx.x == 0 && blockIdx.x == 0 && blockIdx.y == 0 && (blockIdx.z % 24) == 0) {
     const unsigned long long te = gtimer();
@@ -914,3 +935,174 @@
     asm volatile("tcgen05.dealloc.cta_group::1.sync.aligned.b32 %0, %1;" ::"r"(tmem_base), "r"(128u) : "memory");
   }
 }
+
+#define TAIL_MAX_STAGES 4
+struct TailPlan { int fwd0, nfwd, dx0, ndx; };
+
+namespace tc {
+__device__ __forceinline__ void fence_proxy_async_global() { asm volatile("fence.proxy.async.global;" ::: "memory"); }
+}
+
+template <bool F16, bool VAR>
+__global__ void __launch_bounds__(64 + 32 * 8, 1)
+k_tail_tc(const TcOp* __restrict__ ops, int nf, TailPlan plan, FoldState* __restrict__ folds, AdamHyper hp, OperandMode om, int stages,
+          uint32_t stage_bytes) {
+  using namespace tc;
+  constexpr int EPW = 8;
+  constexpr int KBLK = F16 ? 64 : 32;
+  constexpr uint32_t MN_BOX = F16 ? 8192u : 4096u;
+  constexpr uint32_t A_BYTES = 2 * 128 * 128;
+  const int nl = plan.nfwd + plan.ndx;
+  auto layer = [&](int l) -> const TcOp& {
+    return ops[(size_t)(l < plan.nfwd ? plan.fwd0 + l : plan.dx0 - (l - plan.nfwd)) * nf + blockIdx.x];
+  };
+
+  extern __shared__ uint8_t smem_raw[];
+  uint8_t* const base = reinterpret_cast<uint8_t*>((reinterpret_cast<uintptr_t>(smem_raw) + 1023) & ~(uintptr_t)1023);
+  uint8_t* const smem = base + 1024;
+  uint64_t* bars = reinterpret_cast<uint64_t*>(base);
+  uint64_t* full = bars;
+  uint64_t* empty = bars + TAIL_MAX_STAGES;
+  uint64_t* tmem_full = bars + 2 * TAIL_MAX_STAGES;
+  uint64_t* act_ready = tmem_full + 1;
+  uint32_t* tmem_holder = reinterpret_cast<uint32_t*>(act_ready + 1);
+  float* const red = reinterpret_cast<float*>(bars + 16);
+  float* const part = reinterpret_cast<float*>(bars + 32);
+  float* const sl = reinterpret_cast<float*>(smem + (size_t)stages * stage_bytes);
+
+  const int warp = threadIdx.x >> 5, lane = threadIdx.x & 31;
+  if (warp == 0 && lane == 0) {
+    for (int l = 0; l < nl; ++l) { prefetch_map(&layer(l).mapA); prefetch_map(&layer(l).mapB); }
+    for (int s = 0; s < TAIL_MAX_STAGES; ++s) { mbar_init(&full[s], 1); mbar_init(&empty[s], 1); }
+    mbar_init(tmem_full, 1);
+    mbar_init(act_ready, 1);
+    asm volatile("fence.mbarrier_init.release.cluster;" ::: "memory");
+  }
+  if (warp == 1) {
+    asm volatile("tcgen05.alloc.cta_group::1.sync.aligned.shared::cta.b32 [%0], %1;" ::"r"(smem_u32(tmem_holder)), "r"(512u) : "memory");
+    asm volatile("tcgen05.relinquish_alloc_permit.cta_group::1.sync.aligned;" ::: "memory");
+  }
+  fence_before();
+  __syncthreads();
+  fence_after();
+  const uint32_t tmem_base = *tmem_holder;
+
+  if (warp == 0) {
+    if (lane == 0) {
+      int it = 0;
+      for (int l = 0; l < nl; ++l) {
+        const TcOp& op = layer(l);
+        const bool dx = l >= plan.nfwd;
+        const int nmt = op.ME > 128 ? 2 : 1;
+        const int nkb = (op.KE + KBLK - 1) / KBLK;
+        const uint32_t bytes = (uint32_t)nmt * 16384u + (uint32_t)op.bn * 128u;
+        auto load_w = [&](int kb) {
+          uint8_t* sa = smem + (size_t)((it + kb) % stages) * stage_bytes;
+          uint64_t* fb = &full[(it + kb) % stages];
+          if (!dx) {
+            for (int b = 0; b < (128 / KBLK) * nmt; ++b) tma_load_2d(&op.mapA, fb, sa + b * MN_BOX, KBLK * b, kb * KBLK);
+          } else {
+            for (int mt = 0; mt < nmt; ++mt) tma_load_2d(&op.mapA, fb, sa + mt * 16384, kb * KBLK, 128 * mt);
+          }
+        };
+        auto load_act = [&](int kb) {
+          uint8_t* sa = smem + (size_t)((it + kb) % stages) * stage_bytes;
+          tma_load_2d(&op.mapB, &full[(it + kb) % stages], sa + A_BYTES, kb * KBLK, 0);
+        };
+        auto claim = [&](int kb) {
+          const int s = (it + kb) % stages;
+          mbar_wait(&empty[s], ((uint32_t)((it + kb) / stages) & 1u) ^ 1u);
+          mbar_expect_tx(&full[s], bytes);
+        };
+        const int npre = min(nkb, stages);
+        for (int kb = 0; kb < npre; ++kb) { claim(kb); load_w(kb); }
+        if (l > 0) mbar_wait(act_ready, (uint32_t)(l - 1) & 1u);
+        for (int kb = 0; kb < npre; ++kb) load_act(kb);
+        for (int kb = npre; kb < nkb; ++kb) { claim(kb); load_w(kb); load_act(kb); }
+        it += nkb;
+      }
+    }
+  } else if (warp == 1) {
+    if (lane == 0) {
+      constexpr uint32_t fmt = F16 ? 0u : 2u;
+      constexpr uint32_t mn_lbo = MN_BOX, mn_sbo = F16 ? 1024u : 512u, mn_lay = F16 ? 2u : 1u, mn_step = F16 ? 2048u : 1024u;
+      int it = 0;
+      for (int l = 0; l < nl; ++l) {
+        const TcOp& op = layer(l);
+        const bool amn = l < plan.nfwd;
+        const int nmt = op.ME > 128 ? 2 : 1;
+        const int nkb = (op.KE + KBLK - 1) / KBLK;
+        const uint32_t idesc = (1u << 4) | (fmt << 7) | (fmt << 10) | ((amn ? 1u : 0u) << 15) | ((uint32_t)(op.bn >> 3) << 17) |
+                               ((128u >> 4) << 24);
+        const uint32_t lboA = amn ? mn_lbo : 16u, sboA = amn ? mn_sbo : 1024u, layA = amn ? mn_lay : 2u, stepA = amn ? mn_step : 32u;
+        if (l > 0) mbar_wait(act_ready, (uint32_t)(l - 1) & 1u);
+        for (int kb = 0; kb < nkb; ++kb) {
+          const int s = (it + kb) % stages;
+          mbar_wait(&full[s], (uint32_t)((it + kb) / stages) & 1u);
+          fence_after();
+          const uint32_t sa = smem_u32(smem + (size_t)s * stage_bytes), sb = sa + A_BYTES;
+#pragma unroll
+          for (int k = 0; k < 4; ++k) {
+            const uint64_t db = smem_desc(sb + k * 32u, 16u, 1024u, 2u);
+            for (int mt = 0; mt < nmt; ++mt) {
+              const uint64_t da = smem_desc(sa + mt * 16384u + k * stepA, lboA, sboA, layA);
+              if (F16) mma_f16(tmem_base + 256u * mt, da, db, idesc, (kb > 0 || k > 0) ? 1u : 0u);
+              else mma_tf32(tmem_base + 256u * mt, da, db, idesc, (kb > 0 || k > 0) ? 1u : 0u);
+            }
+          }
+          mma_commit(&empty[s]);
+        }
+        mma_commit(tmem_full);
+        it += nkb;
+      }
+    }
+  } else {
+#define TAIL_COORDS                                                                                                          \
+    const int wg = (warp - 2) >> 2, lane_base = 32 * (warp & 3), f = 128 * wg + lane_base + lane;                           \
+    const uint32_t trow = *tmem_holder + 256u * wg + ((uint32_t)lane_base << 16)
+    auto end_layer = [&](int l) {
+      fence_proxy_async_global();
+      fence_before();
+      asm volatile("bar.sync 1, %0;" ::"r"(32 * EPW) : "memory");
+      if (warp == 2 && lane == 0 && l + 1 < nl) mbar_arrive(act_ready);
+    };
+    for (int l = 0; l < plan.nfwd; ++l) {
+      TAIL_COORDS;
+      const TcOp& op = layer(l);
+      const GemmDesc g = op.g;
+      const int bn = op.bn, ncols = min(bn, op.NE), nchunks = (ncols + 15) >> 4;
+      if (wg == 0 || op.ME > 128)
+        epi_fwd<F16, VAR>(g, folds, hp, om, 0, 0, ncols, nchunks, min(((256 - bn) & ~15) >> 4, nchunks), f, f < op.ME, wg, trow,
+                          trow + (uint32_t)bn, tmem_full, (uint32_t)l & 1u, nullptr);
+      if (l + 1 < plan.nfwd) end_layer(l);
+    }
+    {
+      TAIL_COORDS;
+      const int l = plan.nfwd - 1;
+      const TcOp& op = layer(l);
+      const int ncols = min(op.bn, op.NE);
+      const LossDesc& L = *static_cast<const LossDesc*>(op.hd);
+      if (op.head == HEAD_DISC) head_disc<F16, EPW>(trow, 0, wg == 0 ? ncols : 0, ncols, lane_base, lane, warp - 2, L, hp, om, sl, part);
+      else head_fm<F16, VAR>(trow, ncols, f, f < op.ME, lane, L, hp, om, red + (warp - 2));
+      end_layer(l);
+      if (warp == 2 && lane == 0) head_publish<EPW>(op, folds, hp, part, red);
+    }
+    for (int l = plan.nfwd; l < nl; ++l) {
+      TAIL_COORDS;
+      const TcOp& op = layer(l);
+      const GemmDesc g = op.g;
+      const int bn = op.bn, ncols = min(bn, op.NE), nchunks = (ncols + 15) >> 4;
+      epi_dx<F16, VAR, false>(g, hp, om, 0, 0, ncols, nchunks, min(((256 - bn) & ~15) >> 4, nchunks), f, f < op.ME, trow,
+                              trow + (uint32_t)bn, tmem_full, (uint32_t)l & 1u);
+      end_layer(l);
+    }
+#undef TAIL_COORDS
+  }
+
+  fence_before();
+  __syncthreads();
+  if (warp == 1) {
+    fence_after();
+    asm volatile("tcgen05.dealloc.cta_group::1.sync.aligned.b32 %0, %1;" ::"r"(tmem_base), "r"(512u) : "memory");
+  }
+}
diff --git a/mr_gan_b200/csrc/mrgan_api.cu b/mr_gan_b200/csrc/mrgan_api.cu
--- a/mr_gan_b200/csrc/mrgan_api.cu
+++ b/mr_gan_b200/csrc/mrgan_api.cu
@@ -79,6 +79,7 @@
 bool tc_launch_gemm(mrgan_handle* h, int op, int f0, int nfl, int rows_override, cudaStream_t st);
 void tc_launch_dw_adam(mrgan_handle* h, int op, int nlayers, int f0, int nfl, cudaStream_t st);
 bool tc_dw_merge(const mrgan_handle* h);
+void tc_launch_tail(mrgan_handle* h, int gen, int f0, int nfl);
 int tc_debug_gemm(mrgan_handle* h, int mode, const GemmDesc& g, int esz);
 }
 
@@ -690,6 +691,9 @@
 
 int heads_on(const mrgan_handle* h) { return h->cfg.precision != MRGAN_PREC_FP32 ? h->tc_heads : 0; }
 
+constexpr int kTailMinFolds = 8;
+bool use_tail(int nfl) { return nfl >= kTailMinFolds; }
+
 void enqueue_gen_fwd(mrgan_handle* h, int f0, int nfl, int op_g3) {
   launch_gemm(h, OP_G1, f0, nfl, 0);
   if (heads_on(h) & 4) {
@@ -719,8 +723,10 @@
   h->hp.t = t;
   launch_prep(h, f0, nfl, 0, from_stage, t, 2 * B);
   enqueue_gen_fwd(h, f0, nfl, OP_G3D);
-  for (int l = 0; l < 6; ++l) launch_gemm(h, OP_D1 + l, f0, nfl, 0);
-  if (!heads) {
+  const bool tail = heads && use_tail(nfl);
+  for (int l = 0; l < (tail ? 2 : 6); ++l) launch_gemm(h, OP_D1 + l, f0, nfl, 0);
+  if (tail) tc_launch_tail(h, 0, f0, nfl);
+  else if (!heads) {
     int lb = h->dp_losspart ? (3 * B + 511) / 512 : 1;
     lb = lb < 1 ? 1 : (lb > LOSS_MAX_BLOCKS ? LOSS_MAX_BLOCKS : lb);
     launch_k(h, k_loss_disc, dim3(lb, 1, nfl), dim3(256), 0, h->stream, (const LossDesc*)(h->d_loss + f0), h->d_step_stats, f0, h->nf, t, B,
@@ -728,7 +734,7 @@
   }
   const bool merge = tc_dw_merge(h);
   for (int l = 6; l >= 1; --l) {
-    if (l >= 2) launch_gemm(h, OP_DX2 + l - 2, f0, nfl, 0);
+    if (l >= 2 && !(tail && l >= 4)) launch_gemm(h, OP_DX2 + l - 2, f0, nfl, 0);
     if (merge && l > 3) continue;
     fork_side(h);
     if (merge && l == 3) { tc_launch_dw_adam(h, OP_DW3, 4, f0, nfl, h->side); continue; }
@@ -747,8 +753,10 @@
   h->hp.t = t;
   launch_prep(h, f0, nfl, 1, from_stage, t, 2 * B);
   enqueue_gen_fwd(h, f0, nfl, OP_G3G);
-  for (int l = 0; l < 5; ++l) launch_gemm(h, OP_D1G + l, f0, nfl, 0);
-  if (h->d_dpbufs) {
+  const bool tail = (hm & 2) && use_tail(nfl);
+  for (int l = 0; l < (tail ? 2 : 5); ++l) launch_gemm(h, OP_D1G + l, f0, nfl, 0);
+  if (tail) tc_launch_tail(h, 1, f0, nfl);
+  else if (h->d_dpbufs) {
     const dim3 fmg((kDW[4] + BN_COLS - 1) / BN_COLS, split_chunks(B), nfl), fmt(B > 256 ? 1024 : 256);
     k_fm_stats<<<fmg, fmt, 0, h->stream>>>(h->d_loss + f0, h->d_dpbufs + f0, B);
     dp_allreduce(h, h->dp_fm + (size_t)f0 * 2 * kDW[4], (size_t)nfl * 2 * kDW[4]);
@@ -759,7 +767,7 @@
     launch_k(h, k_fm, dim3(1, 1, nfl), dim3(1024), 0, h->stream, (const LossDesc*)(h->d_loss + f0), h->d_step_stats, f0, h->nf, t, B,
              h->om, h->hp.alpha);
   }
-  for (int l = 5; l >= 2; --l) launch_gemm(h, OP_DX2G + l - 2, f0, nfl, 0);
+  for (int l = tail ? 3 : 5; l >= 2; --l) launch_gemm(h, OP_DX2G + l - 2, f0, nfl, 0);
   launch_gemm(h, OP_DX1G, f0, nfl, 0);
   launch_gemm(h, OP_GX3, f0, nfl, 0);
   fork_side(h);
@@ -1060,6 +1068,7 @@
   cudaFuncSetAttribute(K_TC_FWD2(F, V), cudaFuncAttributeMaxDynamicSharedMemorySize, 227 * 1024);
   cudaFuncSetAttribute(K_TC_DX2(F, V), cudaFuncAttributeMaxDynamicSharedMemorySize, 227 * 1024);
   cudaFuncSetAttribute(K_TC_DW(F, V), cudaFuncAttributeMaxDynamicSharedMemorySize, (int)tc_smem_bytes(128, TC_DW_STAGES));
+  cudaFuncSetAttribute(k_tail_tc<F, V>, cudaFuncAttributeMaxDynamicSharedMemorySize, 227 * 1024);
   if (!V) cudaFuncSetAttribute(k_dw_adam_tc<F, (F ? 32 : 16)>, cudaFuncAttributeMaxDynamicSharedMemorySize, (int)TcAdamCfg<F, (F ? 32 : 16)>::SMEM);
 }
 void tc_set_smem_attr() {
@@ -1278,6 +1287,20 @@
 }
 
 bool tc_dw_merge(const mrgan_handle* h) { return h->cfg.precision != MRGAN_PREC_FP32 && h->d_tcadam != nullptr; }
+
+#define K_TAIL(F, V) k_tail_tc<F, V>
+void tc_launch_tail(mrgan_handle* h, int gen, int f0, int nfl) {
+  static const TailPlan plans[2] = {{OP_D3, 4, OP_DX6, 3}, {OP_D3G, 3, OP_DX5G, 2}};
+  const TailPlan& p = plans[gen];
+  int bn = 0;
+  for (int l = 0; l < p.nfwd; ++l) bn = std::max(bn, h->tc_bn[p.fwd0 + l]);
+  for (int l = 0; l < p.ndx; ++l) bn = std::max(bn, h->tc_bn[p.dx0 - l]);
+  const uint32_t stage = 2 * 128 * 128 + (uint32_t)bn * 128;
+  const size_t fixed = 1024 + 1024 + (size_t)h->R * h->cfg.n_classes * sizeof(float);
+  const int stages = (int)std::min<size_t>(TAIL_MAX_STAGES, (227 * 1024 - fixed) / stage);
+  TC_LAUNCH(h, h->om.mode == 2, K_TAIL, dim3(nfl), dim3(TC_FWD_THREADS), fixed + (size_t)stages * stage, h->stream, h->d_tcops + f0, h->nf, p,
+            h->d_folds, h->hp, h->om, stages, stage);
+}
 
 bool tc_launch_gemm(mrgan_handle* h, int op, int f0, int nfl, int rows_override, cudaStream_t st) {
   const OpInfo& oi = h->ops[op];
```

Measured after the change: 45870, median of 6. 4.2% higher.
